# PaddlePaddle/Paddle3D

Measured on AMD Instinct MI355X. Metric: scenes/sec CenterPoint-Pillars nuScenes 300k-pt sweeps, higher is better.
Workload: dtype f32

## Files before the change

### include/paddle3d_amd.h

```cpp
#ifndef PADDLE3D_AMD_H
#define PADDLE3D_AMD_H

#include <stddef.h>
#include <stdint.h>

#ifdef __cplusplus
extern "C" {
#endif

#define PD3_OK 0
#define PD3_EINVAL (-1)
#define PD3_EWORKSPACE (-2)
#define PD3_EUNSUPPORTED (-3)

int pd3_version(void);
const char *pd3_target_arch(void);

int pd3_selfcheck_lds_atomic_order(const uint32_t *addr, uint32_t *old, int blocks, int waves_per_block, int rounds,
                                   int table, void *stream);

size_t pd3_hard_voxelize_workspace(int batch, int64_t max_points, int num_point_dim,
                                   const float *voxel_size, const float *point_cloud_range,
                                   int max_num_points_in_voxel, int max_voxels);
int pd3_hard_voxelize(const float *points, const int32_t *num_points, int batch, int64_t max_points,
                      int num_point_dim, const float *voxel_size, const float *point_cloud_range,
                      int max_num_points_in_voxel, int max_voxels, float *voxels, int32_t *coords,
                      int32_t *num_points_per_voxel, int32_t *num_voxels, int32_t *coors_batched,
                      void *workspace, size_t workspace_bytes, void *stream);
int pd3_hard_voxelize_path(const float *points, const int32_t *num_points, int batch, int64_t max_points,
                           int num_point_dim, const float *voxel_size, const float *point_cloud_range,
                           int max_num_points_in_voxel, int max_voxels, float *voxels, int32_t *coords,
                           int32_t *num_points_per_voxel, int32_t *num_voxels, int32_t *coors_batched,
                           void *workspace, size_t workspace_bytes, void *stream, int path);

int64_t pd3_hard_voxelize_index_list_entries(int batch, int64_t max_points);
int pd3_hard_voxelize_index(const float *points, const int32_t *num_points, int batch, int64_t max_points,
                            int num_point_dim, const float *voxel_size, const float *point_cloud_range,
                            int max_num_points_in_voxel, int max_voxels, int32_t *vox_span, int32_t *point_list,
                            int32_t *coords, int32_t *num_points_per_voxel, int32_t *num_voxels,
                            int32_t *coors_batched, void *workspace, size_t workspace_bytes, void *stream);

int pd3_hard_voxelize_f64(const double *points, const int32_t *num_points, int batch, int64_t max_points,
                          int num_point_dim, const float *voxel_size, const float *point_cloud_range,
                          int max_num_points_in_voxel, int max_voxels, double *voxels, int32_t *coords,
                          int32_t *num_points_per_voxel, int32_t *num_voxels, int32_t *coors_batched,
                          void *workspace, size_t workspace_bytes, void *stream);

int pd3_dynamic_voxelize(const float *points, int64_t num_points, int num_point_dim, const float *voxel_size,
                         const float *point_cloud_range, int32_t *coors, void *stream);

size_t pd3_pointpillars_scatter_workspace(int batch, int ny, int nx);
int pd3_pointpillars_scatter(const float *voxel_features, const int32_t *coords,
                             int64_t num_pillars, int channels, int batch, int ny, int nx,
                             float *canvas, void *workspace, size_t workspace_bytes, void *stream);

int pd3_pointpillars_inverse_map(const int32_t *coords, int64_t num_pillars, int batch, int ny, int nx,
                                 int32_t *inv, void *stream);
int pd3_scatter_conv3x3_bias_relu(const float *voxel_features, const int32_t *inv, const float *w_packed,
                                  const float *bias, int batch, int cin, int cout, int ny, int nx, int stride,
                                  int relu, float *out, int out_w, void *stream);

size_t pd3_pillar_conv_rulebook_workspace(int batch, int ny, int nx, int stride);
int pd3_pillar_conv_rulebook(const int32_t *inverse_map, int batch, int ny, int nx, int stride, int32_t *nbr,
                             int32_t *out_cell, int32_t *cell_row, int32_t *n_out, int capacity, int32_t *order,
                             void *workspace, size_t workspace_bytes, void *stream);
int pd3_rows_to_dense_fill(const float *rows, const int32_t *cell_row, const float *fill, int batch, int channels, int h,
                           int w, float *out, void *stream);

int pd3_pillar_feature_net(const float *voxels, const int32_t *num_points, const int32_t *coors,
                           int64_t num_pillars, int max_points, int num_point_dim,
                           int voxel_center_dims, float vx, float vy, float vz, float x_offset,
                           float y_offset, float z_offset, const float *w1, const float *scale1,
                           const float *shift1, int c1, const float *w2, const float *scale2,
                           const float *shift2, int c2, float *out, void *stream);

int pd3_pillar_feature_net_path(const float *voxels, const int32_t *num_points, const int32_t *coors,
                                int64_t num_pillars, int max_points, int num_point_dim,
                                int voxel_center_dims, float vx, float vy, float vz, float x_offset,
                                float y_offset, float z_offset, const float *w1, const float *scale1,
                                const float *shift1, int c1, const float *w2, const float *scale2,
                                const float *shift2, int c2, float *out, int path, void *stream);

int pd3_pillar_feature_net_indexed(const float *points, int64_t points_per_frame, const int32_t *vox_span,
                                   const int32_t *point_list, int64_t list_stride, const int32_t *coors,
                                   int64_t num_pillars, int pillars_per_frame, int max_points, int num_point_dim,
                                   int voxel_center_dims, float vx, float vy, float vz, float x_offset,
                                   float y_offset, float z_offset, const float *w1, const float *scale1,
                                   const float *shift1, int c1, const float *w2, const float *scale2,
                                   const float *shift2, int c2, float *out, void *stream);

int pd3_voxel_mean(const float *voxels, const int32_t *num_points, int64_t num_voxels,
                   int max_points, int num_point_dim, float *out, void *stream);

size_t pd3_nms_workspace(int num_boxes);
int pd3_nms_bev(const float *boxes, int num_boxes, float nms_overlap_thresh, int32_t *keep,
                int32_t *num_to_keep, void *workspace, size_t workspace_bytes, void *stream);
int pd3_nms_normal(const float *boxes, int num_boxes, float nms_overlap_thresh, int32_t *keep,
                   int32_t *num_to_keep, void *workspace, size_t workspace_bytes, void *stream);
int pd3_boxes_iou_bev(const float *boxes_a, int num_a, const float *boxes_b, int num_b,
                      float *ans_iou, void *stream);
int pd3_boxes_overlap_bev(const float *boxes_a, int num_a, const float *boxes_b, int num_b,
                          float *ans_overlap, void *stream);
int pd3_libm_eval(int op, const float *x, const float *y, float *out, int64_t n, void *stream);

size_t pd3_centerpoint_postprocess_workspace(int batch, int num_tasks, int feat_h, int feat_w,
                                             int nms_pre_max_size, int nms_post_max_size);
int pd3_centerpoint_postprocess(const float *const *hm, const float *const *reg,
                                const float *const *height, const float *const *dim,
                                const float *const *vel, const float *const *rot, int batch,
                                int num_tasks, const int *hm_channels, int feat_h, int feat_w,
                                const float *voxel_size, const float *point_cloud_range,
                                const float *post_center_range, const int *label_offsets,
                                int down_ratio, float score_threshold, float nms_iou_threshold,
                                int nms_pre_max_size, int nms_post_max_size, int with_velocity,
                                float *out_bboxes, float *out_scores, int64_t *out_labels,
                                int32_t *out_count, void *workspace, size_t workspace_bytes,
                                void *stream);

int pd3_centerpoint_postprocess_strided(const float *const *hm, const float *const *reg,
                                const float *const *height, const float *const *dim,
                                const float *const *vel, const float *const *rot, int64_t head_batch_stride, int batch,
                                int num_tasks, const int *hm_channels, int feat_h, int feat_w,
                                const float *voxel_size, const float *point_cloud_range,
                                const float *post_center_range, const int *label_offsets,
                                int down_ratio, float score_threshold, float nms_iou_threshold,
                                int nms_pre_max_size, int nms_post_max_size, int with_velocity,
                                float *out_bboxes, float *out_scores, int64_t *out_labels,
                                int32_t *out_count, void *workspace, size_t workspace_bytes,
                                void *stream, int selection);
int pd3_centerpoint_postprocess_records(const float *const *hm, const float *const *reg,
                                        const float *const *height, const float *const *dim,
                                        const float *const *vel, const float *const *rot,
                                        int64_t head_batch_stride, int batch, int num_tasks,
                                        const int *hm_channels, int feat_h, int feat_w, const float *voxel_size,
                                        const float *point_cloud_range, const float *post_center_range,
                                        const int *label_offsets, int down_ratio, float score_threshold,
                                        float nms_iou_threshold, int nms_pre_max_size, int nms_post_max_size,
                                        int with_velocity, float *out_bboxes, float *out_scores,
                                        int64_t *out_labels, int32_t *out_count, float *out_records,
                                        int max_per_img, void *workspace, size_t workspace_bytes, void *stream);

size_t pd3_bevdet_postprocess_workspace(int batch, int num_tasks, const int *task_classes, int feat_h, int feat_w,
                                        int max_num);
int pd3_bevdet_postprocess(const float *const *heatmap, const float *const *reg, const float *const *height,
                           const float *const *dim, const float *const *rot, const float *const *vel, int batch,
                           int num_tasks, const int *task_classes, int feat_h, int feat_w, const int *nms_type,
                           const float *nms_thr, const double *min_radius, const float *rescale_factors,
                           int max_num, int pre_max_size, int post_max_size, float score_threshold, int norm_bbox,
                           const float *post_center_range, const float *post_center_limit_range,
                           const float *pc_range, const float *voxel_size, float out_size_factor,
                           float *out_bboxes, float *out_scores, int32_t *out_labels, int32_t *out_count,
                           void *workspace, size_t workspace_bytes, void *stream);

size_t pd3_circle_nms_workspace(int n);
int pd3_circle_nms(const float *dets, int n, double thresh, int32_t *keep, int32_t *num_to_keep, void *workspace,
                   size_t workspace_bytes, void *stream);

int pd3_bevdet4d_align(const float *const *feats, const int64_t *strides, int num_frame, int with_current,
                       int batch, int channels, int feat_h, int feat_w, const float *const *rots_cur,
                       const float *const *trans_cur, const float *const *rots_adj, const float *const *trans_adj,
                       const float *const *bda, const float *const *bda_adj, const int64_t *pose_strides,
                       const float *grid_interval, const float *grid_lower_bound, float *out, float *out_grid,
                       void *stream);

int pd3_ms_deform_attn_forward(int dtype, const void *value, const int64_t *spatial_shapes,
                               const int64_t *level_start_index, const void *sampling_loc, const void *attn_weight,
                               int batch, int spatial_size, int num_heads, int channels, int num_levels,
                               int num_query, int num_point, void *out, void *stream);
int pd3_ms_deform_attn_backward(int dtype, const void *value, const int64_t *spatial_shapes,
                                const int64_t *level_start_index, const void *sampling_loc, const void *attn_weight,
                                const void *grad_out, int batch, int spatial_size, int num_heads, int channels,
                                int num_levels, int num_query, int num_point, void *grad_value,
                                void *grad_sampling_loc, void *grad_attn_weight, void *stream);

size_t pd3_farthest_point_sample_workspace(int batch, int n, int tier);
int pd3_farthest_point_sample(const float *xyz, int batch, int n, int m, int tier, void *workspace,
                              size_t workspace_bytes, int *idxs, void *stream);

int pd3_gather_points(const float *points, const int *idx, int batch, int channels, int n, int npoints, float *out,
                      void *stream);
int pd3_gather_points_grad(const float *grad_out, const int *idx, int batch, int channels, int n, int npoints,
                           float *grad_points, void *stream);

int pd3_ball_query_batch(const float *new_xyz, const float *xyz, int batch, int n, int m, float radius, int nsample,
                         int *idx, void *stream);

int pd3_group_points_batch(const float *points, const int *idx, int batch, int channels, int n, int npoints,
                           int nsample, float *out, void *stream);
int pd3_group_points_batch_grad(const float *grad_out, const int *idx, int batch, int channels, int n, int npoints,
                                int nsample, float *grad_points, void *stream);

int pd3_points_in_boxes(const float *pts, const float *boxes, int batch, int npts, int nboxes, int64_t box_row_stride,
                        int64_t box_batch_stride, int *box_idx_of_points, void *stream);

int pd3_ball_query_stack(const float *new_xyz, const int *new_xyz_batch_cnt, const float *xyz,
                         const int *xyz_batch_cnt, int batch, int m, int n, float radius, int nsample, int *idx,
                         void *stream);

int pd3_voxel_query(const float *new_xyz, const float *xyz, const int *new_coords, const int *point_indices, int m,
                    int n, int batch, int z, int y, int x, float radius, int nsample, int z_range, int y_range,
                    int x_range, int *idx, void *stream);

int pd3_group_points_stack(const float *features, const int *features_batch_cnt, const int *idx,
                           const int *idx_batch_cnt, int batch, int n, int channels, int m, int nsample, float *out,
                           void *stream);
int pd3_group_points_stack_grad(const float *grad_out, const int *idx, const int *idx_batch_cnt,
                                const int *features_batch_cnt, int batch, int n, int channels, int m, int nsample,
                                float *grad_features, void *stream);

int pd3_voxel_pool(const float *new_xyz, const float *xyz, const int *new_coords, const int *point_indices,
                   const float *features_in, const float *w_pos, const float *pos_scale, const float *pos_shift, int m,
                   int n, int batch, int z, int y, int x, int c1, float radius, int nsample, int z_range, int y_range,
                   int x_range, int pool, float *pooled, void *stream);

int pd3_roi_grid_points(const float *rois, int64_t num_rois, int rois_per_frame, int grid_size, const float *range_min,
                        const float *voxel_size, const int *strides, int num_strides, float *roi_grid_xyz, int *coords,
                        void *stream);

int pd3_rcnn_decode_boxes(const float *rois, const float *box_preds, int64_t n, float *out, void *stream);

size_t pd3_class_agnostic_nms_workspace(int batch, int64_t num_boxes, int nms_pre_maxsize);
int pd3_class_agnostic_nms(const float *box_preds, const float *cls_preds, int batch, int64_t num_boxes,
                           int num_classes, int apply_sigmoid, float score_thresh, const int64_t *labels,
                           int nms_pre_maxsize, float nms_thresh, int nms_post_maxsize, float *out_boxes,
                           float *out_scores, int64_t *out_labels, int32_t *out_count, void *workspace,
                           size_t workspace_bytes, void *stream);

int pd3_assign_score_withk_forward(const float *scores, const float *points, const float *centers,
                                   const int64_t *knn_idx, int batch, int n, int k, int m, int o, float *output,
                                   void *stream);
size_t pd3_assign_score_withk_backward_workspace(int batch, int n, int k, int o);
int pd3_assign_score_withk_backward(const float *grad_out, const float *scores, const float *points,
                                    const float *centers, const int64_t *knn_idx, int batch, int n, int k, int m,
                                    int o, float *grad_scores, float *grad_points, float *grad_centers,
                                    void *workspace, size_t workspace_bytes, void *stream);

int pd3_bev_pool_v2(const float *depth, const float *feat, const int32_t *ranks_depth,
                    const int32_t *ranks_feat, const int32_t *ranks_bev,
                    const int32_t *interval_lengths, const int32_t *interval_starts,
                    int n_intervals, int channels, int64_t out_elems, float *out, void *stream);
int pd3_bev_pool_v2_bkwd(const float *out_grad, const float *depth, const float *feat,
                         const int32_t *ranks_depth, const int32_t *ranks_feat,
                         const int32_t *ranks_bev, const int32_t *interval_lengths,
                         const int32_t *interval_starts, int n_intervals, int64_t n_points,
                         int channels, int64_t depth_elems, int64_t feat_elems, float *depth_grad,
                         float *feat_grad, void *stream);

int pd3_frustum_to_lidar(const float *frustum, int64_t points_per_camera, int batch, int num_cams,
                         const float *inv_post_rots, const float *post_trans, const float *cam_to_ego,
                         const float *trans, const float *bda, float *coor, void *stream);

size_t pd3_voxel_pooling_prepare_workspace(int64_t num_points);
int pd3_voxel_pooling_prepare(const float *coor, int64_t num_points, int batch, int depth_bins, int feat_hw,
                              const float *grid_lower, const float *grid_interval, const float *grid_size, int mode,
                              int32_t *ranks_bev, int32_t *ranks_depth, int32_t *ranks_feat,
                              int32_t *interval_starts, int32_t *interval_lengths, int32_t *counts, void *workspace,
                              size_t workspace_bytes, void *stream);

size_t pd3_sparse_conv3d_workspace(int n_in, const int *kernel_size, int subm, int out_cap);
int pd3_sparse_conv3d_indices(const int32_t *in_coords, int n_in, int batch, const int *spatial_shape,
                              const int *kernel_size, const int *stride, const int *padding, int subm,
                              int32_t *out_coords, int32_t *nbr, int32_t *n_out, int out_cap,
                              void *workspace, size_t workspace_bytes, void *stream);
int pd3_sparse_conv3d_features(const float *in_feats, const int32_t *nbr, const int32_t *n_out,
                               int n_out_cap, int kernel_volume, int cin, int cout,
                               const float *weight, const float *bias, const float *scale,
                               const float *shift, const float *residual, int relu, float *out,
                               void *stream);
int64_t pd3_sparse_tile_order_entries(int n_out_cap);
int pd3_sparse_tile_order(const int32_t *nbr, const int32_t *n_out, int n_out_cap, int kernel_volume,
                          int32_t *order, void *stream);
int pd3_sparse_conv3d_features_ordered(const float *in_feats, const int32_t *nbr, const int32_t *n_out,
                                       int n_out_cap, int kernel_volume, int cin, int cout,
                                       const float *weight, const float *bias, const float *scale,
                                       const float *shift, const float *residual, int relu,
                                       const int32_t *order, float *out, void *stream);
int pd3_sparse_pack_weight_bf16x3(const float *weight, int kernel_volume, int cin, int cout, void *packed, void *stream);
int pd3_sparse_conv3d_features_bf16x3(const float *in_feats, const int32_t *nbr, const int32_t *n_out, int n_out_cap,
                                      int kernel_volume, int cin, int cout, const void *weight_packed,
                                      const float *bias, const float *scale, const float *shift, const float *residual,
                                      int relu, const int32_t *order, float *out, void *stream);
int pd3_sparse_pack_weight_f16(const float *weight, int kernel_volume, int cin, int cout, void *packed, void *stream);
int pd3_sparse_conv3d_features_f16(const void *in_feats_f16, const int32_t *nbr, const int32_t *n_out, int n_out_cap,
                                   int kernel_volume, int cin, int cout, const void *weight_packed_f16,
                                   const float *bias, const float *scale, const float *shift,
                                   const void *residual_f16, int relu, const int32_t *order, void *out, int out_f32,
                                   void *stream);
int pd3_gather_gemm_f16(const void *in_feats_f16, const int32_t *nbr, const int32_t *n_out, int n_out_cap,
                        int kernel_volume, int cin, int cout, const void *weight_packed_f16, const float *bias,
                        const float *scale, const float *shift, const void *residual_f16, int relu,
                        const int32_t *order, void *out, int out_f32, int out_ld, int out_off, void *stream);
size_t pd3_sparse_plan_workspace(int n_cap);
size_t pd3_sparse_conv_outputs_workspace(int batch, const int *spatial_shape, const int *kernel_size,
                                         const int *stride, const int *padding);
int pd3_sparse_sort_coords(const int32_t *coords, int n, int batch, const int *spatial_shape,
                           uint32_t *keys_sorted, int32_t *order, int32_t *n_valid, void *workspace,
                           size_t workspace_bytes, void *stream);
int pd3_sparse_conv_outputs(const uint32_t *in_keys, const int32_t *n_in, int n_in_cap, int batch,
                            const int *spatial_shape, const int *kernel_size, const int *stride,
                            const int *padding, uint32_t *out_keys, int32_t *n_out, int out_cap,
                            void *workspace, size_t workspace_bytes, void *stream);
size_t pd3_sparse_rulebook_workspace(int batch, const int *spatial_shape);
int pd3_sparse_rulebook(const uint32_t *in_keys, const int32_t *n_in, int n_in_cap, const uint32_t *out_keys,
                        const int32_t *n_out, int n_out_cap, int batch, const int *spatial_shape,
                        const int *kernel_size, const int *stride, const int *padding, int subm, int32_t *nbr,
                        int32_t *out_coords, void *workspace, size_t workspace_bytes, void *stream);
int pd3_sparse_to_dense(const float *feats, const int32_t *coords, const int32_t *n, int n_cap,
                        int channels, int batch, const int *spatial_shape, float *dense, void *stream);

size_t pd3_merge_sweeps_workspace(int64_t num_points);
int pd3_merge_sweeps(const float *points, const int64_t *sweep_offsets, int num_sweeps, int dim_in,
                     int use_dim, const double *ref_from_curr, const int32_t *has_transform,
                     const float *time_lag, int use_time_lag,
                     float remove_radius, float *out, int32_t *num_out, void *workspace,
                     size_t workspace_bytes, void *stream);

int pd3_conv3x3_bias_relu(const float *x, const float *w_packed, const float *bias, int batch, int cin,
                          int cout, int h, int w, int w_valid, int stride, int relu, float *out, int out_w,
                          void *stream);

int pd3_conv3x3_winograd43_bias_relu(const float *x, const float *u_packed, const float *bias, int batch,
                                     int cin, int cout, int h, int w, int w_valid, int relu, float *out,
                                     int channels_per_tile, void *stream);

int pd3_conv3x3_winograd43_pp_bias_relu(const float *x, const float *u_lane, const float *bias, int batch, int cin,
                                        int cout, int h, int w, int w_valid, int relu, float *out, void *stream);

size_t pd3_winograd43_input_transform_floats(int batch, int cin, int h, int w);
int pd3_winograd43_input_transform(const float *x, int batch, int cin, int h, int w, int w_valid, float *v_pre,
                                   void *stream);
int pd3_conv3x3_winograd43_ppv_bias_relu(const float *v_pre, const float *u_lane, const float *bias, int batch, int cin,
                                         int cout, int h, int w, int w_valid, int relu, float *out, void *stream);
int pd3_conv3x3_winograd43_pp_trace(const float *x, const float *u_lane, const float *bias, int batch, int cin, int cout,
                                    int h, int w, int relu, float *out, long long *dbg, void *stream);

size_t pd3_stable_argsort_workspace(int64_t n, uint32_t max_key);
int pd3_stable_argsort(const void *keys, int64_t n, int mode, uint32_t max_key, int32_t *order, void *workspace,
                       size_t workspace_bytes, void *stream);

int pd3_conv3x3_f16_bias_relu(const void *x_f16_nhwc, const void *w_packed_f16, const float *bias, int batch, int cin,
                              int cout, int h, int w, int relu, void *out, int out_mode, int channels_per_tile,
                              void *stream);
int pd3_conv3x3_f16_bias_relu_dual(const void *x_f16_nhwc, const void *w_packed_f16, const float *bias, int batch,
                                   int cin, int cout, int h, int w, int relu, void *out_f16_nhwc, float *out_f32_nchw,
                                   int channels_per_tile, void *stream);
int pd3_conv3x3_s2_f16_bias_relu(const void *x_f16_nhwc, const void *w_packed_f16, const float *bias, int batch, int cin,
                                 int cout, int h, int w, int relu, void *out_f16_nhwc, void *stream);
int pd3_scatter_conv3x3_s2_f16_bias_relu(const void *features_f16, const int32_t *inverse_map, const void *w_packed_f16,
                                         const float *bias, int batch, int cin, int cout, int ny, int nx, int relu,
                                         void *out_f16_nhwc, int channels_per_tile, void *stream);
int pd3_grouped_conv3x3_small_f16(const void *x_f16_nhwc, const void *w_f16, const float *bias, int batch, int groups,
                                  int channels_per_group, int out_per_group, int h, int w, float *out, int out_groups,
                                  int out_group0, void *stream);
int pd3_grouped_conv3x3_small_f16_gm(const void *x_f16_group_major, const void *w_f16, const float *bias, int batch,
                                     int groups, int channels_per_group, int out_per_group, int h, int w, float *out,
                                     int out_groups, int out_group0, void *stream);
int pd3_f32_nchw_to_f16_nhwc(const float *x, int batch, int channels, int h, int w, void *out, void *stream);

int pd3_grouped_conv3x3_small(const float *x, const float *w_grouped, const float *bias, int batch, int groups,
                              int cin_per_group, int cout_per_group, int h, int w, float *out, void *stream);
int pd3_grouped_conv3x3_small_slice(const float *x, const float *w_grouped, const float *bias, int batch, int groups,
                                    int cin_per_group, int cout_per_group, int h, int w, float *out, int out_groups,
                                    int out_group0, void *stream);

int pd3_conv3x3_winograd_bias_relu(const float *x, const float *u_packed, const float *bias, int batch,
                                   int cin, int cout, int h, int w, int relu, float *out, void *stream);

int pd3_patch_conv_bias_relu(const float *x, const float *w_packed, const float *bias, int mode, int batch,
                             int cin, int cout, int h, int w, int w_valid, int relu, float *out,
                             int out_channels_total, int out_channel_offset, void *stream);

int pd3_patch_conv_x3_bias_relu(const float *x, const void *w_packed, const float *bias, int mode, int batch, int cin,
                                int cout, int h, int w, int w_valid, int relu, float *out, int out_channels_total,
                                int out_channel_offset, void *stream);

int pd3_conv3x3_s2_x3_bias_relu(const float *x, const void *w_packed, const float *bias, int batch, int cin, int cout,
                                int h, int w, int w_valid, int relu, float *out, int out_w, void *stream);

size_t pd3_ssd_postprocess_workspace(int batch, int feat_h, int feat_w, int anchors_per_loc, int grid_x, int grid_y,
                                     int nms_pre_max_size);
int pd3_ssd_postprocess(const float *head_map, int64_t batch_stride, int cls_channel0, int box_channel0,
                        int dir_channel0, int batch, int feat_h, int feat_w, int anchors_per_loc, int num_classes,
                        int encode_background_as_zeros, const float *anchors, const int32_t *anchors_bv,
                        const int32_t *coors, int64_t num_coors, int grid_x, int grid_y,
                        float anchor_area_threshold, float score_threshold, const float *center_limit_range,
                        float nms_iou_threshold, int nms_pre_max_size, int nms_post_max_size, float *out_boxes,
                        float *out_scores, int64_t *out_labels, int32_t *out_count, void *workspace,
                        size_t workspace_bytes, void *stream, int selection);

#ifdef __cplusplus
}
#endif
#endif
```

### paddle3d_amd/_lib.py

```python
from __future__ import annotations

import ctypes as C
import os
from functools import lru_cache

_HERE = os.path.dirname(os.path.abspath(__file__))
LIB_PATH = os.path.join(_HERE, "lib", "libpaddle3d_amd.so")

c_f32p = C.c_void_p
c_i32p = C.c_void_p

_SIGNATURES = {
    "pd3_version": (C.c_int, []),
    "pd3_target_arch": (C.c_char_p, []),
    "pd3_hard_voxelize_workspace": (C.c_size_t, [C.c_int, C.c_int64, C.c_int, C.c_void_p, C.c_void_p,
                                                 C.c_int, C.c_int]),
    "pd3_hard_voxelize": (C.c_int, [C.c_void_p, C.c_void_p, C.c_int, C.c_int64, C.c_int, C.c_void_p,
                                    C.c_void_p, C.c_int, C.c_int, C.c_void_p, C.c_void_p, C.c_void_p,
                                    C.c_void_p, C.c_void_p, C.c_void_p, C.c_size_t, C.c_void_p]),
    "pd3_hard_voxelize_f64": (C.c_int, [C.c_void_p, C.c_void_p, C.c_int, C.c_int64, C.c_int, C.c_void_p,
                                    C.c_void_p, C.c_int, C.c_int, C.c_void_p, C.c_void_p, C.c_void_p,
                                    C.c_void_p, C.c_void_p, C.c_void_p, C.c_size_t, C.c_void_p]),
    "pd3_hard_voxelize_path": (C.c_int, [C.c_void_p, C.c_void_p, C.c_int, C.c_int64, C.c_int, C.c_void_p,
                                         C.c_void_p, C.c_int, C.c_int, C.c_void_p, C.c_void_p, C.c_void_p,
                                         C.c_void_p, C.c_void_p, C.c_void_p, C.c_size_t, C.c_void_p, C.c_int]),
    "pd3_hard_voxelize_index_list_entries": (C.c_int64, [C.c_int, C.c_int64]),
    "pd3_hard_voxelize_index": (C.c_int, [C.c_void_p, C.c_void_p, C.c_int, C.c_int64, C.c_int, C.c_void_p,
                                          C.c_void_p, C.c_int, C.c_int, C.c_void_p, C.c_void_p, C.c_void_p,
                                          C.c_void_p, C.c_void_p, C.c_void_p, C.c_void_p, C.c_size_t, C.c_void_p]),
    "pd3_pillar_feature_net_indexed": (C.c_int, [C.c_void_p, C.c_int64, C.c_void_p, C.c_void_p, C.c_int64, C.c_void_p,
                                                 C.c_int64, C.c_int, C.c_int, C.c_int, C.c_int, C.c_float, C.c_float,
                                                 C.c_float, C.c_float, C.c_float, C.c_float, C.c_void_p, C.c_void_p,
                                                 C.c_void_p, C.c_int, C.c_void_p, C.c_void_p, C.c_void_p, C.c_int,
                                                 C.c_void_p, C.c_void_p]),
    "pd3_pointpillars_scatter_workspace": (C.c_size_t, [C.c_int, C.c_int, C.c_int]),
    "pd3_pointpillars_scatter": (C.c_int, [C.c_void_p, C.c_void_p, C.c_int64, C.c_int, C.c_int, C.c_int,
                                           C.c_int, C.c_void_p, C.c_void_p, C.c_size_t, C.c_void_p]),
    "pd3_pillar_feature_net": (C.c_int, [C.c_void_p, C.c_void_p, C.c_void_p, C.c_int64, C.c_int, C.c_int,
                                         C.c_int, C.c_float, C.c_float, C.c_float, C.c_float, C.c_float,
                                         C.c_float, C.c_void_p,
                                         C.c_void_p, C.c_void_p, C.c_int, C.c_void_p, C.c_void_p,
                                         C.c_void_p, C.c_int, C.c_void_p, C.c_void_p]),
    "pd3_pillar_feature_net_path": (C.c_int, [C.c_void_p, C.c_void_p, C.c_void_p, C.c_int64, C.c_int, C.c_int,
                                              C.c_int, C.c_float, C.c_float, C.c_float, C.c_float, C.c_float,
                                              C.c_float, C.c_void_p,
                                              C.c_void_p, C.c_void_p, C.c_int, C.c_void_p, C.c_void_p,
                                              C.c_void_p, C.c_int, C.c_void_p, C.c_int, C.c_void_p]),
    "pd3_voxel_mean": (C.c_int, [C.c_void_p, C.c_void_p, C.c_int64, C.c_int, C.c_int, C.c_void_p,
                                 C.c_void_p]),
    "pd3_nms_workspace": (C.c_size_t, [C.c_int]),
    "pd3_nms_bev": (C.c_int, [C.c_void_p, C.c_int, C.c_float, C.c_void_p, C.c_void_p, C.c_void_p,
                              C.c_size_t, C.c_void_p]),
    "pd3_nms_normal": (C.c_int, [C.c_void_p, C.c_int, C.c_float, C.c_void_p, C.c_void_p, C.c_void_p,
                                 C.c_size_t, C.c_void_p]),
    "pd3_boxes_iou_bev": (C.c_int, [C.c_void_p, C.c_int, C.c_void_p, C.c_int, C.c_void_p, C.c_void_p]),
    "pd3_boxes_overlap_bev": (C.c_int, [C.c_void_p, C.c_int, C.c_void_p, C.c_int, C.c_void_p,
                                        C.c_void_p]),
    "pd3_libm_eval": (C.c_int, [C.c_int, C.c_void_p, C.c_void_p, C.c_void_p, C.c_int64, C.c_void_p]),
    "pd3_centerpoint_postprocess_workspace": (C.c_size_t, [C.c_int, C.c_int, C.c_int, C.c_int, C.c_int, C.c_int]),
    "pd3_centerpoint_postprocess": (C.c_int, [C.c_void_p] * 6 + [C.c_int, C.c_int, C.c_void_p, C.c_int, C.c_int,
                                              C.c_void_p, C.c_void_p, C.c_void_p, C.c_void_p, C.c_int,
                                              C.c_float, C.c_float, C.c_int, C.c_int, C.c_int,
                                              C.c_void_p, C.c_void_p, C.c_void_p, C.c_void_p,
                                              C.c_void_p, C.c_size_t, C.c_void_p]),
    "pd3_centerpoint_postprocess_strided": (C.c_int, [C.c_void_p] * 6 + [C.c_int64, C.c_int, C.c_int, C.c_void_p,
                                                      C.c_int, C.c_int, C.c_void_p, C.c_void_p, C.c_void_p,
                                                      C.c_void_p, C.c_int, C.c_float, C.c_float, C.c_int, C.c_int,
                                                      C.c_int, C.c_void_p, C.c_void_p, C.c_void_p, C.c_void_p,
                                                      C.c_void_p, C.c_size_t, C.c_void_p, C.c_int]),
    "pd3_centerpoint_postprocess_records": (C.c_int, [C.c_void_p] * 6 + [C.c_int64, C.c_int, C.c_int, C.c_void_p,
                                                      C.c_int, C.c_int, C.c_void_p, C.c_void_p, C.c_void_p,
                                                      C.c_void_p, C.c_int, C.c_float, C.c_float, C.c_int, C.c_int,
                                                      C.c_int, C.c_void_p, C.c_void_p, C.c_void_p, C.c_void_p,
                                                      C.c_void_p, C.c_int, C.c_void_p, C.c_size_t, C.c_void_p]),
    "pd3_ms_deform_attn_forward": (C.c_int, [C.c_int] + [C.c_void_p] * 5 + [C.c_int] * 7 + [C.c_void_p] * 2),
    "pd3_ms_deform_attn_backward": (C.c_int, [C.c_int] + [C.c_void_p] * 6 + [C.c_int] * 7 + [C.c_void_p] * 4),
    "pd3_farthest_point_sample_workspace": (C.c_size_t, [C.c_int, C.c_int, C.c_int]),
    "pd3_farthest_point_sample": (C.c_int, [C.c_void_p, C.c_int, C.c_int, C.c_int, C.c_int, C.c_void_p, C.c_size_t,
                                            C.c_void_p, C.c_void_p]),
    "pd3_gather_points": (C.c_int, [C.c_void_p, C.c_void_p] + [C.c_int] * 4 + [C.c_void_p, C.c_void_p]),
    "pd3_gather_points_grad": (C.c_int, [C.c_void_p, C.c_void_p] + [C.c_int] * 4 + [C.c_void_p, C.c_void_p]),
    "pd3_ball_query_batch": (C.c_int, [C.c_void_p, C.c_void_p, C.c_int, C.c_int, C.c_int, C.c_float, C.c_int,
                                       C.c_void_p, C.c_void_p]),
    "pd3_group_points_batch": (C.c_int, [C.c_void_p, C.c_void_p] + [C.c_int] * 5 + [C.c_void_p, C.c_void_p]),
    "pd3_group_points_batch_grad": (C.c_int, [C.c_void_p, C.c_void_p] + [C.c_int] * 5 + [C.c_void_p, C.c_void_p]),
    "pd3_points_in_boxes": (C.c_int, [C.c_void_p, C.c_void_p, C.c_int, C.c_int, C.c_int, C.c_int64, C.c_int64,
                                      C.c_void_p, C.c_void_p]),
    "pd3_ball_query_stack": (C.c_int, [C.c_void_p] * 4 + [C.c_int] * 3 + [C.c_float, C.c_int, C.c_void_p,
                                                                            C.c_void_p]),
    "pd3_voxel_query": (C.c_int, [C.c_void_p] * 4 + [C.c_int] * 6 + [C.c_float] + [C.c_int] * 4 + [C.c_void_p] * 2),
    "pd3_group_points_stack": (C.c_int, [C.c_void_p] * 4 + [C.c_int] * 5 + [C.c_void_p] * 2),
    "pd3_group_points_stack_grad": (C.c_int, [C.c_void_p] * 4 + [C.c_int] * 5 + [C.c_void_p] * 2),
    "pd3_assign_score_withk_forward": (C.c_int, [C.c_void_p] * 4 + [C.c_int] * 5 + [C.c_void_p] * 2),
    "pd3_assign_score_withk_backward_workspace": (C.c_size_t, [C.c_int] * 4),
    "pd3_assign_score_withk_backward": (C.c_int, [C.c_void_p] * 5 + [C.c_int] * 5 + [C.c_void_p] * 4 +
                                        [C.c_size_t, C.c_void_p]),
    "pd3_bev_pool_v2": (C.c_int, [C.c_void_p] * 7 + [C.c_int, C.c_int, C.c_int64, C.c_void_p,
                                                     C.c_void_p]),
    "pd3_bev_pool_v2_bkwd": (C.c_int, [C.c_void_p] * 8 + [C.c_int, C.c_int64, C.c_int, C.c_int64, C.c_int64,
                                                          C.c_void_p, C.c_void_p, C.c_void_p]),
    "pd3_frustum_to_lidar": (C.c_int, [C.c_void_p, C.c_int64, C.c_int, C.c_int] + [C.c_void_p] * 7),
    "pd3_voxel_pooling_prepare_workspace": (C.c_size_t, [C.c_int64]),
    "pd3_voxel_pooling_prepare": (C.c_int, [C.c_void_p, C.c_int64, C.c_int, C.c_int, C.c_int, C.c_void_p, C.c_void_p,
                                            C.c_void_p, C.c_int] + [C.c_void_p] * 7 + [C.c_size_t, C.c_void_p]),
    "pd3_sparse_conv3d_workspace": (C.c_size_t, [C.c_int, C.c_void_p, C.c_int, C.c_int]),
    "pd3_sparse_conv3d_indices": (C.c_int, [C.c_void_p, C.c_int, C.c_int, C.c_void_p, C.c_void_p, C.c_void_p,
                                            C.c_void_p, C.c_int, C.c_void_p, C.c_void_p, C.c_void_p, C.c_int,
                                            C.c_void_p, C.c_size_t, C.c_void_p]),
    "pd3_sparse_conv3d_features": (C.c_int, [C.c_void_p, C.c_void_p, C.c_void_p, C.c_int, C.c_int, C.c_int,
                                             C.c_int, C.c_void_p, C.c_void_p, C.c_void_p, C.c_void_p,
                                             C.c_void_p, C.c_int, C.c_void_p, C.c_void_p]),
    "pd3_sparse_conv3d_features_ordered": (C.c_int, [C.c_void_p, C.c_void_p, C.c_void_p, C.c_int, C.c_int, C.c_int,
                                                     C.c_int, C.c_void_p, C.c_void_p, C.c_void_p, C.c_void_p,
                                                     C.c_void_p, C.c_int, C.c_void_p, C.c_void_p, C.c_void_p]),
    "pd3_sparse_pack_weight_bf16x3": (C.c_int, [C.c_void_p, C.c_int, C.c_int, C.c_int, C.c_void_p, C.c_void_p]),
    "pd3_sparse_conv3d_features_bf16x3": (C.c_int, [C.c_void_p, C.c_void_p, C.c_void_p, C.c_int, C.c_int, C.c_int,
                                                    C.c_int, C.c_void_p, C.c_void_p, C.c_void_p, C.c_void_p, C.c_void_p,
                                                    C.c_int, C.c_void_p, C.c_void_p, C.c_void_p]),
    "pd3_sparse_pack_weight_f16": (C.c_int, [C.c_void_p, C.c_int, C.c_int, C.c_int, C.c_void_p, C.c_void_p]),
    "pd3_sparse_conv3d_features_f16": (C.c_int, [C.c_void_p, C.c_void_p, C.c_void_p, C.c_int, C.c_int, C.c_int, C.c_int,
                                                 C.c_void_p, C.c_void_p, C.c_void_p, C.c_void_p, C.c_void_p, C.c_int,
                                                 C.c_void_p, C.c_void_p, C.c_int, C.c_void_p]),
    "pd3_gather_gemm_f16": (C.c_int, [C.c_void_p, C.c_void_p, C.c_void_p, C.c_int, C.c_int, C.c_int, C.c_int,
                                      C.c_void_p, C.c_void_p, C.c_void_p, C.c_void_p, C.c_void_p, C.c_int, C.c_void_p,
                                      C.c_void_p, C.c_int, C.c_int, C.c_int, C.c_void_p]),
    "pd3_sparse_tile_order_entries": (C.c_int64, [C.c_int]),
    "pd3_sparse_tile_order": (C.c_int, [C.c_void_p, C.c_void_p, C.c_int, C.c_int, C.c_void_p, C.c_void_p]),
    "pd3_sparse_plan_workspace": (C.c_size_t, [C.c_int]),
    "pd3_sparse_conv_outputs_workspace": (C.c_size_t, [C.c_int] + [C.c_void_p] * 4),
    "pd3_sparse_sort_coords": (C.c_int, [C.c_void_p, C.c_int, C.c_int, C.c_void_p, C.c_void_p, C.c_void_p,
                                         C.c_void_p, C.c_void_p, C.c_size_t, C.c_void_p]),
    "pd3_sparse_conv_outputs": (C.c_int, [C.c_void_p, C.c_void_p, C.c_int, C.c_int, C.c_void_p, C.c_void_p,
                                          C.c_void_p, C.c_void_p, C.c_void_p, C.c_void_p, C.c_int, C.c_void_p,
                                          C.c_size_t, C.c_void_p]),
    "pd3_sparse_rulebook_workspace": (C.c_size_t, [C.c_int, C.c_void_p]),
    "pd3_sparse_rulebook": (C.c_int, [C.c_void_p, C.c_void_p, C.c_int, C.c_void_p, C.c_void_p, C.c_int, C.c_int,
                                      C.c_void_p, C.c_void_p, C.c_void_p, C.c_void_p, C.c_int, C.c_void_p,
                                      C.c_void_p, C.c_void_p, C.c_size_t, C.c_void_p]),
    "pd3_sparse_to_dense": (C.c_int, [C.c_void_p, C.c_void_p, C.c_void_p, C.c_int, C.c_int, C.c_int,
                                      C.c_void_p, C.c_void_p, C.c_void_p]),
    "pd3_selfcheck_lds_atomic_order": (C.c_int, [C.c_void_p, C.c_void_p, C.c_int, C.c_int, C.c_int, C.c_int,
                                                 C.c_void_p]),
    "pd3_conv3x3_f16_bias_relu": (C.c_int, [C.c_void_p, C.c_void_p, C.c_void_p, C.c_int, C.c_int, C.c_int, C.c_int,
                                            C.c_int, C.c_int, C.c_void_p, C.c_int, C.c_int, C.c_void_p]),
    "pd3_f32_nchw_to_f16_nhwc": (C.c_int, [C.c_void_p, C.c_int, C.c_int, C.c_int, C.c_int, C.c_void_p, C.c_void_p]),
    "pd3_conv3x3_f16_bias_relu_dual": (C.c_int, [C.c_void_p, C.c_void_p, C.c_void_p, C.c_int, C.c_int, C.c_int, C.c_int,
                                                 C.c_int, C.c_int, C.c_void_p, C.c_void_p, C.c_int, C.c_void_p]),
    "pd3_conv3x3_s2_f16_bias_relu": (C.c_int, [C.c_void_p, C.c_void_p, C.c_void_p, C.c_int, C.c_int, C.c_int, C.c_int,
                                               C.c_int, C.c_int, C.c_void_p, C.c_void_p]),
    "pd3_scatter_conv3x3_s2_f16_bias_relu": (C.c_int, [C.c_void_p, C.c_void_p, C.c_void_p, C.c_void_p, C.c_int, C.c_int,
                                                       C.c_int, C.c_int, C.c_int, C.c_int, C.c_void_p, C.c_int,
                                                       C.c_void_p]),
    "pd3_grouped_conv3x3_small_f16": (C.c_int, [C.c_void_p, C.c_void_p, C.c_void_p, C.c_int, C.c_int, C.c_int, C.c_int,
                                                C.c_int, C.c_int, C.c_void_p, C.c_int, C.c_int, C.c_void_p]),
    "pd3_grouped_conv3x3_small_f16_gm": (C.c_int, [C.c_void_p, C.c_void_p, C.c_void_p, C.c_int, C.c_int, C.c_int, C.c_int,
                                                   C.c_int, C.c_int, C.c_void_p, C.c_int, C.c_int, C.c_void_p]),
    "pd3_stable_argsort_workspace": (C.c_size_t, [C.c_int64, C.c_uint32]),
    "pd3_stable_argsort": (C.c_int, [C.c_void_p, C.c_int64, C.c_int, C.c_uint32, C.c_void_p, C.c_void_p, C.c_size_t,
                                     C.c_void_p]),
    "pd3_conv3x3_winograd43_pp_bias_relu": (C.c_int, [C.c_void_p, C.c_void_p, C.c_void_p, C.c_int, C.c_int, C.c_int,
                                                       C.c_int, C.c_int, C.c_int, C.c_int, C.c_void_p, C.c_void_p]),
    "pd3_conv3x3_winograd43_pp_trace": (C.c_int, [C.c_void_p, C.c_void_p, C.c_void_p, C.c_int, C.c_int, C.c_int, C.c_int,
                                                  C.c_int, C.c_int, C.c_void_p, C.c_void_p, C.c_void_p]),
    "pd3_merge_sweeps_workspace": (C.c_size_t, [C.c_int64]),
    "pd3_merge_sweeps": (C.c_int, [C.c_void_p, C.c_void_p, C.c_int, C.c_int, C.c_int, C.c_void_p, C.c_void_p,
                                   C.c_void_p, C.c_int, C.c_float, C.c_void_p, C.c_void_p, C.c_void_p, C.c_size_t,
                                   C.c_void_p]),
    "pd3_dynamic_voxelize": (C.c_int, [C.c_void_p, C.c_int64, C.c_int, C.c_void_p, C.c_void_p, C.c_void_p, C.c_void_p]),
    "pd3_conv3x3_bias_relu": (C.c_int, [C.c_void_p, C.c_void_p, C.c_void_p, C.c_int, C.c_int, C.c_int, C.c_int,
                                        C.c_int, C.c_int, C.c_int, C.c_int, C.c_void_p, C.c_int, C.c_void_p]),
    "pd3_conv3x3_winograd_bias_relu": (C.c_int, [C.c_void_p, C.c_void_p, C.c_void_p, C.c_int, C.c_int, C.c_int,
                                                 C.c_int, C.c_int, C.c_int, C.c_void_p, C.c_void_p]),
    "pd3_conv3x3_winograd43_bias_relu": (C.c_int, [C.c_void_p, C.c_void_p, C.c_void_p, C.c_int, C.c_int, C.c_int,
                                                   C.c_int, C.c_int, C.c_int, C.c_int, C.c_void_p, C.c_int,
                                                   C.c_void_p]),
    "pd3_patch_conv_bias_relu": (C.c_int, [C.c_void_p, C.c_void_p, C.c_void_p, C.c_int, C.c_int, C.c_int, C.c_int,
                                           C.c_int, C.c_int, C.c_int, C.c_int, C.c_void_p, C.c_int, C.c_int,
                                           C.c_void_p]),
    "pd3_patch_conv_x3_bias_relu": (C.c_int, [C.c_void_p, C.c_void_p, C.c_void_p, C.c_int, C.c_int, C.c_int, C.c_int,
                                              C.c_int, C.c_int, C.c_int, C.c_int, C.c_void_p, C.c_int, C.c_int,
                                              C.c_void_p]),
    "pd3_conv3x3_s2_x3_bias_relu": (C.c_int, [C.c_void_p, C.c_void_p, C.c_void_p, C.c_int, C.c_int, C.c_int, C.c_int,
                                              C.c_int, C.c_int, C.c_int, C.c_void_p, C.c_int, C.c_void_p]),
    "pd3_winograd43_input_transform_floats": (C.c_size_t, [C.c_int] * 4),
    "pd3_winograd43_input_transform": (C.c_int, [C.c_void_p, C.c_int, C.c_int, C.c_int, C.c_int, C.c_int, C.c_void_p,
                                                 C.c_void_p]),
    "pd3_conv3x3_winograd43_ppv_bias_relu": (C.c_int, [C.c_void_p, C.c_void_p, C.c_void_p, C.c_int, C.c_int, C.c_int,
                                                       C.c_int, C.c_int, C.c_int, C.c_int, C.c_void_p, C.c_void_p]),
    "pd3_ssd_postprocess_workspace": (C.c_size_t, [C.c_int] * 7),
    "pd3_ssd_postprocess": (C.c_int, [C.c_void_p, C.c_int64, C.c_int, C.c_int, C.c_int, C.c_int, C.c_int, C.c_int,
                                      C.c_int, C.c_int, C.c_int, C.c_void_p, C.c_void_p, C.c_void_p, C.c_int64,
                                      C.c_int, C.c_int, C.c_float, C.c_float, C.c_void_p, C.c_float, C.c_int, C.c_int,
                                      C.c_void_p, C.c_void_p, C.c_void_p, C.c_void_p, C.c_void_p, C.c_size_t,
                                      C.c_void_p, C.c_int]),
    "pd3_pointpillars_inverse_map": (C.c_int, [C.c_void_p, C.c_int64, C.c_int, C.c_int, C.c_int, C.c_void_p,
                                               C.c_void_p]),
    "pd3_scatter_conv3x3_bias_relu": (C.c_int, [C.c_void_p, C.c_void_p, C.c_void_p, C.c_void_p, C.c_int, C.c_int,
                                                C.c_int, C.c_int, C.c_int, C.c_int, C.c_int, C.c_void_p, C.c_int,
                                                C.c_void_p]),
    "pd3_pillar_conv_rulebook_workspace": (C.c_size_t, [C.c_int] * 4),
    "pd3_pillar_conv_rulebook": (C.c_int, [C.c_void_p, C.c_int, C.c_int, C.c_int, C.c_int, C.c_void_p, C.c_void_p,
                                           C.c_void_p, C.c_void_p, C.c_int, C.c_void_p, C.c_void_p, C.c_size_t,
                                           C.c_void_p]),
    "pd3_rows_to_dense_fill": (C.c_int, [C.c_void_p, C.c_void_p, C.c_void_p, C.c_int, C.c_int, C.c_int, C.c_int,
                                         C.c_void_p, C.c_void_p]),
    "pd3_bevdet_postprocess_workspace": (C.c_size_t, [C.c_int, C.c_int, C.c_void_p, C.c_int, C.c_int, C.c_int]),
    "pd3_bevdet_postprocess": (C.c_int, [C.c_void_p] * 6 + [C.c_int, C.c_int, C.c_void_p, C.c_int, C.c_int,
                                         C.c_void_p, C.c_void_p, C.c_void_p, C.c_void_p, C.c_int, C.c_int,
                                         C.c_int, C.c_float, C.c_int, C.c_void_p, C.c_void_p, C.c_void_p,
                                         C.c_void_p, C.c_float, C.c_void_p, C.c_void_p, C.c_void_p, C.c_void_p,
                                         C.c_void_p, C.c_size_t, C.c_void_p]),
    "pd3_circle_nms_workspace": (C.c_size_t, [C.c_int]),
    "pd3_circle_nms": (C.c_int, [C.c_void_p, C.c_int, C.c_double, C.c_void_p, C.c_void_p, C.c_void_p, C.c_size_t,
                                 C.c_void_p]),
    "pd3_bevdet4d_align": (C.c_int, [C.c_void_p, C.c_void_p] + [C.c_int] * 6 + [C.c_void_p] * 12),
    "pd3_grouped_conv3x3_small": (C.c_int, [C.c_void_p, C.c_void_p, C.c_void_p, C.c_int, C.c_int, C.c_int, C.c_int,
                                            C.c_int, C.c_int, C.c_void_p, C.c_void_p]),
    "pd3_grouped_conv3x3_small_slice": (C.c_int, [C.c_void_p, C.c_void_p, C.c_void_p, C.c_int, C.c_int, C.c_int,
                                                  C.c_int, C.c_int, C.c_int, C.c_void_p, C.c_int, C.c_int,
                                                  C.c_void_p]),
}

SYMBOLS = tuple(_SIGNATURES)

_SIGNATURES_ROI = {
    "pd3_voxel_pool": (C.c_int, [C.c_void_p] * 8 + [C.c_int] * 7 + [C.c_float] + [C.c_int] * 5 + [C.c_void_p] * 2),
    "pd3_roi_grid_points": (C.c_int, [C.c_void_p, C.c_int64, C.c_int, C.c_int] + [C.c_void_p] * 3 + [C.c_int] +
                            [C.c_void_p] * 3),
    "pd3_rcnn_decode_boxes": (C.c_int, [C.c_void_p, C.c_void_p, C.c_int64, C.c_void_p, C.c_void_p]),
    "pd3_class_agnostic_nms_workspace": (C.c_size_t, [C.c_int, C.c_int64, C.c_int]),
    "pd3_class_agnostic_nms": (C.c_int, [C.c_void_p, C.c_void_p, C.c_int, C.c_int64, C.c_int, C.c_int, C.c_float,
                                         C.c_void_p, C.c_int, C.c_float, C.c_int] + [C.c_void_p] * 5 +
                               [C.c_size_t, C.c_void_p]),
}

SYMBOLS_ROI = tuple(_SIGNATURES_ROI)


class Paddle3DAmdError(RuntimeError):
    pass


@lru_cache(maxsize=None)
def lib() -> C.CDLL:
    if not os.path.exists(LIB_PATH):
        raise Paddle3DAmdError(
            f"{LIB_PATH} not found: build it with `python -m paddle3d_amd.build` "
            "(there is no CPU / PyTorch fallback for the HIP ops)")
    handle = C.CDLL(LIB_PATH)
    for name, (res, args) in list(_SIGNATURES.items()) + list(_SIGNATURES_ROI.items()):
        try:
            fn = getattr(handle, name)
        except AttributeError as e:
            raise Paddle3DAmdError(f"{LIB_PATH} does not export {name}") from e
        fn.restype = res
        fn.argtypes = args
    return handle


def check(status: int, what: str) -> None:
    if status == 0:
        return
    if status < 0:
        msg = {-1: "invalid argument", -2: "workspace too small", -3: "unsupported configuration"}.get(
            status, "error")
        raise Paddle3DAmdError(f"{what}: {msg} (status {status})")
    raise Paddle3DAmdError(f"{what}: HIP error {status}")
```

### paddle3d_amd/build.py

```python
from __future__ import annotations

import concurrent.futures as cf
import os
import subprocess
import sys

HERE = os.path.dirname(os.path.abspath(__file__))
CSRC = os.path.join(HERE, "csrc")
OBJ = os.path.join(HERE, "lib", "obj")
LIB = os.path.join(HERE, "lib", "libpaddle3d_amd.so")
ARCH = "gfx950"
HIPCC = os.environ.get("HIPCC", "/opt/rocm/bin/hipcc")
FLAGS = [f"--offload-arch={ARCH}", "-O3", "-std=c++17", "-fPIC", "-ffp-contract=off", "-fno-fast-math",
         "-Wall", "-Wno-unused-function", "-Wno-unused-result"]


def _sources():
    return sorted(os.path.join(CSRC, f) for f in os.listdir(CSRC) if f.endswith(".hip"))


def _headers():
    hs = [os.path.join(CSRC, f) for f in os.listdir(CSRC) if f.endswith(".hpp")]
    hs.append(os.path.join(HERE, "..", "include", "paddle3d_amd.h"))
    return hs


def _stale(target, deps):
    if not os.path.exists(target):
        return True
    t = os.path.getmtime(target)
    return any(os.path.getmtime(d) > t for d in deps)


EXTRA_FLAGS = {}


def _compile(src, force):
    obj = os.path.join(OBJ, os.path.basename(src)[:-4] + ".o")
    if force or _stale(obj, [src] + _headers()):
        cmd = [HIPCC, *FLAGS, *EXTRA_FLAGS.get(os.path.basename(src), []), "-c", src, "-o", obj]
        r = subprocess.run(cmd, capture_output=True, text=True)
        if r.returncode != 0:
            raise RuntimeError(f"hipcc failed for {src}:\n{r.stdout}\n{r.stderr}")
        if r.stderr.strip():
            sys.stderr.write(r.stderr)
    return obj


def build(force: bool = False) -> str:
    os.makedirs(OBJ, exist_ok=True)
    srcs = _sources()
    with cf.ThreadPoolExecutor(max_workers=min(8, len(srcs))) as ex:
        objs = list(ex.map(lambda s: _compile(s, force), srcs))
    if force or _stale(LIB, objs):
        cmd = [HIPCC, f"--offload-arch={ARCH}", "-shared", "-fPIC", "-o", LIB, *objs]
        r = subprocess.run(cmd, capture_output=True, text=True)
        if r.returncode != 0:
            raise RuntimeError(f"link failed:\n{r.stdout}\n{r.stderr}")
    return LIB


if __name__ == "__main__":
    print(build(force="--force" in sys.argv))
```

### paddle3d_amd/centerpoint.py

```python
from __future__ import annotations

import math

import numpy as np
import torch
import torch.nn as nn

from ._lib import Paddle3DAmdError
from .ops import centerpoint_postprocess as _cp
from .ops import conv as _conv
from .ops import pointpillars_scatter as _ps
from .ops import sparse_conv3d as _sp3
from .ops import voxel_encoder as _ve
from .ops import voxelize as _vox

__all__ = ["HardVoxelizer", "PillarFeatureNet", "HardVFE", "VoxelMean", "PointPillarsScatter", "SecondBackbone",
           "SecondFPN", "CenterHead", "CenterPoint", "centerpoint_pillars_nuscenes", "centerpoint_pillars_kitti",
           "centerpoint_voxels_nuscenes", "centerpoint_voxels_kitti", "load_paddle_state_dict"]


def _grid(voxel_size, point_cloud_range):
    pr = np.array(point_cloud_range, dtype=np.float32)
    vs = np.array(voxel_size, dtype=np.float32)
    return np.round((pr[3:] - pr[:3]) / vs).astype(np.int64)


class HardVoxelizer(nn.Module):

    def __init__(self, voxel_size, point_cloud_range, max_num_points_in_voxel, max_num_voxels, path: int = 0):
        super().__init__()
        self.path = int(path)
        self.voxel_size = list(map(float, voxel_size))
        self.point_cloud_range = list(map(float, point_cloud_range))
        self.max_num_points_in_voxel = int(max_num_points_in_voxel)
        if isinstance(max_num_voxels, (tuple, list)):
            self.max_num_voxels = list(max_num_voxels)
        else:
            self.max_num_voxels = [max_num_voxels, max_num_voxels]

    def forward(self, points: torch.Tensor, num_points: torch.Tensor | None = None):
        v = self.max_num_voxels[0] if self.training else self.max_num_voxels[1]
        voxels, _, npv, nv, coors = _vox.hard_voxelize_batch(points, self.voxel_size, self.point_cloud_range,
                                                             self.max_num_points_in_voxel, v, num_points,
                                                             with_batch_coors=True, path=self.path)
        return voxels, coors, npv, nv

    def index(self, points: torch.Tensor, num_points: torch.Tensor | None = None):
        if self.path != 0:
            return None
        v = self.max_num_voxels[0] if self.training else self.max_num_voxels[1]
        res = _vox.hard_voxelize_index_batch(points, self.voxel_size, self.point_cloud_range,
                                             self.max_num_points_in_voxel, v, num_points)
        if res is None:
            return None
        span, plist, _, npv, nv, coors = res
        return span, plist, coors, npv, nv


class PFNLayer(nn.Module):

    def __init__(self, in_channels, out_channels, last_layer=False):
        super().__init__()
        self.last_vfe = last_layer
        self.units = out_channels if last_layer else out_channels // 2
        self.linear = nn.Linear(in_channels, self.units, bias=False)
        self.norm = nn.BatchNorm1d(self.units, eps=1e-3, momentum=0.01)
        bound = 1 / math.sqrt(in_channels)
        nn.init.uniform_(self.linear.weight, -bound, bound)


class PillarFeatureNet(nn.Module):

    def __init__(self, in_channels=4, feat_channels=(64,), with_distance=False, max_num_points_in_voxel=20,
                 voxel_size=(0.2, 0.2, 4), point_cloud_range=(0, -40, -3, 70.4, 40, 1), legacy=False):
        super().__init__()
        if with_distance or legacy:
            raise NotImplementedError("with_distance / legacy PFN variants are not on the hot path")
        if len(feat_channels) not in (1, 2):
            raise NotImplementedError("the fused PFN op covers one or two PFN layers")
        self.in_channels = in_channels
        chans = [in_channels + 5] + list(feat_channels)
        self.pfn_layers = nn.ModuleList(
            PFNLayer(chans[i], chans[i + 1], last_layer=(i == len(chans) - 2)) for i in range(len(chans) - 1))
        for i in range(1, len(self.pfn_layers)):
            assert self.pfn_layers[i].linear.in_features == 2 * self.pfn_layers[i - 1].units
        self.vx, self.vy = float(voxel_size[0]), float(voxel_size[1])
        self.x_offset = self.vx / 2 + point_cloud_range[0]
        self.y_offset = self.vy / 2 + point_cloud_range[1]
        self.max_num_points_in_voxel = max_num_points_in_voxel
        self._folded = None

    def train(self, mode: bool = True):
        self._folded = None
        return super().train(mode)

    def _fold(self):
        out = []
        for l in self.pfn_layers:
            scale, shift = _ve.fold_batchnorm(l.norm.weight, l.norm.bias, l.norm.running_mean,
                                              l.norm.running_var, l.norm.eps)
            out += [l.linear.weight.t().contiguous(), scale, shift]
        return [t.detach() for t in out]

    def forward(self, features, num_points_per_voxel, coors):
        sig = _param_signature(self)
        if self.training or self._folded is None or self._folded[0] != sig:
            self._folded = (sig, self._fold())
        return _ve.pillar_feature_net(features, num_points_per_voxel, coors, self.vx, self.vy, self.x_offset,
                                      self.y_offset, *self._folded[1])

    def forward_indexed(self, points, vox_span, point_list, coors):
        if len(self.pfn_layers) != 2:
            return None
        sig = _param_signature(self)
        if self.training or self._folded is None or self._folded[0] != sig:
            self._folded = (sig, self._fold())
        return _ve.pillar_feature_net_indexed(points, vox_span, point_list, coors, self.max_num_points_in_voxel,
                                              self.vx, self.vy, self.x_offset, self.y_offset, *self._folded[1])


class HardVFE(nn.Module):

    def __init__(self, in_channels=4, feat_channels=(64, 64), with_distance=False, with_cluster_center=True,
                 with_voxel_center=True, voxel_size=(0.2, 0.2, 4), point_cloud_range=(0, -40, -3, 70.4, 40, 1)):
        super().__init__()
        if with_distance or not (with_cluster_center and with_voxel_center) or len(feat_channels) != 2:
            raise NotImplementedError("HardVFE: only the BEVFusion configuration is on the hot path")
        self.voxel_size, self.point_cloud_range = tuple(voxel_size), tuple(point_cloud_range)
        chans = [in_channels + 6] + list(feat_channels)

        class _VFE(nn.Module):
            def __init__(self, cin, cout):
                super().__init__()
                self.linear = nn.Linear(cin, cout, bias=False)
                self.norm = nn.BatchNorm1d(cout, eps=1e-3, momentum=0.01)

        self.vfe_layers = nn.ModuleList([_VFE(chans[0], chans[1]), _VFE(2 * chans[1], chans[2])])

    def forward(self, features, num_points, coors):
        args = []
        for l in self.vfe_layers:
            scale, shift = _ve.fold_batchnorm(l.norm.weight, l.norm.bias, l.norm.running_mean, l.norm.running_var,
                                              l.norm.eps)
            args += [l.linear.weight.t().contiguous().detach(), scale.detach(), shift.detach()]
        return _ve.hard_vfe(features, num_points, coors, self.voxel_size, self.point_cloud_range, *args)


class VoxelMean(nn.Module):

    def __init__(self, in_channels=4):
        super().__init__()
        self.in_channels = in_channels

    def forward(self, features, num_points_per_voxel, coors=None):
        assert self.in_channels == features.shape[-1]
        return _ve.voxel_mean(features, num_points_per_voxel)


class PointPillarsScatter(nn.Module):

    def __init__(self, in_channels, voxel_size, point_cloud_range):
        super().__init__()
        self.in_channels = in_channels
        g = _grid(voxel_size, point_cloud_range)
        self.nx, self.ny = int(g[0]), int(g[1])

    def forward(self, voxel_features, coords, batch_size):
        return _ps.pointpillars_scatter(voxel_features, coords, batch_size, self.ny, self.nx)

    def sparse(self, voxel_features, coords, batch_size):
        return _ps.SparseCanvas(voxel_features, coords, batch_size, self.ny, self.nx)


def _param_signature(module):
    return tuple((t.data_ptr(), t._version, str(t.device)) for t in list(module.parameters()) + list(module.buffers()))


def invalidate_derived(module):
    for m in module.modules():
        if hasattr(m, "_drop_cache"):
            m._drop_cache()
        if hasattr(m, "_folded"):
            m._folded = None
        if getattr(m, "_pd3_folded", None) is not None:
            object.__setattr__(m, "_pd3_folded", None)
    return module


class _InferenceCache:

    _cache = None
    _cache_sig = None

    def _drop_cache(self):
        self.__dict__["_cache"] = None
        self.__dict__["_cache_sig"] = None

    def _cache_valid(self):
        return self._cache is not None and self._cache_sig == _param_signature(self)

    def _store_cache(self, value):
        self.__dict__["_cache"] = value
        self.__dict__["_cache_sig"] = _param_signature(self)
        return value

    def train(self, mode: bool = True):
        self._drop_cache()
        return super().train(mode)

    def invalidate(self):
        invalidate_derived(self)
        return self

    def _require_eval(self):
        if self.training:
            raise RuntimeError(f"{type(self).__name__}: paddle3d_amd implements the inference path only "
                               "(BatchNorm folded into the HIP kernels); call .eval() first")


def _conv_bn_relu(cin, cout, k, stride=1, padding=0, transpose=False, eps=1e-3, momentum=0.01, bias=False):
    conv = (nn.ConvTranspose2d if transpose else nn.Conv2d)(cin, cout, k, stride=stride, padding=padding, bias=bias)
    return [conv, nn.BatchNorm2d(cout, eps=eps, momentum=momentum), nn.ReLU()]


def _fold_conv_bn(conv: nn.Conv2d, bn: nn.BatchNorm2d):
    scale = bn.weight / torch.sqrt(bn.running_var + bn.eps)
    if isinstance(conv, nn.ConvTranspose2d):
        w = conv.weight * scale.reshape(1, -1, 1, 1)
    else:
        w = conv.weight * scale.reshape(-1, 1, 1, 1)
    b = (conv.bias if conv.bias is not None else torch.zeros_like(bn.running_mean))
    return w.detach().contiguous(), ((b - bn.running_mean) * scale + bn.bias).detach().contiguous()


class _Conv3x3:

    def __init__(self, w, b, stride):
        self.w, self.b, self.stride = w, b, int(stride)
        self.cout, self.cin = int(w.shape[0]), int(w.shape[1])
        self.packed = {}

    def winograd43(self, h, pitch):
        if self.stride != 1:
            return None, None
        if self.cin >= _conv.WINOGRAD43_PP_MIN_CIN and _conv.winograd43_pp_supported(self.cin, self.cout, h, pitch):
            form, key, pack = "pp", "w43pp", _conv.pack_winograd43_lane_weight
        elif _conv.winograd43_supported(self.cin, self.cout, h, pitch):
            form, key, pack = "packed", "w43", _conv.pack_winograd43_weight
        else:
            return None, None
        if key not in self.packed:
            self.packed[key] = pack(self.w)
        return form, self.packed[key]

    def __call__(self, x, w_valid=None):
        h, wv = int(x.shape[2]), int(x.shape[3] if w_valid is None else w_valid)
        form, u = self.winograd43(h, int(x.shape[3]))
        if form == "pp":
            if 0 < _conv.WINOGRAD43_PPV_MIN_BLOCKS <= self.cout // 64:
                vpre = _conv.winograd43_input_transform(x, w_valid=wv)
                return _conv.conv3x3_winograd43_ppv_bias_relu(vpre, x.shape, u, self.b, self.cout, relu=True,
                                                              w_valid=wv), wv
            return _conv.conv3x3_winograd43_pp_bias_relu(x, u, self.b, self.cout, relu=True, w_valid=wv), wv
        if form == "packed":
            return _conv.conv3x3_winograd43_bias_relu(x, u, self.b, self.cout, relu=True, w_valid=wv), wv
        if (self.stride == 2 and _conv.S2_BF16X3 and int(x.shape[3]) % 4 == 0
                and _conv.conv3x3_s2_x3_supported(self.cin, self.cout, h, wv, int(x.shape[0]))):
            if "s2x3" not in self.packed:
                self.packed["s2x3"] = _conv.pack_conv3x3_s2_x3_weight(self.w)
            return _conv.conv3x3_s2_x3_bias_relu(x, self.packed["s2x3"], self.b, self.cout, relu=True,
                                                 w_valid=wv), wv // 2
        if _conv.supported(self.cin, self.cout, h, wv, self.stride):
            if "direct" not in self.packed:
                self.packed["direct"] = _conv.pack_conv3x3_weight(self.w)
            return _conv.conv3x3_bias_relu(x, self.packed["direct"], self.b, self.cout, relu=True, stride=self.stride,
                                           w_valid=wv), wv // self.stride
        raise Paddle3DAmdError(f"conv3x3: unsupported configuration (cin {self.cin}, cout {self.cout}, stride "
                               f"{self.stride}, input {h}x{wv}) (status -3)")

    def f16_ok(self, h, w):
        return self.stride == 1 and _conv.f16_supported(self.cin, self.cout, int(h), int(w))

    def f16_s2_ok(self):
        return self.stride == 2 and _conv.s2_f16_supported(self.cin, self.cout)

    def f16_s2(self, x_h):
        if "f16s2" not in self.packed:
            self.packed["f16s2"] = _conv.pack_conv3x3_f16_weight(self.w, tile=128)
        return _conv.conv3x3_s2_f16_bias_relu(x_h, self.packed["f16s2"], self.b, self.cout, relu=True)

    def f16_dual(self, x_h):
        if "f16" not in self.packed:
            self.packed["f16"] = _conv.pack_conv3x3_f16_weight(self.w)
        return _conv.conv3x3_f16_bias_relu_dual(x_h, self.packed["f16"], self.b, self.cout, relu=True)

    def f16(self, x_h, out_f32_nchw=False, out=None, tiles=None, group_major=False):
        if "f16" not in self.packed:
            self.packed["f16"] = _conv.pack_conv3x3_f16_weight(self.w)
        wp, b, cout = self.packed["f16"], self.b, self.cout
        if tiles is not None:
            t = int(wp.shape[4])
            wp, b, cout = wp[tiles[0]:tiles[1]], self.b[tiles[0] * t:tiles[1] * t], (tiles[1] - tiles[0]) * t
        return _conv.conv3x3_f16_bias_relu(x_h, wp, b, cout, relu=True, out_f32_nchw=out_f32_nchw, out=out,
                                           group_major=group_major)


def _valid_w(t) -> int:
    return int(getattr(t, "_pd3_valid_w", t.shape[3]))


def _f16_nhwc_to_f32_nchw(xh):
    x = xh.permute(0, 3, 1, 2).float()
    w = int(x.shape[3])
    pad = _conv.pitch4(w) - w
    if pad:
        x = torch.nn.functional.pad(x, (0, pad))
    return _tag_valid_w(x.contiguous(), w)


def _tag_valid_w(t, wv):
    if t.dtype == torch.float16:
        return t
    if wv != t.shape[3]:
        t._pd3_valid_w = int(wv)
    return t


def _fold_conv3x3(conv, bn):
    if (isinstance(conv, nn.ConvTranspose2d) or tuple(conv.kernel_size) != (3, 3) or tuple(conv.padding) != (1, 1)
            or tuple(conv.stride) not in ((1, 1), (2, 2))):
        raise Paddle3DAmdError(f"unsupported configuration: {conv} is not a 3x3 / pad 1 / stride 1|2 convolution")
    w, b = _fold_conv_bn(conv, bn)
    return _Conv3x3(w, b, conv.stride[0])


class SecondBackbone(_InferenceCache, nn.Module):

    def __init__(self, in_channels=128, out_channels=(128, 128, 256), layer_nums=(3, 5, 5),
                 downsample_strides=(2, 2, 2)):
        super().__init__()
        in_filters = [in_channels, *out_channels[:-1]]
        blocks = []
        for i, n in enumerate(layer_nums):
            block = _conv_bn_relu(in_filters[i], out_channels[i], 3, stride=downsample_strides[i], padding=1)
            for _ in range(n):
                block += _conv_bn_relu(out_channels[i], out_channels[i], 3, padding=1)
            blocks.append(nn.Sequential(*block))
        self.blocks = nn.ModuleList(blocks)
        self.sparse_first = True
        self.amp = False
        self.amp_out_f16 = False

    def _plan(self):
        if not self._cache_valid():
            plan = []
            for blk in self.blocks:
                mods = list(blk)
                plan.append([_fold_conv3x3(mods[i], mods[i + 1]) for i in range(0, len(mods), 3)])
            self._store_cache(plan)
        return self._cache

    def forward(self, x):
        self._require_eval()
        plan = self._plan()
        first = None
        first_h = None
        if isinstance(x, _ps.SparseCanvas):
            c0 = plan[0][0]
            if (self.amp and c0.stride == 2 and x.shape[1] == c0.cin and len(plan[0]) > 1
                    and _conv.scatter_conv_s2_f16_supported(c0.cin, c0.cout, x.ny, x.nx)
                    and plan[0][1].f16_ok(x.ny // 2, x.nx // 2)):
                key = "f16s2_64" if c0.cout % 128 else "f16s2"
                if key not in c0.packed:
                    c0.packed[key] = _conv.pack_conv3x3_f16_weight(c0.w, tile=64 if c0.cout % 128 else 128)
                first_h = _conv.scatter_conv3x3_s2_f16_bias_relu(x, c0.packed[key], c0.b, c0.cout)
                first = (None, x.nx // 2)
            elif (self.sparse_first and x.shape[1] == c0.cin
                  and _conv.scatter_conv_sparse_supported(c0.cin, c0.cout, x.ny, x.nx, c0.stride)):
                y, c0.packed["x3sparse"] = _conv.scatter_conv3x3_sparse(x, c0.w, c0.b, c0.packed.get("x3sparse"))
                first = (y, x.nx // 2)
            elif _conv.scatter_conv_supported(c0.cin, c0.cout, x.ny, x.nx, c0.stride) and x.shape[1] == c0.cin:
                if "direct" not in c0.packed:
                    c0.packed["direct"] = _conv.pack_conv3x3_weight(c0.w)
                first = (_conv.scatter_conv3x3_bias_relu(x, c0.packed["direct"], c0.b, c0.cout), x.nx // 2)
            else:
                x = x.dense()
        if first is None and x.shape[3] % 4:
            raise Paddle3DAmdError(f"SecondBackbone: unsupported configuration (input width {x.shape[3]} is not a "
                                   "multiple of 4) (status -3)")
        outs, wv = [], (0 if first is not None else int(x.shape[3]))
        carry = None
        for bi, layers in enumerate(plan):
            li = 0
            while li < len(layers):
                conv = layers[li]
                xh = None
                if first is not None and bi == 0 and li == 0:
                    x, wv = first
                    li += 1
                    if first_h is None:
                        continue
                    xh = first_h
                    conv = layers[li]
                if self.amp and li == 0 and carry is not None and conv.f16_s2_ok() and wv == carry.shape[2]:
                    xh = conv.f16_s2(carry)
                    li, wv = 1, wv // 2
                    x = None
                carry = None
                if xh is None and x.dtype == torch.float16:
                    x = _f16_nhwc_to_f32_nchw(x)
                h_now = int(xh.shape[1]) if xh is not None else int(x.shape[2])
                w_now = int(xh.shape[2]) if xh is not None else int(x.shape[3])
                run = li
                while (self.amp and run < len(layers) and wv == w_now and layers[run].f16_ok(h_now, w_now)):
                    run += 1
                if run > li and w_now % 4 and not (run == len(layers) and self.amp_out_f16):
                    run = li
                if run > li:
                    if xh is None:
                        xh = _conv.to_f16_nhwc(x)
                    nxt = plan[bi + 1][0] if bi + 1 < len(plan) else None
                    opens = run == len(layers) and nxt is not None and nxt.f16_s2_ok()
                    stage_h = run == len(layers) and self.amp_out_f16
                    for k in range(li, run):
                        if k == run - 1 and stage_h:
                            xh = layers[k].f16(xh)
                            x, carry = xh, (xh if opens else None)
                        elif k == run - 1 and opens:
                            carry, x = layers[k].f16_dual(xh)
                        else:
                            xh = layers[k].f16(xh, out_f32_nchw=(k == run - 1))
                            x = xh
                    li = run
                    continue
                if xh is not None:
                    x = _f16_nhwc_to_f32_nchw(xh)
                    continue
                x, wv = conv(x, wv)
                li += 1
            outs.append(_tag_valid_w(x, wv))
        return tuple(outs)


class SecondFPN(_InferenceCache, nn.Module):

    def __init__(self, in_channels=(128, 128, 256), out_channels=(256, 256, 256), upsample_strides=(1, 2, 4),
                 use_conv_for_no_stride=False):
        super().__init__()
        deblocks = []
        for i, oc in enumerate(out_channels):
            stride = upsample_strides[i]
            if stride > 1 or (stride == 1 and not use_conv_for_no_stride):
                layer = _conv_bn_relu(in_channels[i], oc, int(stride), stride=int(stride), transpose=True)
            else:
                s = round(1 / stride)
                layer = _conv_bn_relu(in_channels[i], oc, s, stride=s)
            deblocks.append(nn.Sequential(*layer))
        self.deblocks = nn.ModuleList(deblocks)

    def _plan(self):
        if not self._cache_valid():
            plan, off = [], 0
            for blk in self.deblocks:
                conv, bn = blk[0], blk[1]
                tr = isinstance(conv, nn.ConvTranspose2d)
                w, b = _fold_conv_bn(conv, bn)
                mode = _conv.patch_mode(w, conv.stride[0], tr)
                if mode is None or tuple(conv.padding) != (0, 0) or conv.stride[0] != conv.stride[1]:
                    raise Paddle3DAmdError(f"unsupported configuration: FPN level {conv} is not a kernel = stride "
                                           "(conv 1 / 2, transposed conv 1 / 2 / 4) layer (status -3)")
                cout = int(w.shape[1] if tr else w.shape[0])
                cin = int(w.shape[0] if tr else w.shape[1])
                plan.append(dict(mode=mode, w=_conv.pack_patch_weight(w, mode, tr), wraw=w, tr=tr, b=b, cin=cin, cout=cout, off=off,
                                 scale={0: 0.5, 1: 1, 2: 2, 3: 4}[mode]))
                off += cout
            self._store_cache((plan, off))
        return self._cache

    def _amp_level(self, i, p, n, h, w, dev, tag=None):
        key = (i, n, h, w, str(dev))
        cache = self.__dict__.setdefault("_amp_tables", {})
        if len(cache) > 64:
            cache.clear()
        if key not in cache:
            conv = self.deblocks[i][0]
            s = int(conv.stride[0])
            tr = isinstance(conv, nn.ConvTranspose2d)
            ho, wo = (h * s, w * s) if tr else (h // s, w // s)
            b = torch.arange(n, device=dev).view(n, 1, 1)
            y = torch.arange(ho, device=dev).view(1, ho, 1)
            x = torch.arange(wo, device=dev).view(1, 1, wo)
            if tr:
                src = ((b * h + y // s) * w + x // s).reshape(-1)
                tap = ((y % s) * s + x % s).expand(n, ho, wo).reshape(-1)
                nbr = torch.full((n * ho * wo, s * s), -1, dtype=torch.int32, device=dev)
                nbr[torch.arange(n * ho * wo, device=dev), tap] = src.int()
            else:
                cols = [((b * h + y * s + dy) * w + x * s + dx).reshape(-1) for dy in range(s) for dx in range(s)]
                nbr = torch.stack(cols, 1).int().contiguous()
            order = _sp3.tile_order(nbr) if tr and s > 1 else None
            cache[key] = (nbr, order, ho, wo)
        wkey = ("w", i, str(dev))
        if tag is None:
            tag = _param_signature(self)
        if wkey not in cache or cache[wkey][0] != tag:
            conv, bn = self.deblocks[i][0], self.deblocks[i][1]
            tr = isinstance(conv, nn.ConvTranspose2d)
            wf, bf = _fold_conv_bn(conv, bn)
            wk = wf.permute(2, 3, 0, 1) if tr else wf.permute(2, 3, 1, 0)
            wk = wk.reshape(-1, wk.shape[2], wk.shape[3]).contiguous()
            parts = []
            step = 128 if wk.shape[2] % 128 == 0 else (64 if wk.shape[2] % 64 == 0 else 32)
            for c0 in range(0, wk.shape[2], step):
                parts.append((c0, step, _sp3.pack_weight_f16(wk[:, :, c0:c0 + step].contiguous()), bf[c0:c0 + step].contiguous()))
            cache[wkey] = (tag, parts)
        return cache[key], cache[wkey][1]

    def amp_ok(self, xs):
        plan, _ = self._plan()
        return all(p["cin"] % 16 == 0 and p["cout"] % 32 == 0 and p["scale"] in (0.5, 1, 2, 4) for p in plan)

    def forward_f16(self, xs):
        self._require_eval()
        plan, ctot = self._plan()
        n = int(xs[0].shape[0])
        out = None
        tag = _param_signature(self)
        for i, (p, x) in enumerate(zip(plan, xs)):
            h, w = int(x.shape[1]), int(x.shape[2])
            (nbr, order, ho, wo), parts = self._amp_level(i, p, n, h, w, x.device, tag)
            if out is None:
                out = torch.empty((n, ho, wo, ctot), dtype=torch.float16, device=x.device)
            elif tuple(out.shape[1:3]) != (ho, wo):
                raise Paddle3DAmdError("SecondFPN: the levels do not meet at one resolution")
            for c0, step, wp, bias in parts:
                _sp3.gather_gemm_f16(x.view(n * h * w, p["cin"]), nbr, wp, p["cin"], step, out.view(n * ho * wo, ctot),
                                     p["off"] + c0, bias=bias, relu=True, order=order)
        return out

    def forward(self, xs):
        self._require_eval()
        plan, ctot = self._plan()
        if all(x.dtype == torch.float16 for x in xs):
            return self.forward_f16(xs)
        xs = [_f16_nhwc_to_f32_nchw(x) if x.dtype == torch.float16 else x for x in xs]
        sizes = {(int(x.shape[2] * p["scale"]), int(_valid_w(x) * p["scale"])) for p, x in zip(plan, xs)}
        if len(sizes) != 1 or len(plan) != len(xs):
            raise Paddle3DAmdError(f"SecondFPN: the levels do not meet at one resolution ({sorted(sizes)})")
        hw = sizes.pop()
        out = torch.empty((xs[0].shape[0], ctot, hw[0], hw[1]), dtype=torch.float32, device=xs[0].device)
        for p, x in zip(plan, xs):
            if not _conv.patch_supported(p["mode"], p["cin"], p["cout"], int(x.shape[2]), int(x.shape[3])):
                raise Paddle3DAmdError(f"patch_conv: unsupported configuration (mode {p['mode']}, cin {p['cin']}, "
                                       f"cout {p['cout']}, input {tuple(x.shape[2:])}) (status -3)")
            if p["mode"] < 2 and _valid_w(x) != x.shape[3]:
                raise Paddle3DAmdError(f"patch_conv: unsupported configuration (mode {p['mode']} on a map of width "
                                       f"{_valid_w(x)}, not a multiple of 4) (status -3)")
            if _conv.PATCH_BF16X3 and _conv.patch_x3_supported(p["mode"], p["cin"], p["cout"], int(x.shape[2]),
                                                               int(x.shape[3]), int(x.shape[0]), ctot):
                if "wx3" not in p:
                    p["wx3"] = _conv.pack_patch_weight_x3(p["wraw"], p["mode"], p["tr"])
                _conv.patch_conv_x3_bias_relu(x, p["wx3"], p["b"], p["mode"], p["cout"], out, p["off"], relu=True,
                                              w_valid=_valid_w(x))
                continue
            _conv.patch_conv_bias_relu(x, p["w"], p["b"], p["mode"], p["cout"], out, p["off"], relu=True,
                                       w_valid=_valid_w(x))
        return out


class ConvModule(nn.Module):

    def __init__(self, cin, cout, k, padding=0):
        super().__init__()
        self.conv = nn.Conv2d(cin, cout, k, padding=padding, bias=True)
        self.bn = nn.BatchNorm2d(cout, eps=1e-5, momentum=0.1)
        self.activate = nn.ReLU()


class SeparateHead(nn.Module):

    def __init__(self, in_channels, heads, head_conv=64, final_kernel=1, init_bias=-2.19):
        super().__init__()
        self.heads = heads
        for head, (classes, num_conv) in heads.items():
            layers, c_in = [], in_channels
            for _ in range(num_conv - 1):
                layers.append(ConvModule(c_in, head_conv, final_kernel, padding=final_kernel // 2))
                c_in = head_conv
            layers.append(nn.Conv2d(head_conv, classes, final_kernel, padding=final_kernel // 2, bias=True))
            setattr(self, head, nn.Sequential(*layers))
        with torch.no_grad():
            getattr(self, "hm")[-1].bias.fill_(init_bias)


class CenterHead(_InferenceCache, nn.Module):

    def __init__(self, in_channels, tasks, common_heads, init_bias=-2.19, share_conv_channel=64, num_hm_conv=2,
                 **_unused):
        super().__init__()
        self.num_classes = [len(t["class_names"]) for t in tasks]
        self.class_names = [t["class_names"] for t in tasks]
        self.with_velocity = "vel" in common_heads
        self.box_n_dim = 9 if self.with_velocity else 7
        self.shared_conv = ConvModule(in_channels, share_conv_channel, 3, padding=1)
        self.head_chunk = 0
        self.head_chunk_bytes = 1 << 30
        self.amp = False
        self.tasks = nn.ModuleList()
        for ncls in self.num_classes:
            heads = dict(common_heads)
            heads.update(hm=(ncls, num_hm_conv))
            self.tasks.append(SeparateHead(share_conv_channel, heads, final_kernel=3, init_bias=init_bias))

    def _plan(self):
        if not self._cache_valid():
            w0, b0 = _fold_conv_bn(self.shared_conv.conv, self.shared_conv.bn)
            ws, bs, plan, finals = [], [], [], []
            for t, task in enumerate(self.tasks):
                for head in task.heads:
                    seq = getattr(task, head)
                    if len(seq) != 2 or tuple(seq[1].kernel_size) != (3, 3):
                        raise Paddle3DAmdError("unsupported configuration: the fused CenterHead expects num_conv == 2 "
                                               "and 3x3 final convolutions for every head (status -3)")
                    w, b = _fold_conv_bn(seq[0].conv, seq[0].bn)
                    ws.append(w)
                    bs.append(b)
                    plan.append((t, head))
                    finals.append((seq[1].weight.detach(), seq[1].bias.detach()))
            cmax = max(f[0].shape[0] for f in finals)
            hc = ws[0].shape[0]
            wf = torch.zeros(len(finals) * cmax, hc, 3, 3, device=w0.device, dtype=w0.dtype)
            bf = torch.zeros(len(finals) * cmax, device=w0.device, dtype=w0.dtype)
            for g, (w, b) in enumerate(finals):
                wf[g * cmax:g * cmax + w.shape[0]] = w
                bf[g * cmax:g * cmax + w.shape[0]] = b
            self._store_cache(dict(
                shared=_Conv3x3(w0, b0, 1), first=_Conv3x3(torch.cat(ws, 0).contiguous(), torch.cat(bs, 0).contiguous(), 1),
                pf=_conv.pack_grouped_weight(wf, len(finals)), bf=bf, hc=int(hc), plan=plan, cmax=int(cmax), wf=wf,
                groups=len(finals), ncls=[int(f[0].shape[0]) for f in finals]))
        return self._cache

    def forward(self, x, want_shared=True):
        self._require_eval()
        f = self._plan()
        nhwc = x.dtype == torch.float16
        hh, ww = (int(x.shape[1]), int(x.shape[2])) if nhwc else (int(x.shape[2]), int(x.shape[3]))
        if ww % 4:
            raise Paddle3DAmdError(f"CenterHead: unsupported configuration (map width {ww} is not a multiple "
                                   "of 4) (status -3)")
        amp = self.amp and f["shared"].f16_ok(hh, ww) and f["first"].f16_ok(hh, ww) and f["hc"] == 64
        if nhwc and not amp:
            x, nhwc = x.permute(0, 3, 1, 2).float().contiguous(), False
        if amp:
            x = f["shared"].f16(x if nhwc else _conv.to_f16_nhwc(x))
            n, h, w, _ = (int(v) for v in x.shape)
        else:
            x, _ = f["shared"](x)
            n, _, h, w = (int(v) for v in x.shape)
        if not _conv.grouped_small_supported(f["hc"], f["cmax"], h, w):
            raise Paddle3DAmdError(f"grouped_conv3x3_small: unsupported configuration ({f['hc']} -> {f['cmax']} "
                                   f"channels per group, map {(h, w)}) (status -3)")
        first, groups = f["first"], f["groups"]
        full = n * f["hc"] * h * w * 4 * groups
        k = self.head_chunk if self.head_chunk else ((groups + 1) // 2 if full > self.head_chunk_bytes else groups)
        if amp:
            if "pf16" not in f:
                f["pf16"] = _conv.pack_grouped_weight_f16(f["wf"], groups)
            full = full // 2
            k = self.head_chunk if self.head_chunk else ((groups + 1) // 2 if full > self.head_chunk_bytes else groups)
            k = k + (k & 1) if k < groups else groups
            z = torch.empty((n, groups * f["cmax"], h, w), dtype=torch.float32, device=x.device)
            buf = torch.empty((n * min(k, groups) * 64 * h * w,), dtype=torch.float16, device=x.device)
            per = _conv.f16_tile(first.cout) // 64
            for c0 in range(0, groups, k):
                c1 = min(c0 + k, groups)
                y = buf[: n * (c1 - c0) * 64 * h * w].view(n, c1 - c0, h, w, 64)
                first.f16(x, out_f32_nchw=False, out=y, tiles=(c0 // per, c1 // per), group_major=True)
                _conv.grouped_conv3x3_small_f16(y, f["pf16"][c0:c1], f["bf"][c0 * f["cmax"]:c1 * f["cmax"]], c1 - c0,
                                                out=z, out_groups=groups, out_group0=c0, group_major=True)
            rets = [dict() for _ in self.tasks]
            for g, (t, head) in enumerate(f["plan"]):
                rets[t][head] = z[:, g * f["cmax"]:g * f["cmax"] + f["ncls"][g]]
            return rets, (x.permute(0, 3, 1, 2).float() if want_shared else None)
        form, u = first.winograd43(h, w) if k < groups and f["hc"] == 64 and w % 4 == 0 else (None, None)
        pp = form == "pp"
        if pp or (form == "packed" and int(u.shape[2]) * 16 == 64):
            wino = _conv.conv3x3_winograd43_pp_bias_relu if pp else _conv.conv3x3_winograd43_bias_relu
            z = torch.empty((n, groups * f["cmax"], h, w), dtype=torch.float32, device=x.device)
            buf = torch.empty((n * k * 64 * h * w,), dtype=torch.float32, device=x.device)
            vpre = (_conv.winograd43_input_transform(x)
                    if pp and 0 < _conv.WINOGRAD43_PPV_MIN_BLOCKS <= groups else None)
            for c0 in range(0, groups, k):
                c1 = min(c0 + k, groups)
                y = buf[: n * (c1 - c0) * 64 * h * w].view(n, (c1 - c0) * 64, h, w)
                if vpre is not None:
                    _conv.conv3x3_winograd43_ppv_bias_relu(vpre, x.shape, u[c0:c1], first.b[c0 * 64:c1 * 64],
                                                           (c1 - c0) * 64, relu=True, out=y)
                else:
                    wino(x, u[c0:c1], first.b[c0 * 64:c1 * 64], (c1 - c0) * 64, relu=True, out=y)
                _conv.grouped_conv3x3_small(y, f["pf"][c0:c1], f["bf"][c0 * f["cmax"]:c1 * f["cmax"]], c1 - c0, out=z,
                                            out_groups=groups, out_group0=c0)
        else:
            y, _ = first(x)
            z = _conv.grouped_conv3x3_small(y, f["pf"], f["bf"], groups)
        rets = [dict() for _ in self.tasks]
        for g, (t, head) in enumerate(f["plan"]):
            rets[t][head] = z[:, g * f["cmax"]:g * f["cmax"] + f["ncls"][g]]
        return rets, x

    @torch.no_grad()
    def predict_by_custom_op(self, preds_dicts, test_cfg, device_only=False, records=0):
        hm, reg, height, dim, vel, rot = [], [], [], [], [], []
        for preds in preds_dicts:
            hm.append(preds["hm"])
            reg.append(preds["reg"])
            height.append(preds["height"])
            dim.append(preds["dim"])
            vel.append(preds["vel"] if self.with_velocity else preds["reg"])
            rot.append(preds["rot"])
        offsets = np.concatenate([[0], np.cumsum(self.num_classes)[:-1]]).astype(int).tolist()
        num_classes = offsets * len(preds_dicts)
        out = _cp.centerpoint_postprocess_device(
            hm, reg, height, dim, vel, rot, test_cfg["voxel_size"], test_cfg["point_cloud_range"],
            test_cfg["post_center_limit_range"], num_classes, test_cfg["down_ratio"], test_cfg["score_threshold"],
            test_cfg["nms"]["nms_iou_threshold"], test_cfg["nms"]["nms_pre_max_size"],
            test_cfg["nms"]["nms_post_max_size"], self.with_velocity, allow_batch=True,
            records=records if device_only else 0)
        if device_only:
            return out
        b, s, l, n = out
        counts = n.cpu().tolist()
        return [dict(box3d_lidar=b[i, :k], label_preds=l[i, :k], scores=s[i, :k]) for i, k in enumerate(counts)]


class CenterPoint(nn.Module):

    def __init__(self, voxelizer, voxel_encoder, middle_encoder, backbone, neck, bbox_head, test_cfg,
                 box_with_velocity=True):
        super().__init__()
        self.voxelizer = voxelizer
        self.voxel_encoder = voxel_encoder
        self.middle_encoder = middle_encoder
        self.backbone = backbone
        self.neck = neck
        self.bbox_head = bbox_head
        self.test_cfg = test_cfg
        self.box_with_velocity = box_with_velocity
        self.fuse_scatter = isinstance(middle_encoder, PointPillarsScatter) and isinstance(backbone, SecondBackbone)
        self.fuse_rows = isinstance(voxel_encoder, PillarFeatureNet) and isinstance(middle_encoder, PointPillarsScatter)

    def scatter(self, feats, coors, batch_size):
        if self.fuse_scatter:
            return self.middle_encoder.sparse(feats, coors, batch_size)
        return self.middle_encoder(feats, coors, batch_size)

    def invalidate(self):
        invalidate_derived(self)
        return self

    def set_amp(self, enabled: bool = True):
        for m in (self.backbone, self.bbox_head, self.middle_encoder):
            if hasattr(m, "amp"):
                m.amp = bool(enabled)
        if hasattr(self.backbone, "amp_out_f16"):
            self.backbone.amp_out_f16 = bool(enabled) and hasattr(self.neck, "amp_ok") and self.neck.amp_ok(None)
        return self

    def _pack(self, points):
        if isinstance(points, torch.Tensor):
            return points, None
        n = max(p.shape[0] for p in points)
        d = points[0].shape[1]
        out = torch.zeros((len(points), n, d), dtype=torch.float32, device=points[0].device)
        for i, p in enumerate(points):
            out[i, : p.shape[0]] = p
        lens = torch.tensor([p.shape[0] for p in points], dtype=torch.int32, device=points[0].device)
        return out, lens

    def extract_pillars(self, points, num_points=None, dense=True):
        if self.fuse_rows and isinstance(points, torch.Tensor) and points.dim() == 3:
            idx = self.voxelizer.index(points, num_points)
            if idx is not None:
                span, plist, coors, npv, nv = idx
                b, v = int(coors.shape[0]), int(coors.shape[1])
                coors = coors.view(b * v, 4)
                feats = self.voxel_encoder.forward_indexed(points, span, plist, coors)
                if feats is not None:
                    return self.middle_encoder(feats, coors, b) if dense else self.scatter(feats, coors, b)
        voxels, coors, npv, nv = self.voxelizer(points, num_points)
        b, v, p, d = voxels.shape
        voxels, coors, npv = voxels.view(b * v, p, d), coors.view(b * v, 4), npv.view(b * v)
        if not isinstance(self.middle_encoder, PointPillarsScatter) and \
                not getattr(self.middle_encoder, "accepts_padding_rows", False):
            keep = coors[:, 0] >= 0
            voxels, coors, npv = voxels[keep], coors[keep].contiguous(), npv[keep]
        feats = self.voxel_encoder(voxels, npv, coors)
        if dense:
            return self.middle_encoder(feats, coors, b)
        return self.scatter(feats, coors, b)

    def dense_forward(self, x):
        return self.neck(self.backbone(x))

    @torch.no_grad()
    def test_forward(self, points, device_only=False):
        import contextlib

        pts, lens = self._pack(points)
        checked = getattr(self.middle_encoder, "overflow_checked", None)
        take = getattr(self.middle_encoder, "take_overflow", None)
        for _attempt in range(2):
            with (checked() if (checked is not None and not device_only) else contextlib.nullcontext()):
                x = self.extract_pillars(pts, lens, dense=False)
            x = self.dense_forward(x)
            preds, _ = self.bbox_head(x, want_shared=False)
            out = self.bbox_head.predict_by_custom_op(preds, self.test_cfg, device_only=device_only)
            if device_only or take is None or not take():
                break
        return out

    forward = test_forward


NUSC_TASKS = [dict(num_class=1, class_names=["car"]), dict(num_class=2, class_names=["truck", "construction_vehicle"]),
              dict(num_class=2, class_names=["bus", "trailer"]), dict(num_class=1, class_names=["barrier"]),
              dict(num_class=2, class_names=["motorcycle", "bicycle"]),
              dict(num_class=2, class_names=["pedestrian", "traffic_cone"])]


def centerpoint_pillars_nuscenes(max_num_voxels=(30000, 60000)) -> CenterPoint:
    pcr, vs = [-51.2, -51.2, -5.0, 51.2, 51.2, 3.0], [0.2, 0.2, 8]
    test_cfg = dict(post_center_limit_range=[-61.2, -61.2, -10.0, 61.2, 61.2, 10.0], max_per_img=500,
                    nms=dict(nms_pre_max_size=1000, nms_post_max_size=83, nms_iou_threshold=0.2),
                    score_threshold=0.1, point_cloud_range=[-51.2, -51.2], down_ratio=4, voxel_size=[0.2, 0.2])
    return CenterPoint(
        voxelizer=HardVoxelizer(vs, pcr, 20, list(max_num_voxels)),
        voxel_encoder=PillarFeatureNet(5, (64, 64), False, 20, vs, pcr, legacy=False),
        middle_encoder=PointPillarsScatter(64, vs, pcr),
        backbone=SecondBackbone(64, (64, 128, 256), (3, 5, 5), (2, 2, 2)),
        neck=SecondFPN((64, 128, 256), (128, 128, 128), (0.5, 1, 2), use_conv_for_no_stride=True),
        bbox_head=CenterHead(384, NUSC_TASKS, dict(reg=(2, 2), height=(1, 2), dim=(3, 2), rot=(2, 2), vel=(2, 2))),
        test_cfg=test_cfg, box_with_velocity=True)


KITTI_TASKS = [dict(num_class=1, class_names=["Car"]), dict(num_class=2, class_names=["Cyclist", "Pedestrian"])]


def centerpoint_pillars_kitti(max_num_voxels=(12000, 40000)) -> CenterPoint:
    pcr, vs = [0.0, -39.68, -3.0, 69.12, 39.68, 1.0], [0.16, 0.16, 4]
    test_cfg = dict(post_center_limit_range=[-10.0, -50.0, -10.0, 80.0, 50.0, 10.0], max_per_img=500,
                    nms=dict(nms_pre_max_size=1000, nms_post_max_size=83, nms_iou_threshold=0.1),
                    score_threshold=0.1, point_cloud_range=pcr[:2], down_ratio=2, voxel_size=[0.16, 0.16])
    return CenterPoint(
        voxelizer=HardVoxelizer(vs, pcr, 100, list(max_num_voxels)),
        voxel_encoder=PillarFeatureNet(4, (64, 64), False, 100, vs, pcr, legacy=False),
        middle_encoder=PointPillarsScatter(64, vs, pcr),
        backbone=SecondBackbone(64, (64, 128, 256), (3, 5, 5), (1, 2, 2)),
        neck=SecondFPN((64, 128, 256), (128, 128, 128), (0.5, 1, 2), use_conv_for_no_stride=True),
        bbox_head=CenterHead(384, KITTI_TASKS, dict(reg=(2, 2), height=(1, 2), dim=(3, 2), rot=(2, 2))),
        test_cfg=test_cfg, box_with_velocity=False)


def centerpoint_voxels_nuscenes(max_num_voxels=(120000, 160000), point_cloud_range=None) -> CenterPoint:
    from .sparse import SparseResNet3D

    pcr = [-54.0, -54.0, -5.0, 54.0, 54.0, 3.0] if point_cloud_range is None else list(map(float, point_cloud_range))
    vs = [0.075, 0.075, 0.2]
    test_cfg = dict(post_center_limit_range=[-61.2, -61.2, -10.0, 61.2, 61.2, 10.0], max_per_img=500,
                    nms=dict(nms_pre_max_size=1000, nms_post_max_size=83, nms_iou_threshold=0.2),
                    score_threshold=0.1, point_cloud_range=pcr[:2], down_ratio=8, voxel_size=[0.075, 0.075])
    return CenterPoint(
        voxelizer=HardVoxelizer(vs, pcr, 10, list(max_num_voxels)),
        voxel_encoder=VoxelMean(5),
        middle_encoder=SparseResNet3D(5, vs, pcr),
        backbone=SecondBackbone(256, (128, 256), (5, 5), (1, 2)),
        neck=SecondFPN((128, 256), (256, 256), (1, 2), use_conv_for_no_stride=True),
        bbox_head=CenterHead(512, NUSC_TASKS, dict(reg=(2, 2), height=(1, 2), dim=(3, 2), rot=(2, 2), vel=(2, 2))),
        test_cfg=test_cfg, box_with_velocity=True)


def centerpoint_voxels_kitti(max_num_voxels=(12000, 40000)) -> CenterPoint:
    from .sparse import SparseResNet3D

    pcr, vs = [0.0, -39.68, -3.0, 69.12, 39.68, 1.0], [0.08, 0.08, 0.1]
    test_cfg = dict(post_center_limit_range=[-10.0, -50.0, -10.0, 80.0, 50.0, 10.0], max_per_img=500,
                    nms=dict(nms_pre_max_size=1000, nms_post_max_size=83, nms_iou_threshold=0.1),
                    score_threshold=0.1, point_cloud_range=pcr[:2], down_ratio=8, voxel_size=[0.08, 0.08])
    return CenterPoint(
        voxelizer=HardVoxelizer(vs, pcr, 100, list(max_num_voxels)),
        voxel_encoder=VoxelMean(4),
        middle_encoder=SparseResNet3D(4, vs, pcr),
        backbone=SecondBackbone(256, (128, 256), (5, 5), (1, 2)),
        neck=SecondFPN((128, 256), (256, 256), (1, 2), use_conv_for_no_stride=True),
        bbox_head=CenterHead(512, KITTI_TASKS, dict(reg=(2, 2), height=(1, 2), dim=(3, 2), rot=(2, 2))),
        test_cfg=test_cfg, box_with_velocity=False)


from .checkpoint import load_paddle_state_dict
```

### paddle3d_amd/csrc/conv3x3.hip

```cpp
#include "../../include/paddle3d_amd.h"
#include "common.hpp"


namespace pd3 {

typedef float cv_f32x16 __attribute__((ext_vector_type(16)));
typedef float cv_f32x4 __attribute__((ext_vector_type(4)));

constexpr int kCvCo = 64;
constexpr int kCvCi = 8;
constexpr int kCvK = kCvCi * 9;

template <int R, int WT, int S, int XB, bool FUSED = false>
__global__ __launch_bounds__(256) void conv3x3_mfma_kernel(const float* __restrict__ x,
                                                           const float* __restrict__ wp,
                                                           const float* __restrict__ bias,
                                                           float* __restrict__ out, int cin, int cout,
                                                           int h, int w, int wi, int wv, int relu, int ptiles,
                                                           const int* __restrict__ imap) {
  static_assert(R * WT == 128 || R * WT == 256, "tile must hold 128 or 256 pixels");
  constexpr int NB = R * WT / 128;
  constexpr int XR = (R - 1) * S + 3, XW = S * WT + 8;
  constexpr int XQ = XW / 4;
  constexpr int XPL = XR * XW;
  constexpr int XN4 = kCvCi * XR * XQ;
  constexpr int XPT = (XN4 + 255) / 256;
  constexpr int WN4 = kCvK * kCvCo / 4;
  constexpr int WPT = (WN4 + 255) / 256;
  constexpr int XSZ = kCvCi * XPL;
  constexpr int WSZ = kCvK * kCvCo;
  extern __shared__ __attribute__((aligned(16))) float cv_smem[];
  const int lane = lane_id(), wave = wave_id();
  const int tiles_x = (w + WT - 1) / WT, tiles_y = (h + R - 1) / R;
  const int nct = cout / kCvCo;
  const int xcd = blockIdx.x & 7, slot = blockIdx.x >> 3;
  const int ct = slot % nct, pt = (slot / nct) * 8 + xcd;
  if (pt >= ptiles) return;
  const int tx = pt % tiles_x, ty = (pt / tiles_x) % tiles_y, n = pt / (tiles_x * tiles_y);
  const int y0 = ty * R, x0 = tx * WT;
  const int kk = lane >> 5;
  int xb[NB];
#pragma unroll
  for (int t = 0; t < NB; ++t) {
    const int pj = (wave * NB + t) * 32 + (lane & 31);
    xb[t] = kk * XPL + (pj / WT) * S * XW + (pj % WT) * S + 3;
  }
  const int wb = XB * XSZ + kk * kCvCo + (lane & 31);
  cv_f32x16 acc[2][NB];
#pragma unroll
  for (int m = 0; m < 2; ++m)
#pragma unroll
    for (int t = 0; t < NB; ++t)
#pragma unroll
      for (int i = 0; i < 16; ++i) acc[m][t][i] = 0.f;
  const int chunks = cin / kCvCi;
  const int64_t plane = (int64_t)h * w;
  const int hi = S * h;
  const int64_t iplane = (int64_t)hi * wi;
  const float* xin = x + (int64_t)n * cin * iplane;
  int gofs[XPT], ldst[XPT];
  unsigned live = 0;
  constexpr int NCELL = XR * XW, CPT = (NCELL + 255) / 256;
  int cpid[FUSED ? CPT : 1], cdst[FUSED ? CPT : 1];
  if (FUSED) {
    const int* im = imap + (int64_t)n * iplane;
#pragma unroll
    for (int i = 0; i < CPT; ++i) {
      const int e = (int)threadIdx.x + i * 256;
      const int r = e / XW, c = e - r * XW;
      const int gy = S * y0 - 1 + r, gx = S * x0 - 4 + c;
      const bool ok = e < NCELL && gy >= 0 && gy < hi && gx >= 0 && gx < wi;
      cpid[i] = ok ? im[(int64_t)gy * wi + gx] : -1;
      cdst[i] = min(e, NCELL - 1);
    }
    for (int e = threadIdx.x; e < XB * XSZ / 4; e += 256)
      reinterpret_cast<cv_f32x4*>(cv_smem)[e] = (cv_f32x4){0.f, 0.f, 0.f, 0.f};
    __syncthreads();
  }
#pragma unroll
  for (int i = 0; i < XPT; ++i) {
    const int e = min((int)threadIdx.x + i * 256, XN4 - 1);
    const int ci = e / (XR * XQ), rem = e - ci * (XR * XQ);
    const int r = rem / XQ, c4 = rem - r * XQ;
    const int gy = S * y0 - 1 + r, gx = S * x0 - 4 + c4 * 4;
    const bool ok = gy >= 0 && gy < hi && gx >= 0 && gx < wi;
    gofs[i] = ok ? (int)(ci * iplane + (int64_t)gy * wi + gx) : 0;
    live |= ok ? (1u << i) : 0u;
    ldst[i] = e * 4;
  }
  int wofs[WPT];
#pragma unroll
  for (int i = 0; i < WPT; ++i) wofs[i] = min((int)threadIdx.x + i * 256, WN4 - 1);
  const cv_f32x4* wsrc = reinterpret_cast<const cv_f32x4*>(wp) + (int64_t)ct * chunks * WN4;
  cv_f32x4 xr[FUSED ? 2 * CPT : XPT], wr[WPT];

#define CV_FETCH(cc)                                                                     \
  {                                                                                      \
    if (FUSED) {                                                                         \
      _Pragma("unroll") for (int i = 0; i < CPT; ++i)                                    \
        if (cpid[i] >= 0) {                                                              \
          const float* f_ = x + (int64_t)cpid[i] * cin + (cc) * kCvCi;                   \
          xr[2 * i] = *reinterpret_cast<const cv_f32x4*>(f_);                            \
          xr[2 * i + 1] = *reinterpret_cast<const cv_f32x4*>(f_ + 4);                    \
        }                                                                                \
    } else {                                                                             \
      const float* xc_ = xin + (int64_t)(cc) * kCvCi * iplane;                           \
      _Pragma("unroll") for (int i = 0; i < XPT; ++i)                                    \
          xr[i] = *reinterpret_cast<const cv_f32x4*>(xc_ + gofs[i]);                     \
    }                                                                                    \
    const cv_f32x4* wc_ = wsrc + (int64_t)(cc) * WN4;                                      \
    _Pragma("unroll") for (int i = 0; i < WPT; ++i) wr[i] = wc_[wofs[i]];                \
  }
#define CV_STASH(buf)                                                                    \
  {                                                                                      \
    float* xd_ = cv_smem + (XB == 2 ? (buf) : 0) * XSZ;                                  \
    float* wd_ = cv_smem + XB * XSZ + (buf) * WSZ;                                       \
    if (FUSED) {                                                                         \
      _Pragma("unroll") for (int i = 0; i < CPT; ++i)                                    \
        if (cpid[i] >= 0) {                                                              \
          float* d_ = xd_ + cdst[i];                                                     \
          _Pragma("unroll") for (int k_ = 0; k_ < 4; ++k_) {                             \
            d_[k_ * XPL] = xr[2 * i][k_];                                                \
            d_[(4 + k_) * XPL] = xr[2 * i + 1][k_];                                      \
          }                                                                              \
        }                                                                                \
    } else {                                                                             \
      _Pragma("unroll") for (int i = 0; i < XPT; ++i) {                                  \
        const bool on_ = (live >> i) & 1u;                                               \
        const cv_f32x4 z_ = {0.f, 0.f, 0.f, 0.f};                                        \
        *reinterpret_cast<cv_f32x4*>(xd_ + ldst[i]) = on_ ? xr[i] : z_;                  \
      }                                                                                  \
    }                                                                                    \
    _Pragma("unroll") for (int i = 0; i < WPT; ++i)                                      \
        *reinterpret_cast<cv_f32x4*>(wd_ + wofs[i] * 4) = wr[i];                         \
  }

  CV_FETCH(0)
  CV_STASH(0)
  __syncthreads();
  for (int cc = 0; cc < chunks; ++cc) {
    const int nx = min(cc + 1, chunks - 1);
    CV_FETCH(nx)
    __builtin_amdgcn_sched_barrier(0);
    const float* Xs = cv_smem + (XB == 2 ? (cc & 1) : 0) * XSZ;
    const float* Ws = cv_smem + (cc & 1) * WSZ + wb;
    float a0_[3], a1_[3], b_[3][NB];
#define CV_OPERANDS(s_, slot_)                                                           \
  {                                                                                      \
    const int cp_ = (s_) / 9, tap_ = (s_) % 9;                                           \
    const int xo_ = 2 * cp_ * XPL + (tap_ / 3) * XW + (tap_ % 3);                        \
    a0_[slot_] = Ws[(s_) * 2 * kCvCo];                                                   \
    a1_[slot_] = Ws[(s_) * 2 * kCvCo + 32];                                              \
    _Pragma("unroll") for (int t = 0; t < NB; ++t) b_[slot_][t] = Xs[xb[t] + xo_];       \
  }
    CV_OPERANDS(0, 0)
    CV_OPERANDS(1, 1)
#pragma unroll
    for (int s = 0; s < kCvK / 2; ++s) {
      if (s + 2 < kCvK / 2) CV_OPERANDS(s + 2, (s + 2) % 3)
      __builtin_amdgcn_sched_barrier(0);
#pragma unroll
      for (int t = 0; t < NB; ++t) {
        acc[0][t] = __builtin_amdgcn_mfma_f32_32x32x2f32(a0_[s % 3], b_[s % 3][t], acc[0][t], 0, 0, 0);
        acc[1][t] = __builtin_amdgcn_mfma_f32_32x32x2f32(a1_[s % 3], b_[s % 3][t], acc[1][t], 0, 0, 0);
      }
      __builtin_amdgcn_sched_barrier(0);
    }
#undef CV_OPERANDS
    __builtin_amdgcn_sched_barrier(0);
    if (XB == 1) __syncthreads();
    CV_STASH((cc + 1) & 1)
    __syncthreads();
  }
#undef CV_FETCH
#undef CV_STASH
  float bv[2][16];
#pragma unroll
  for (int m = 0; m < 2; ++m)
#pragma unroll
    for (int reg = 0; reg < 16; ++reg) bv[m][reg] = 0.f;
  if (bias) {
#pragma unroll
    for (int m = 0; m < 2; ++m)
#pragma unroll
      for (int reg = 0; reg < 16; ++reg)
        bv[m][reg] = bias[ct * kCvCo + m * 32 + (reg & 3) + 8 * (reg >> 2) + 4 * kk];
  }
#pragma unroll
  for (int t = 0; t < NB; ++t) {
    const int pj = (wave * NB + t) * 32 + (lane & 31);
    if (y0 + pj / WT >= h || x0 + pj % WT >= w) continue;
    float* obase = out + (int64_t)n * cout * plane + (int64_t)(y0 + pj / WT) * w + x0 + (pj % WT);
#pragma unroll
    for (int m = 0; m < 2; ++m)
#pragma unroll
      for (int reg = 0; reg < 16; ++reg) {
        const int co = ct * kCvCo + m * 32 + (reg & 3) + 8 * (reg >> 2) + 4 * kk;
        float v = acc[m][t][reg] + bv[m][reg];
        if (relu) v = fmaxf(v, 0.f);
        obase[(int64_t)co * plane] = (x0 + pj % WT < wv) ? v : 0.f;
      }
  }
}

template <int R, int WT, int S, int XB = 2, bool FUSED = false>
static int launch_conv3x3(int64_t tiles, hipStream_t s, const float* x, const float* wp, const float* bias,
                          float* out, int cin, int cout, int h, int w, int wi, int wv, int relu,
                          const int* imap = nullptr) {
  constexpr size_t lds = (size_t)(XB * kCvCi * ((R - 1) * S + 3) * (S * WT + 8) + 2 * kCvK * kCvCo) * sizeof(float);
  hipError_t e = pd3_max_dynamic_lds(reinterpret_cast<const void*>(conv3x3_mfma_kernel<R, WT, S, XB, FUSED>), (int)lds);
  if (e != hipSuccess) return (int)e;
  const int64_t nwg = (tiles + 7) / 8 * 8 * (cout / kCvCo);
  if (nwg >= (int64_t)1 << 31) return PD3_EUNSUPPORTED;
  conv3x3_mfma_kernel<R, WT, S, XB, FUSED><<<(unsigned)nwg, 256, lds, s>>>(x, wp, bias, out, cin, cout, h, w, wi, wv,
                                                                           relu, (int)tiles, imap);
  return launch_status();
}

constexpr int kGcCi = 4;
constexpr int kGcR = 8, kGcW = 128;
constexpr int kGcXR = kGcR + 2, kGcXW = kGcW + 8;

template <int CO>
__global__ __launch_bounds__(256) void grouped_conv3x3_small_kernel(const float* __restrict__ x,
                                                                    const float* __restrict__ wg,
                                                                    const float* __restrict__ bias,
                                                                    float* __restrict__ out, int groups,
                                                                    int cg, int h, int w, int out_groups,
                                                                    int out_group0) {
  __shared__ __attribute__((aligned(16))) float Xs[kGcCi * kGcXR * kGcXW];
  const int tiles_x = (w + kGcW - 1) / kGcW, tiles_y = (h + kGcR - 1) / kGcR;
  const int pt = blockIdx.x;
  const int tx = pt % tiles_x, ty = (pt / tiles_x) % tiles_y, n = pt / (tiles_x * tiles_y);
  const int g = blockIdx.y;
  const int y0 = ty * kGcR, x0 = tx * kGcW;
  const int tr = threadIdx.x >> 5, tc = (threadIdx.x & 31) * 4;
  const int64_t plane = (int64_t)h * w;
  const float* xin = x + ((int64_t)n * groups + g) * cg * plane;
  const float* wgp = wg + (int64_t)g * cg * CO * 9;
  float acc[CO][4];
#pragma unroll
  for (int c = 0; c < CO; ++c)
#pragma unroll
    for (int p = 0; p < 4; ++p) acc[c][p] = 0.f;
  constexpr int XQ = kGcXW / 4, XN4 = kGcCi * kGcXR * XQ;
  constexpr int XPT = (XN4 + 255) / 256;
  int gofs[XPT];
  unsigned live = 0;
#pragma unroll
  for (int i = 0; i < XPT; ++i) {
    const int e = min((int)threadIdx.x + i * 256, XN4 - 1);
    const int ci = e / (kGcXR * XQ), rem = e - ci * (kGcXR * XQ);
    const int r = rem / XQ, c4 = rem - r * XQ;
    const int gy = y0 - 1 + r, gx = x0 - 4 + c4 * 4;
    const bool ok = gy >= 0 && gy < h && gx >= 0 && gx < w;
    gofs[i] = ok ? (int)(ci * plane + (int64_t)gy * w + gx) : 0;
    live |= ok ? 1u << i : 0u;
  }
  cv_f32x4 xr[XPT];
#pragma unroll
  for (int i = 0; i < XPT; ++i) xr[i] = *reinterpret_cast<const cv_f32x4*>(xin + gofs[i]);
  for (int c0 = 0; c0 < cg; c0 += kGcCi) {
    __syncthreads();
#pragma unroll
    for (int i = 0; i < XPT; ++i) {
      const int e = min((int)threadIdx.x + i * 256, XN4 - 1);
      const cv_f32x4 z = {0.f, 0.f, 0.f, 0.f};
      *reinterpret_cast<cv_f32x4*>(Xs + e * 4) = ((live >> i) & 1u) ? xr[i] : z;
    }
    if (c0 + kGcCi < cg) {
      const float* xn = xin + (int64_t)(c0 + kGcCi) * plane;
#pragma unroll
      for (int i = 0; i < XPT; ++i) xr[i] = *reinterpret_cast<const cv_f32x4*>(xn + gofs[i]);
    }
    __syncthreads();
#pragma unroll
    for (int ci = 0; ci < kGcCi; ++ci) {
      const float* wc = wgp + (int64_t)(c0 + ci) * CO * 9;
#pragma unroll
      for (int ky = 0; ky < 3; ++ky) {
        const float* row = Xs + (ci * kGcXR + tr + ky) * kGcXW + tc;
        const cv_f32x4 mid = *reinterpret_cast<const cv_f32x4*>(row + 4);
        float in[6];
        in[1] = mid[0];
        in[2] = mid[1];
        in[3] = mid[2];
        in[4] = mid[3];
        in[0] = row[3];
        in[5] = row[8];
#pragma unroll
        for (int c = 0; c < CO; ++c)
#pragma unroll
          for (int kx = 0; kx < 3; ++kx) {
            const float wv = wc[c * 9 + ky * 3 + kx];
#pragma unroll
            for (int p = 0; p < 4; ++p) acc[c][p] = __builtin_fmaf(wv, in[p + kx], acc[c][p]);
          }
      }
    }
  }
#pragma unroll
  for (int c = 0; c < CO; ++c) {
    const float b = bias ? bias[g * CO + c] : 0.f;
    cv_f32x4 v = {acc[c][0] + b, acc[c][1] + b, acc[c][2] + b, acc[c][3] + b};
    if (y0 + tr < h && x0 + tc < w)
      *reinterpret_cast<cv_f32x4*>(out + ((int64_t)n * out_groups * CO + (out_group0 + g) * CO + c) * plane +
                                   (int64_t)(y0 + tr) * w + x0 + tc) = v;
  }
}

}

using namespace pd3;

extern "C" int pd3_conv3x3_bias_relu(const float* x, const float* w_packed, const float* bias,
                                     int batch, int cin, int cout, int h, int w, int w_valid, int stride, int relu,
                                     float* out, int out_w, void* stream) {
  if (!x || !w_packed || !out || batch <= 0 || cin <= 0 || cout <= 0 || h <= 0 || w <= 0 || w_valid <= 0 ||
      w_valid > w || out_w <= 0)
    return PD3_EINVAL;
  if (stride != 1 && stride != 2) return PD3_EUNSUPPORTED;
  if (cin % kCvCi != 0 || cout % kCvCo != 0 || h % stride != 0 || w_valid % stride != 0) return PD3_EUNSUPPORTED;
  if (w % 4 != 0 || out_w % 4 != 0 || out_w < w_valid / stride) return PD3_EUNSUPPORTED;
  if (reinterpret_cast<uintptr_t>(w_packed) % 16 != 0 || reinterpret_cast<uintptr_t>(x) % 16 != 0)
    return PD3_EINVAL;
  if ((int64_t)cin * h * w >= (int64_t)1 << 31) return PD3_EUNSUPPORTED;
  hipStream_t s = static_cast<hipStream_t>(stream);
  const int ho = h / stride, wo = out_w, wv = w_valid / stride;
#define PD3_CV(R, WT, S)                                                                                     \
  launch_conv3x3<R, WT, S>((int64_t)batch * ceil_div(ho, R) * ceil_div(wo, WT), s, x, w_packed, bias, out, cin, \
                           cout, ho, wo, w, wv, relu)
  if (stride == 1) {
    if (wo % 128 == 0 && ho % 2 == 0) return PD3_CV(2, 128, 1);
    if (wo % 64 == 0 && ho % 4 == 0) return PD3_CV(4, 64, 1);
    if (wo % 128 == 0) return PD3_CV(1, 128, 1);
    if (wo % 64 == 0 && ho % 2 == 0) return PD3_CV(2, 64, 1);
    return PD3_CV(4, 32, 1);
  } else {
    if (wo % 128 == 0 && ho % 2 == 0)
      return launch_conv3x3<2, 128, 2, 1>((int64_t)batch * ho * wo / 256, s, x, w_packed, bias, out, cin, cout, ho, wo,
                                          w, wv, relu);
    if (wo % 64 == 0 && ho % 2 == 0) return PD3_CV(2, 64, 2);
    return PD3_CV(4, 32, 2);
  }
#undef PD3_CV
}

extern "C" int pd3_scatter_conv3x3_bias_relu(const float* feats, const int32_t* imap, const float* w_packed,
                                             const float* bias, int batch, int cin, int cout, int ny, int nx,
                                             int stride, int relu, float* out, int out_w, void* stream) {
  if (!feats || !imap || !w_packed || !out || batch <= 0 || cin <= 0 || cout <= 0 || ny <= 0 || nx <= 0 || out_w <= 0)
    return PD3_EINVAL;
  if (stride != 2) return PD3_EUNSUPPORTED;
  if (cin % kCvCi != 0 || cout % kCvCo != 0 || ny % 2 != 0 || nx % 2 != 0 || out_w % 4 != 0 || out_w < nx / 2)
    return PD3_EUNSUPPORTED;
  if (reinterpret_cast<uintptr_t>(w_packed) % 16 != 0 || reinterpret_cast<uintptr_t>(feats) % 16 != 0 || cin % 4 != 0)
    return PD3_EINVAL;
  if ((int64_t)ny * nx >= (int64_t)1 << 31) return PD3_EUNSUPPORTED;
  hipStream_t s = static_cast<hipStream_t>(stream);
  const int ho = ny / 2, wo = out_w, wv = nx / 2;
  const int* im = reinterpret_cast<const int*>(imap);
  if (wo % 128 == 0 && ho % 2 == 0)
    return launch_conv3x3<2, 128, 2, 1, true>((int64_t)batch * ho * wo / 256, s, feats, w_packed, bias, out, cin, cout, ho,
                                              wo, nx, wv, relu, im);
  if (wo % 64 == 0 && ho % 2 == 0)
    return launch_conv3x3<2, 64, 2, 2, true>((int64_t)batch * ceil_div(ho, 2) * ceil_div(wo, 64), s, feats, w_packed, bias,
                                             out, cin, cout, ho, wo, nx, wv, relu, im);
  return launch_conv3x3<4, 32, 2, 2, true>((int64_t)batch * ceil_div(ho, 4) * ceil_div(wo, 32), s, feats, w_packed, bias,
                                           out, cin, cout, ho, wo, nx, wv, relu, im);
}

static int grouped_small_launch(const float* x, const float* w_grouped, const float* bias, int batch, int groups,
                                int cin_per_group, int cout_per_group, int h, int w, float* out, int out_groups,
                                int out_group0, void* stream) {
  if (!x || !w_grouped || !out || batch <= 0 || groups <= 0 || cin_per_group <= 0 || h <= 0 || w <= 0 ||
      out_group0 < 0 || out_group0 + groups > out_groups)
    return PD3_EINVAL;
  if (cout_per_group < 1 || cout_per_group > 4 || cin_per_group % kGcCi != 0 || w % 4 != 0)
    return PD3_EUNSUPPORTED;
  if (reinterpret_cast<uintptr_t>(x) % 16 != 0 || reinterpret_cast<uintptr_t>(out) % 16 != 0) return PD3_EINVAL;
  hipStream_t s = static_cast<hipStream_t>(stream);
  dim3 grid((unsigned)((int64_t)batch * ceil_div(h, kGcR) * ceil_div(w, kGcW)), (unsigned)groups);
#define PD3_GC(CO)                                                                                                  \
  grouped_conv3x3_small_kernel<CO><<<grid, 256, 0, s>>>(x, w_grouped, bias, out, groups, cin_per_group, h, w,        \
                                                        out_groups, out_group0)
  switch (cout_per_group) {
    case 1: PD3_GC(1); break;
    case 2: PD3_GC(2); break;
    case 3: PD3_GC(3); break;
    default: PD3_GC(4); break;
  }
#undef PD3_GC
  return launch_status();
}

extern "C" int pd3_grouped_conv3x3_small(const float* x, const float* w_grouped, const float* bias, int batch,
                                         int groups, int cin_per_group, int cout_per_group, int h, int w,
                                         float* out, void* stream) {
  return grouped_small_launch(x, w_grouped, bias, batch, groups, cin_per_group, cout_per_group, h, w, out, groups, 0,
                              stream);
}

extern "C" int pd3_grouped_conv3x3_small_slice(const float* x, const float* w_grouped, const float* bias, int batch,
                                               int groups, int cin_per_group, int cout_per_group, int h, int w,
                                               float* out, int out_groups, int out_group0, void* stream) {
  return grouped_small_launch(x, w_grouped, bias, batch, groups, cin_per_group, cout_per_group, h, w, out, out_groups,
                              out_group0, stream);
}
```

### paddle3d_amd/csrc/conv_winograd43.hpp

```cpp
#pragma once
#include "../../include/paddle3d_amd.h"
#include "common.hpp"

#include <type_traits>

namespace pd3 {

typedef float w4_f32x4 __attribute__((ext_vector_type(4)));
typedef float w4_f32x2 __attribute__((ext_vector_type(2)));

constexpr int kW4Ci = 4;
constexpr int kW4TR = 2, kW4TC = 16;
constexpr int kW4Cs = 36;
constexpr int kW4RawR = 4 * kW4TR + 2;
constexpr int kW4RawW = 4 * kW4TC + 8;
constexpr int kW4RawPl = kW4RawR * kW4RawW;
constexpr int kW4Vsz = kW4TR * kW4Ci * kW4TC * kW4Cs;
constexpr int kW4RawSz = kW4Ci * kW4RawPl;
constexpr int kW4XN4 = kW4RawSz / 4;

__device__ __forceinline__ void w4_in(const float d0, const float d1, const float d2, const float d3, const float d4,
                                      const float d5, float (&t)[6]) {
  const float a = __builtin_fmaf(-4.f, d2, d4), b = __builtin_fmaf(-4.f, d1, d3);
  const float c = d4 - d2, e = d3 - d1;
  t[0] = __builtin_fmaf(4.f, d0, __builtin_fmaf(-5.f, d2, d4));
  t[1] = a + b;
  t[2] = a - b;
  t[3] = __builtin_fmaf(2.f, e, c);
  t[4] = __builtin_fmaf(-2.f, e, c);
  t[5] = __builtin_fmaf(4.f, d1, __builtin_fmaf(-5.f, d3, d5));
}

__device__ __forceinline__ void w4_out(const float m0, const float m1, const float m2, const float m3, const float m4,
                                       const float m5, float (&s)[4]) {
  const float p = m1 + m2, q = m1 - m2, r = m3 + m4, u = m3 - m4;
  s[0] = m0 + p + r;
  s[1] = __builtin_fmaf(2.f, u, q);
  s[2] = __builtin_fmaf(4.f, r, p);
  s[3] = __builtin_fmaf(8.f, u, q) + m5;
}

__device__ __forceinline__ float w4_swap_pair(float v) {
  return __builtin_bit_cast(float, __builtin_amdgcn_mov_dpp(__builtin_bit_cast(int, v), 0xB1, 0xf, 0xf, true));
}

__device__ __forceinline__ void w4_lds_barrier() { asm volatile("s_waitcnt lgkmcnt(0)\n\ts_barrier" ::: "memory"); }

__device__ inline void w4_pair_transform(const float (&rv)[3][6], const int hf, float* v) {
  float lo[3][3], hi[3][3];
#pragma unroll
  for (int b = 0; b < 3; ++b) {
    float t[6];
    w4_in(rv[b][0], rv[b][1], rv[b][2], rv[b][3], rv[b][4], rv[b][5], t);
#pragma unroll
    for (int a = 0; a < 3; ++a) {
      lo[a][b] = t[a];
      hi[a][b] = t[3 + a];
    }
  }
#pragma unroll
  for (int a = 0; a < 3; ++a) {
    float f[3], l[3];
#pragma unroll
    for (int b = 0; b < 3; ++b) {
      const float ph = w4_swap_pair(hi[a][b]), pl = w4_swap_pair(lo[a][b]);
      f[b] = hf ? ph : lo[a][b];
      l[b] = hf ? hi[a][b] : pl;
    }
    float o[6];
    w4_in(f[0], f[1], f[2], l[0], l[1], l[2], o);
    *reinterpret_cast<w4_f32x2*>(v + a * 6 + 0) = (w4_f32x2){o[0], o[1]};
    *reinterpret_cast<w4_f32x2*>(v + a * 6 + 2) = (w4_f32x2){o[2], o[3]};
    *reinterpret_cast<w4_f32x2*>(v + a * 6 + 4) = (w4_f32x2){o[4], o[5]};
  }
}

struct w4_no_hook {
  __device__ __forceinline__ void operator()() const {}
};
template <int N, int HOOK = -1, class UA, class VP, class F = w4_no_hook>
__device__ __forceinline__ void w4_mfma_stream(w4_f32x4 (&acc)[36], const UA& ua, const VP& vptr, const F& hook = F()) {
  constexpr bool kRing = !std::is_array<UA>::value;
  w4_f32x4 a[3], b[3];
  auto load = [&](const int g) {
    if constexpr (kRing) a[g % 3] = *reinterpret_cast<const w4_f32x4*>(ua(g));
    b[g % 3] = *reinterpret_cast<const w4_f32x4*>(vptr(g));
  };
  load(0);
  load(1);
#pragma unroll
  for (int g = 0; g < N; ++g) {
    if (g + 2 < N) load(g + 2);
    __builtin_amdgcn_sched_barrier(0);
#pragma unroll
    for (int j = 0; j < 4; ++j) {
      float av;
      if constexpr (kRing) av = a[g % 3][j];
      else av = ua[g][j];
      acc[(g % 9) * 4 + j] = __builtin_amdgcn_mfma_f32_16x16x4f32(av, b[g % 3][j], acc[(g % 9) * 4 + j], 0, 0, 0);
    }
    __builtin_amdgcn_sched_barrier(0);
    if (g == HOOK) {
      hook();
      __builtin_amdgcn_sched_barrier(0);
    }
  }
}

__device__ __forceinline__ void w4_output_step(const w4_f32x4 (&acc)[36], const w4_f32x4 bv, const int n, const int cout,
                                               const int co0, const int oy, const int ox, const int h, const int w,
                                               const int wv, const int relu, const int64_t plane,
                                               float* __restrict__ out) {
#pragma unroll
  for (int r = 0; r < 4; ++r) {
    float s[4][6];
#pragma unroll
    for (int j = 0; j < 6; ++j) {
      float c4[4];
      w4_out(acc[0 * 6 + j][r], acc[1 * 6 + j][r], acc[2 * 6 + j][r], acc[3 * 6 + j][r], acc[4 * 6 + j][r],
             acc[5 * 6 + j][r], c4);
#pragma unroll
      for (int k = 0; k < 4; ++k) s[k][j] = c4[k];
    }
    float* o = out + ((int64_t)n * cout + co0 + r) * plane + (int64_t)oy * w + ox;
#pragma unroll
    for (int k = 0; k < 4; ++k) {
      float y4[4];
      w4_out(s[k][0], s[k][1], s[k][2], s[k][3], s[k][4], s[k][5], y4);
#pragma unroll
      for (int j = 0; j < 4; ++j) {
        y4[j] += bv[r];
        if (relu) y4[j] = fmaxf(y4[j], 0.f);
        if (ox + j >= wv) y4[j] = 0.f;
      }
      if (oy + k < h && ox < w)
        __builtin_nontemporal_store((w4_f32x4){y4[0], y4[1], y4[2], y4[3]},
                                    reinterpret_cast<w4_f32x4*>(o + (int64_t)k * w));
    }
  }
}

struct w4_tile {
  int cg, pt, n, y0, x0;
};
__device__ __forceinline__ w4_tile w4_decode_block(const int groups, const int h, const int w) {
  const int tiles_x = (w + 4 * kW4TC - 1) / (4 * kW4TC), tiles_y = (h + 4 * kW4TR - 1) / (4 * kW4TR);
  const int xcd = blockIdx.x & 7, slot = blockIdx.x >> 3;
  const int pt = (slot / groups) * 8 + xcd;
  const int tx = pt % tiles_x, ty = (pt / tiles_x) % tiles_y;
  return {slot % groups, pt, pt / (tiles_x * tiles_y), ty * 4 * kW4TR, tx * 4 * kW4TC};
}

inline int w4_check_args(const void* in, const void* u, const void* out, int batch, int cin, int cout, int h, int w,
                         int w_valid, int cin_multiple, int cout_multiple) {
  if (!in || !u || !out || batch <= 0 || cin <= 0 || cout <= 0 || h <= 0 || w <= 0 || w_valid <= 0 || w_valid > w)
    return PD3_EINVAL;
  if (cin % cin_multiple != 0 || cout % cout_multiple != 0 || w % 4 != 0) return PD3_EUNSUPPORTED;
  if (reinterpret_cast<uintptr_t>(in) % 16 != 0 || reinterpret_cast<uintptr_t>(u) % 16 != 0 ||
      reinterpret_cast<uintptr_t>(out) % 16 != 0)
    return PD3_EINVAL;
  return PD3_OK;
}

inline int64_t w4_grid(int batch, int h, int w, int groups, int64_t* ptiles) {
  *ptiles = (int64_t)batch * ceil_div(h, 4 * kW4TR) * ceil_div(w, 4 * kW4TC);
  return (*ptiles + 7) / 8 * 8 * groups;
}

}
```

### paddle3d_amd/csrc/conv_winograd43_pp.hip

```cpp
#include "../../include/paddle3d_amd.h"
#include "common.hpp"
#include "conv_winograd43_pp.hpp"

#include <type_traits>

namespace pd3 {

constexpr int kPpRawR = 6;
constexpr int kPpRawPl = kPpRawR * kW4RawW;
constexpr int kPpRawSz = kPpCi * kPpRawPl;
constexpr int kPpXPT = (2 * kPpRawPl / 4 + 63) / 64;

__global__ __launch_bounds__(512, 1) void conv3x3_winograd43_pp_kernel(const float* __restrict__ x,
                                                                       const float* __restrict__ ulane,
                                                                       const float* __restrict__ bias,
                                                                       float* __restrict__ out, int cin, int cout, int h,
                                                                       int w, int wv, int relu, int ptiles,
                                                                       long long* __restrict__ dbg) {
  constexpr int CO = 64;
  long long t_tr = 0, t_mu = 0, t_ba = 0, t_all = dbg ? clock64() : 0;
  extern __shared__ __attribute__((aligned(16))) float smem[];
  const int lane = lane_id(), wave = __builtin_amdgcn_readfirstlane(wave_id());
  const int grp = wave >> 2, cb = wave & 3;
  const int gt = cb * 64 + lane;
  float* Us = smem;
  float* Raw = smem + kPpUsz + grp * (kPpRawSz + kPpVsz);
  float* Vs = Raw + kPpRawSz;
  const w4_tile tl = w4_decode_block(cout / CO, h, w);
  if (tl.pt >= ptiles) return;
  const int ct = tl.cg, n = tl.n, y0 = tl.y0, x0 = tl.x0;
  const int slots = cin / kPpCi;
  const int64_t plane = (int64_t)h * w;
  const float* xin = x + (int64_t)n * cin * plane;

  constexpr int kWvN4 = 2 * kPpRawPl / 4;
  unsigned gofs[kPpXPT];
#pragma unroll
  for (int i = 0; i < kPpXPT; ++i) {
    const int e = min(lane + i * 64, kWvN4 - 1);
    const int cl = e / (kPpRawR * (kW4RawW / 4)), rem = e - cl * (kPpRawR * (kW4RawW / 4));
    const int r = rem / (kW4RawW / 4), c4 = rem - r * (kW4RawW / 4);
    const int gy = y0 + 4 * grp - 1 + r, gx = x0 - 4 + c4 * 4;
    const bool ok = gy >= 0 && gy < h && gx >= 0 && gx < w;
    gofs[i] = ok ? (unsigned)(4 * ((2 * cb + cl) * plane + (int64_t)gy * w + gx)) : 0x7ffffff0u;
  }
  const int pidx = gt >> 1, hf = gt & 1;
  const int pci = pidx >> 4, ptile = pidx & 15;
  const int rsrc = pci * kPpRawPl + 4 * ptile + 3 + 3 * hf;
  const int vdst = (pci * kW4TC + ptile) * kW4Cs + 18 * hf;
  const int bbase = pp_bbase(lane);
  const float* uct = ulane + (int64_t)ct * slots * kPpUsz;

  w4_f32x4 acc[36];
#pragma unroll
  for (int c = 0; c < 36; ++c) acc[c] = (w4_f32x4){0.f, 0.f, 0.f, 0.f};

  auto fetch_x = [&](int s) {
#pragma unroll
    for (int i = 0; i < kPpXPT; ++i) {
      if (lane + i * 64 < kWvN4)
        pp_dma(xin + (int64_t)s * kPpCi * plane, (unsigned)(kPpCi * plane * 4), Raw + 2 * cb * kPpRawPl + i * 256, gofs[i],
               0);
    }
  };
  auto fetch_u = [&](int s, int hh) { pp_fetch_u(uct, (unsigned)((int64_t)slots * kPpUsz * 4), Us, cb, lane, s, hh); };
  float rv[3][6];
  auto read_rows = [&]() {
#pragma unroll
    for (int b = 0; b < 3; ++b) {
      const float* d = Raw + rsrc + b;
#pragma unroll
      for (int r = 0; r < 6; ++r) rv[b][r] = d[r * kW4RawW];
    }
  };
  auto transform = [&](int sn, auto&& after_fetch) {
    fetch_x(sn);
    after_fetch();
    __builtin_amdgcn_sched_barrier(0);
    __builtin_amdgcn_sched_barrier(0);
    w4_pair_transform(rv, hf, Vs + vdst);
  };
  auto vptr = [&](int g) { return pp_vptr(Vs, bbase, g); };
  auto uptr = [&](int g) { return pp_uptr(Us, cb, lane, g); };
  w4_f32x4 ua[18];
  auto next_rows = [&]() {
    __builtin_amdgcn_s_waitcnt(0x0f70);
    read_rows();
  };
  auto multiply_ring = [&]() { w4_mfma_stream<18, 15>(acc, uptr, vptr, next_rows); };
  auto multiply_regs = [&]() { w4_mfma_stream<18, 16>(acc, ua, vptr, next_rows); };

  fetch_x(0);
  if (grp == 0) {
    fetch_u(0, 0);
    fetch_u(0, 1);
  }
  __builtin_amdgcn_s_waitcnt(0x0f70);
  read_rows();
  w4_lds_barrier();
  auto sync = [&]() {
    const long long c1 = dbg ? clock64() : 0;
    w4_lds_barrier();
    if (dbg) t_ba += clock64() - c1;
  };
  auto run = [&](auto is_g0) {
    constexpr bool G0 = decltype(is_g0)::value;
    if (!G0) sync();
    for (int s = 0; s < slots; ++s) {
      {
        const long long c0 = dbg ? clock64() : 0;
        const int sn = min(s + 1, slots - 1);
        if (G0) {
          if (s > 0) {
            fetch_u(s, 0);
            fetch_u(s, 1);
          }
          transform(sn, [&]() {});
          __builtin_amdgcn_s_waitcnt(0x0f70 | 4);
        } else {
          transform(sn, [&]() {
#pragma unroll
            for (int g = 0; g < 9; ++g) ua[g] = *reinterpret_cast<const w4_f32x4*>(uptr(g));
          });
#pragma unroll
          for (int g = 9; g < 18; ++g) ua[g] = *reinterpret_cast<const w4_f32x4*>(uptr(g));
        }
        if (dbg) t_tr += clock64() - c0;
      }
      sync();
      {
        const long long c0 = dbg ? clock64() : 0;
        if (G0) multiply_ring();
        else multiply_regs();
        if (dbg) t_mu += clock64() - c0;
      }
      sync();
    }
    if (G0) sync();
  };
  if (grp == 0) run(std::true_type{});
  else run(std::false_type{});
  if (dbg && blockIdx.x == 8 && lane == 0) {
    dbg[wave * 4 + 0] = t_tr;
    dbg[wave * 4 + 1] = t_mu;
    dbg[wave * 4 + 2] = t_ba;
    dbg[wave * 4 + 3] = (clock64() - t_all) | ((long long)__builtin_amdgcn_s_getreg(2308) << 56);
  }

  w4_f32x4 bv = {0.f, 0.f, 0.f, 0.f};
  const int co0 = ct * CO + cb * 16 + 4 * (lane >> 4);
  if (bias) {
#pragma unroll
    for (int r = 0; r < 4; ++r) bv[r] = bias[co0 + r];
  }
  w4_output_step(acc, bv, n, cout, co0, y0 + 4 * grp, x0 + 4 * (lane & 15), h, w, wv, relu, plane, out);
}

}

using namespace pd3;

static int launch_wino43_pp(const float* x, const float* u_lane, const float* bias, int batch, int cin, int cout, int h,
                            int w, int w_valid, int relu, float* out, hipStream_t s, long long* dbg = nullptr) {
  constexpr size_t lds = ((size_t)kPpUsz + 2 * (kPpRawSz + kPpVsz)) * sizeof(float);
  const void* fn = reinterpret_cast<const void*>(conv3x3_winograd43_pp_kernel);
  hipError_t e = pd3_max_dynamic_lds(fn, (int)lds);
  if (e != hipSuccess) return (int)e;
  int64_t ptiles;
  const int64_t nwg = w4_grid(batch, h, w, cout / 64, &ptiles);
  if (nwg >= (int64_t)1 << 31) return PD3_EUNSUPPORTED;
  conv3x3_winograd43_pp_kernel<<<(unsigned)nwg, 512, lds, s>>>(x, u_lane, bias, out, cin, cout, h, w, w_valid, relu,
                                                               (int)ptiles, dbg);
  return launch_status();
}

static int check_wino43_pp(const float* x, const float* u_lane, const float* out, int batch, int cin, int cout, int h,
                           int w, int w_valid) {
  const int st = w4_check_args(x, u_lane, out, batch, cin, cout, h, w, w_valid, kPpCi, 64);
  if (st != PD3_OK) return st;
  if ((int64_t)kPpCi * h * w >= (int64_t)1 << 29) return PD3_EUNSUPPORTED;
  if ((int64_t)(cin / kPpCi) * kPpUsz >= (int64_t)1 << 29) return PD3_EUNSUPPORTED;
  return PD3_OK;
}

extern "C" int pd3_conv3x3_winograd43_pp_bias_relu(const float* x, const float* u_lane, const float* bias, int batch,
                                                   int cin, int cout, int h, int w, int w_valid, int relu, float* out,
                                                   void* stream) {
  const int st = check_wino43_pp(x, u_lane, out, batch, cin, cout, h, w, w_valid);
  if (st != PD3_OK) return st;
  return launch_wino43_pp(x, u_lane, bias, batch, cin, cout, h, w, w_valid, relu, out, static_cast<hipStream_t>(stream));
}

extern "C" int pd3_conv3x3_winograd43_pp_trace(const float* x, const float* u_lane, const float* bias, int batch, int cin,
                                               int cout, int h, int w, int relu, float* out, long long* dbg,
                                               void* stream) {
  const int st = check_wino43_pp(x, u_lane, out, batch, cin, cout, h, w, w);
  if (st != PD3_OK || !dbg) return st != PD3_OK ? st : PD3_EINVAL;
  return launch_wino43_pp(x, u_lane, bias, batch, cin, cout, h, w, w, relu, out, static_cast<hipStream_t>(stream), dbg);
}
```

### paddle3d_amd/csrc/conv_winograd43_pp.hpp

```cpp
#pragma once
#include "conv_winograd43.hpp"

namespace pd3 {

constexpr int kPpKT = 2;
constexpr int kPpCi = kPpKT * kW4Ci;
constexpr int kPpVsz = kPpCi * kW4TC * kW4Cs;
constexpr int kPpUHalf = 9 * 64 * 4;
constexpr int kPpUsz = kPpKT * 4 * kPpUHalf;

__device__ __forceinline__ void pp_dma(const float* base, unsigned bytes, float* lds, unsigned voff, unsigned soff) {
  const __amdgpu_buffer_rsrc_t r = __builtin_amdgcn_make_buffer_rsrc(const_cast<float*>(base), 0, (int)bytes, 0x00020000);
  __builtin_amdgcn_raw_ptr_buffer_load_lds(r, (__attribute__((address_space(3))) void*)lds, 16, (int)voff, (int)soff, 0, 0);
}

__device__ __forceinline__ int pp_bbase(int lane) { return ((lane >> 4) * kW4TC + (lane & 15)) * kW4Cs; }
__device__ __forceinline__ const float* pp_vptr(const float* V, int bbase, int g) {
  return V + (g / 9) * (kW4Ci * kW4TC * kW4Cs) + bbase + (g % 9) * 4;
}
__device__ __forceinline__ const float* pp_uptr(const float* Us, int cb, int lane, int g) {
  return Us + (((g / 9) * 4 + cb) * 9 + (g % 9)) * 256 + lane * 4;
}

__device__ __forceinline__ void pp_fetch_u(const float* u, unsigned bytes, float* Us, int cb, int lane, int slot, int hh) {
  const int blk = (hh * 4 + cb) * kPpUHalf;
  const unsigned so = __builtin_amdgcn_readfirstlane((unsigned)((slot * kPpUsz + blk) * 4));
#pragma unroll
  for (int q = 0; q < 9; ++q) pp_dma(u, bytes, Us + blk + q * 256, lane * 16, so + (unsigned)(q * 1024));
}

}
```

### paddle3d_amd/csrc/conv_winograd43_ppv.hip

```cpp
#include "../../include/paddle3d_amd.h"
#include "common.hpp"
#include "conv_winograd43_pp.hpp"

#include <type_traits>

namespace pd3 {

constexpr int kPvMaxBlocks = 18;

__global__ __launch_bounds__(128) void w43_input_transform_kernel(const float* __restrict__ x, int cin, int h, int w,
                                                                  int wv, int tiles_x, int tiles_y, int slots,
                                                                  float* __restrict__ v) {
  __shared__ __attribute__((aligned(16))) float blk[kPpVsz];
  const int g = blockIdx.x & 1, s = (blockIdx.x >> 1) % slots, pt = (blockIdx.x >> 1) / slots;
  const int tx = pt % tiles_x, ty = (pt / tiles_x) % tiles_y, n = pt / (tiles_x * tiles_y);
  const int ci = threadIdx.x >> 4, tile = threadIdx.x & 15;
  const int y0 = ty * 4 * kW4TR + 4 * g - 1, x0 = tx * 4 * kW4TC + 4 * tile - 1;
  const float* xin = x + ((int64_t)n * cin + s * kPpCi + ci) * (int64_t)h * w;
  float d[6][6];
#pragma unroll
  for (int r = 0; r < 6; ++r)
#pragma unroll
    for (int c = 0; c < 6; ++c) {
      const int gy = y0 + r, gx = x0 + c;
      d[r][c] = gy >= 0 && gy < h && gx >= 0 && gx < wv ? xin[(int64_t)gy * w + gx] : 0.f;
    }
  float t[6][6];
#pragma unroll
  for (int c = 0; c < 6; ++c) {
    float o[6];
    w4_in(d[0][c], d[1][c], d[2][c], d[3][c], d[4][c], d[5][c], o);
#pragma unroll
    for (int a = 0; a < 6; ++a) t[a][c] = o[a];
  }
  float* dst = blk + (ci * kW4TC + tile) * kW4Cs;
#pragma unroll
  for (int a = 0; a < 6; ++a) {
    float o[6];
    w4_in(t[a][0], t[a][1], t[a][2], t[a][3], t[a][4], t[a][5], o);
#pragma unroll
    for (int c = 0; c < 6; ++c) dst[a * 6 + c] = o[c];
  }
  __syncthreads();
  w4_f32x4* out4 = reinterpret_cast<w4_f32x4*>(v + (int64_t)blockIdx.x * kPpVsz);
  const w4_f32x4* b4 = reinterpret_cast<const w4_f32x4*>(blk);
#pragma unroll
  for (int i = 0; i < kPpVsz / 4 / 128; ++i) out4[threadIdx.x + i * 128] = b4[threadIdx.x + i * 128];
}

__global__ __launch_bounds__(512, 1) void conv3x3_winograd43_ppv_kernel(const float* __restrict__ vpre,
                                                                        const float* __restrict__ ulane,
                                                                        const float* __restrict__ bias,
                                                                        float* __restrict__ out, int cin, int cout, int h,
                                                                        int w, int wv, int relu, int ptiles, int ipw) {
  constexpr int CO = 64;
  extern __shared__ __attribute__((aligned(16))) float smem[];
  const int lane = lane_id(), wave = __builtin_amdgcn_readfirstlane(wave_id());
  const int grp = wave >> 2, cb = wave & 3;
  float* Us = smem;
  float* Vs = smem + kPpUsz + grp * 2 * kPpVsz;
  float* bias_s = smem + kPpUsz + 4 * kPpVsz;
  const w4_tile tl = w4_decode_block((cout / CO) / ipw, h, w);
  if (tl.pt >= ptiles) return;
  const int ct0 = tl.cg * ipw, pt = tl.pt, n = tl.n, y0 = tl.y0, x0 = tl.x0;
  const int slots = cin / kPpCi;
  const bool whole_tiles = h % (4 * kW4TR) == 0 && w % (4 * kW4TC) == 0;
  const int64_t plane = (int64_t)h * w;
  const int bbase = pp_bbase(lane);
  const float* vpt = vpre + (int64_t)pt * slots * 2 * kPpVsz;
  const unsigned vbytes = (unsigned)(slots * 2 * kPpVsz * 4);
  const int nv = cb < 2 ? 5 : 4;

  w4_f32x4 acc[36];
#pragma unroll
  for (int c = 0; c < 36; ++c) acc[c] = (w4_f32x4){0.f, 0.f, 0.f, 0.f};

  auto fetch_v = [&](int s) {
    float* dst = Vs + (s & 1) * kPpVsz;
    const unsigned so = (unsigned)((s * 2 + grp) * kPpVsz * 4);
#pragma unroll
    for (int i = 0; i < 5; ++i) {
      const int piece = cb + 4 * i;
      if (i < 4 || cb < 2) pp_dma(vpt, vbytes, dst + piece * 256, lane * 16, so + piece * 1024);
    }
  };
  const unsigned ubytes = (unsigned)((int64_t)(cout / CO) * slots * kPpUsz * 4);
  int ct = ct0;
  auto fetch_u = [&](int c, int s, int hh) {
    pp_fetch_u(ulane, ubytes, Us, cb, lane, c * slots + s, hh);
  };
  auto uptr = [&](int g) { return pp_uptr(Us, cb, lane, g); };
  w4_f32x4 ua[18];
  auto multiply_ring = [&](const float* V) { w4_mfma_stream<18>(acc, uptr, [&](int g) { return pp_vptr(V, bbase, g); }); };
  auto multiply_regs = [&](const float* V) { w4_mfma_stream<18>(acc, ua, [&](int g) { return pp_vptr(V, bbase, g); }); };

  for (int t = threadIdx.x; t < ipw * CO; t += 512) bias_s[t] = bias ? bias[ct0 * CO + t] : 0.f;
  fetch_v(0);
  if (grp == 0) {
    fetch_u(ct0, 0, 0);
    fetch_u(ct0, 0, 1);
  }
  __builtin_amdgcn_s_waitcnt(0x0f70);
  w4_lds_barrier();
  auto run = [&](auto is_g0) {
    constexpr bool G0 = decltype(is_g0)::value;
    if (!G0) w4_lds_barrier();
    for (int s = 0; s < slots; ++s) {
      {
        if (G0 && s > 0) {
          fetch_u(ct, s, 0);
          fetch_u(ct, s, 1);
        }
        const bool more = s + 1 < slots;
        if (more) fetch_v(s + 1);
        if (!G0) {
#pragma unroll
          for (int g = 0; g < 18; ++g) ua[g] = *reinterpret_cast<const w4_f32x4*>(uptr(g));
        }
        if (s == 0 && ct != ct0) {
        } else if (!more) {
          __builtin_amdgcn_s_waitcnt(0x0f70);
        } else if (nv == 5) {
          __builtin_amdgcn_s_waitcnt(0x0f70 | 5);
        } else {
          __builtin_amdgcn_s_waitcnt(0x0f70 | 4);
        }
      }
      w4_lds_barrier();
      {
        const float* V = Vs + (s & 1) * kPpVsz;
        if (G0) multiply_ring(V);
        else multiply_regs(V);
      }
      w4_lds_barrier();
    }
    if (G0) w4_lds_barrier();
  };
  auto blocks = [&](auto is_g0) {
  for (int it = 0; it < ipw; ++it) {
  ct = ct0 + it;
  run(is_g0);
  if (it + 1 < ipw) {
    fetch_v(0);
    if (grp == 0) {
      fetch_u(ct + 1, 0, 0);
      fetch_u(ct + 1, 0, 1);
    }
  }

  const int co0 = ct * CO + cb * 16 + 4 * (lane >> 4);
  const w4_f32x4 b4 = *reinterpret_cast<const w4_f32x4*>(bias_s + it * CO + cb * 16 + 4 * (lane >> 4));
  w4_output_step(acc, b4, n, cout, co0, y0 + 4 * grp, x0 + 4 * (lane & 15), h, w, wv, relu, plane, out);
  if (it + 1 < ipw) {
#pragma unroll
    for (int c = 0; c < 36; ++c) acc[c] = (w4_f32x4){0.f, 0.f, 0.f, 0.f};
    if (whole_tiles) __builtin_amdgcn_s_waitcnt(0x0f70 | (16 & 15) | ((16 >> 4) << 14));
    else __builtin_amdgcn_s_waitcnt(0x0f70);
    w4_lds_barrier();
  }
  }
  };
  if (grp == 0) blocks(std::true_type{});
  else blocks(std::false_type{});
}

}

using namespace pd3;

extern "C" size_t pd3_winograd43_input_transform_floats(int batch, int cin, int h, int w) {
  if (batch <= 0 || cin <= 0 || h <= 0 || w <= 0 || cin % kPpCi != 0) return 0;
  int64_t ptiles;
  w4_grid(batch, h, w, 1, &ptiles);
  return (size_t)(ptiles * (cin / kPpCi) * 2 * kPpVsz);
}

extern "C" int pd3_winograd43_input_transform(const float* x, int batch, int cin, int h, int w, int w_valid, float* v,
                                              void* stream) {
  if (!x || !v || batch <= 0 || cin <= 0 || h <= 0 || w <= 0 || w_valid <= 0 || w_valid > w) return PD3_EINVAL;
  if (cin % kPpCi != 0) return PD3_EUNSUPPORTED;
  if (reinterpret_cast<uintptr_t>(v) % 16 != 0) return PD3_EINVAL;
  const int tiles_x = (int)ceil_div(w, 4 * kW4TC), tiles_y = (int)ceil_div(h, 4 * kW4TR);
  const int64_t blocks = (int64_t)batch * tiles_x * tiles_y * (cin / kPpCi) * 2;
  if (blocks >= (int64_t)1 << 31) return PD3_EUNSUPPORTED;
  w43_input_transform_kernel<<<(unsigned)blocks, 128, 0, static_cast<hipStream_t>(stream)>>>(x, cin, h, w, w_valid, tiles_x,
                                                                                           tiles_y, cin / kPpCi, v);
  return launch_status();
}

extern "C" int pd3_conv3x3_winograd43_ppv_bias_relu(const float* v_pre, const float* u_lane, const float* bias, int batch,
                                                    int cin, int cout, int h, int w, int w_valid, int relu, float* out,
                                                    void* stream) {
  const int st = w4_check_args(v_pre, u_lane, out, batch, cin, cout, h, w, w_valid, kPpCi, 64);
  if (st != PD3_OK) return st;
  if ((int64_t)(cout / 64) * (cin / kPpCi) * kPpUsz >= (int64_t)1 << 29 ||
      (int64_t)(cin / kPpCi) * 2 * kPpVsz >= (int64_t)1 << 29)
    return PD3_EUNSUPPORTED;
  const int nct = cout / 64;
  int64_t ptiles;
  const int64_t ptiles8 = w4_grid(batch, h, w, 1, &ptiles);
  int ipw = 1;
  for (int d = 2; d <= kPvMaxBlocks; ++d)
    if (nct % d == 0 && ptiles8 * (nct / d) >= 6 * 256) ipw = d;
  const size_t lds = ((size_t)kPpUsz + 4 * kPpVsz + kPvMaxBlocks * 64) * sizeof(float);
  const void* fn = reinterpret_cast<const void*>(conv3x3_winograd43_ppv_kernel);
  const hipError_t e = pd3_max_dynamic_lds(fn, (int)lds);
  if (e != hipSuccess) return (int)e;
  const int64_t nwg = ptiles8 * (nct / ipw);
  if (nwg >= (int64_t)1 << 31) return PD3_EUNSUPPORTED;
  conv3x3_winograd43_ppv_kernel<<<(unsigned)nwg, 512, lds, static_cast<hipStream_t>(stream)>>>(
      v_pre, u_lane, bias, out, cin, cout, h, w, w_valid, relu, (int)ptiles, ipw);
  return launch_status();
}
```

### paddle3d_amd/ops/conv.py

```python
from __future__ import annotations

import torch

from ._common import check, lib, ptr, require_gpu, stream_ptr

__all__ = ["pack_conv3x3_weight", "conv3x3_bias_relu", "supported", "pitch4", "pack_grouped_weight", "grouped_conv3x3_small",
           "grouped_small_supported", "winograd_supported", "pack_winograd_weight", "conv3x3_winograd_bias_relu",
           "patch_mode", "patch_supported", "pack_patch_weight", "patch_conv_bias_relu",
           "patch_x3_supported", "pack_patch_weight_x3", "patch_conv_x3_bias_relu", "split_bf16x3",
           "conv3x3_s2_x3_supported", "pack_conv3x3_s2_x3_weight", "conv3x3_s2_x3_bias_relu",
           "winograd43_input_transform", "conv3x3_winograd43_ppv_bias_relu",
           "winograd43_supported", "winograd43_tile", "pack_winograd43_weight", "conv3x3_winograd43_bias_relu",
           "WINOGRAD43_PP_MIN_CIN", "winograd43_pp_supported", "pack_winograd43_lane_weight", "conv3x3_winograd43_pp_bias_relu",
           "f16_supported", "f16_tile", "pack_conv3x3_f16_weight", "conv3x3_f16_bias_relu", "to_f16_nhwc",
           "pack_grouped_weight_f16", "grouped_conv3x3_small_f16", "conv3x3_f16_bias_relu_dual",
           "s2_f16_supported", "conv3x3_s2_f16_bias_relu", "scatter_conv_s2_f16_supported",
           "scatter_conv3x3_s2_f16_bias_relu", "scatter_conv_sparse_supported", "scatter_conv3x3_sparse"]


def pitch4(w: int) -> int:
    return (int(w) + 3) // 4 * 4


def supported(cin: int, cout: int, h: int, w: int, stride: int = 1) -> bool:
    return stride in (1, 2) and cin % 8 == 0 and cout % 64 == 0 and h % stride == 0 and w % stride == 0


def pack_conv3x3_weight(weight: torch.Tensor) -> torch.Tensor:
    cout, cin = weight.shape[:2]
    assert weight.shape[2:] == (3, 3) and cout % 64 == 0 and cin % 8 == 0
    w = weight.reshape(cout // 64, 64, cin // 8, 4, 2, 9).permute(0, 2, 3, 5, 4, 1)
    return w.reshape(cout // 64, cin // 8, 72, 64).contiguous()


def conv3x3_bias_relu(x: torch.Tensor, w_packed: torch.Tensor, bias, cout: int, relu: bool = True,
                      stride: int = 1, out: torch.Tensor | None = None, w_valid: int | None = None) -> torch.Tensor:
    xx = require_gpu(x, "conv3x3_bias_relu")
    n, cin, h, w = xx.shape
    wv = w if w_valid is None else int(w_valid)
    if out is None:
        out = torch.empty((n, cout, h // stride, pitch4(wv // stride)), dtype=torch.float32, device=xx.device)
    check(lib().pd3_conv3x3_bias_relu(ptr(xx), ptr(w_packed), ptr(bias), n, cin, cout, h, w, wv, int(stride),
                                      int(bool(relu)), ptr(out), int(out.shape[3]), stream_ptr(xx.device)),
          "conv3x3_bias_relu")
    return out


def scatter_conv_supported(cin: int, cout: int, ny: int, nx: int, stride: int) -> bool:
    return stride == 2 and cin % 8 == 0 and cout % 64 == 0 and ny % 2 == 0 and nx % 2 == 0


def scatter_conv3x3_bias_relu(canvas, w_packed: torch.Tensor, bias, cout: int, relu: bool = True) -> torch.Tensor:
    f, inv = canvas.features, canvas.inv
    n, cin, ny, nx = canvas.shape
    wo = pitch4(nx // 2)
    out = torch.empty((n, cout, ny // 2, wo), dtype=torch.float32, device=f.device)
    check(lib().pd3_scatter_conv3x3_bias_relu(ptr(f), ptr(inv), ptr(w_packed), ptr(bias), n, cin, cout, ny, nx, 2,
                                              int(bool(relu)), ptr(out), wo, stream_ptr(f.device)),
          "scatter_conv3x3_bias_relu")
    return out


def scatter_conv_sparse_supported(cin: int, cout: int, ny: int, nx: int, stride: int) -> bool:
    ho, wo = (ny - 1) // stride + 1, (nx - 1) // stride + 1
    return stride == 2 and cin % 16 == 0 and cout in (64, 128) and wo % 4 == 0 and (ho * wo) % 4 == 0


def scatter_conv3x3_sparse(canvas, weight: torch.Tensor, bias: torch.Tensor, packed=None, relu: bool = True):
    from . import sparse_conv3d as sp
    from ._common import workspace

    f, inv = canvas.features, canvas.inv
    n, cin, ny, nx = canvas.shape
    cout = int(weight.shape[0])
    ho, wo = (ny - 1) // 2 + 1, (nx - 1) // 2 + 1
    cap = n * ho * wo
    dev = f.device
    L = lib()
    nbr = torch.empty((cap, 9), dtype=torch.int32, device=dev)
    out_cell = torch.empty((cap,), dtype=torch.int32, device=dev)
    cell_row = torch.empty((n, ho * wo), dtype=torch.int32, device=dev)
    n_out = torch.empty((1,), dtype=torch.int32, device=dev)
    ws = workspace(L.pd3_pillar_conv_rulebook_workspace(n, ny, nx, 2), dev)
    order = torch.empty((int(L.pd3_sparse_tile_order_entries(cap)),), dtype=torch.int32, device=dev)
    check(L.pd3_pillar_conv_rulebook(ptr(inv), n, ny, nx, 2, ptr(nbr), ptr(out_cell), ptr(cell_row), ptr(n_out), cap,
                                     ptr(order), ptr(ws), ws.numel(), stream_ptr(dev)), "pillar_conv_rulebook")
    idx = sp.SparseIndices(None, nbr, cap, (1, ho, wo), 9, order, n_out)
    if packed is None:
        packed = sp.pack_weight_bf16x3(weight.permute(2, 3, 1, 0).reshape(1, 3, 3, cin, cout).contiguous())
    rows = sp.features_bf16x3(f, idx, packed, cin, cout, bias, None, None, None, relu)
    fill = torch.relu(bias) if relu else bias
    out = torch.empty((n, cout, ho, wo), dtype=torch.float32, device=dev)
    check(L.pd3_rows_to_dense_fill(ptr(rows), ptr(cell_row), ptr(fill.contiguous()), n, cout, ho, wo, ptr(out),
                                   stream_ptr(dev)), "rows_to_dense_fill")
    return out, packed


def winograd_supported(cin: int, cout: int, h: int, w: int) -> bool:
    return cin % 8 == 0 and cout % 32 == 0 and w % 4 == 0


def pack_winograd_weight(weight: torch.Tensor) -> torch.Tensor:
    cout, cin = weight.shape[:2]
    assert weight.shape[2:] == (3, 3) and cout % 32 == 0 and cin % 8 == 0
    g = torch.tensor([[1.0, 0.0, 0.0], [0.5, 0.5, 0.5], [0.5, -0.5, 0.5], [0.0, 0.0, 1.0]], dtype=torch.float64,
                     device=weight.device)
    u = torch.einsum("ij,ocjk,lk->ocil", g, weight.double(), g).float()
    u = u.reshape(cout // 32, 2, 16, cin // 8, 8, 16).permute(0, 3, 1, 4, 2, 5)
    return u.contiguous()


def conv3x3_winograd_bias_relu(x: torch.Tensor, u_packed: torch.Tensor, bias, cout: int, relu: bool = True,
                               out: torch.Tensor | None = None) -> torch.Tensor:
    xx = require_gpu(x, "conv3x3_winograd_bias_relu")
    n, cin, h, w = xx.shape
    if out is None:
        out = torch.empty((n, cout, h, w), dtype=torch.float32, device=xx.device)
    check(lib().pd3_conv3x3_winograd_bias_relu(ptr(xx), ptr(u_packed), ptr(bias), n, cin, cout, h, w,
                                               int(bool(relu)), ptr(out), stream_ptr(xx.device)),
          "conv3x3_winograd_bias_relu")
    return out


def winograd43_supported(cin: int, cout: int, h: int, w: int) -> bool:
    return cin % 4 == 0 and cout % 32 == 0


def winograd43_tile(cout: int) -> int:
    return 64 if cout % 64 == 0 else 32


def _winograd43_u(weight: torch.Tensor) -> torch.Tensor:
    g = torch.tensor([[1 / 4, 0, 0], [-1 / 6, -1 / 6, -1 / 6], [-1 / 6, 1 / 6, -1 / 6], [1 / 24, 1 / 12, 1 / 6],
                      [1 / 24, -1 / 12, 1 / 6], [0, 0, 1]], dtype=torch.float64, device=weight.device)
    return torch.einsum("ij,ocjk,lk->ocil", g, weight.double(), g).float()


def pack_winograd43_weight(weight: torch.Tensor, tile: int | None = None) -> torch.Tensor:
    cout, cin = weight.shape[:2]
    t = winograd43_tile(cout) if tile is None else tile
    assert weight.shape[2:] == (3, 3) and cout % t == 0 and cin % 4 == 0 and t in (32, 64)
    u = _winograd43_u(weight).reshape(cout // t, t // 16, 16, cin // 4, 4, 36).permute(0, 3, 1, 4, 2, 5)
    return u.contiguous()


def conv3x3_winograd43_bias_relu(x: torch.Tensor, u_packed: torch.Tensor, bias, cout: int, relu: bool = True,
                                 out: torch.Tensor | None = None, w_valid: int | None = None) -> torch.Tensor:
    xx = require_gpu(x, "conv3x3_winograd43_bias_relu")
    n, cin, h, w = xx.shape
    tile = 16 * u_packed.shape[2]
    if out is None:
        out = torch.empty((n, cout, h, w), dtype=torch.float32, device=xx.device)
    check(lib().pd3_conv3x3_winograd43_bias_relu(ptr(xx), ptr(u_packed), ptr(bias), n, cin, cout, h, w,
                                                 w if w_valid is None else int(w_valid), int(bool(relu)), ptr(out),
                                                 tile, stream_ptr(xx.device)),
          "conv3x3_winograd43_bias_relu")
    return out


def patch_mode(weight: torch.Tensor, stride: int, transpose: bool):
    k = weight.shape[2]
    if weight.shape[2] != weight.shape[3] or k != stride:
        return None
    if k == 1:
        return 1
    if k == 2:
        return 2 if transpose else 0
    if k == 4 and transpose:
        return 3
    return None


def patch_supported(mode: int, cin: int, cout: int, h: int, w: int) -> bool:
    if mode == 0:
        return h % 4 == 0 and w % 4 == 0 and (cin * 4) % 16 == 0 and cout % 64 == 0
    if (h * w) % 4 or cin % 16:
        return False
    return {1: cout >= 1, 2: (cout * 4) % 64 == 0, 3: (cout * 16) % 64 == 0}.get(mode, False)


def pack_patch_weight(weight: torch.Tensor, mode: int, transpose: bool) -> torch.Tensor:
    if mode == 0:
        a = weight.reshape(weight.shape[0], -1)
    elif mode == 1:
        a = weight[:, :, 0, 0].t() if transpose else weight[:, :, 0, 0]
        if a.shape[0] % 64:
            a = torch.cat([a, a.new_zeros(64 - a.shape[0] % 64, a.shape[1])], 0)
    else:
        a = weight.permute(1, 2, 3, 0).reshape(-1, weight.shape[0])
    m, k = a.shape
    assert m % 64 == 0 and k % 16 == 0
    return a.reshape(m // 64, 64, k // 16, 16).permute(0, 2, 3, 1).contiguous()


def patch_conv_bias_relu(x: torch.Tensor, w_packed: torch.Tensor, bias, mode: int, cout: int, out: torch.Tensor,
                         channel_offset: int = 0, relu: bool = True, w_valid: int | None = None) -> torch.Tensor:
    xx = require_gpu(x, "patch_conv_bias_relu")
    n, cin, h, w = xx.shape
    check(lib().pd3_patch_conv_bias_relu(ptr(xx), ptr(w_packed), ptr(bias), int(mode), n, cin, cout, h, w,
                                         w if w_valid is None else int(w_valid), int(bool(relu)), ptr(out),
                                         out.shape[1], int(channel_offset), stream_ptr(xx.device)),
          "patch_conv_bias_relu")
    return out


PATCH_BF16X3 = True


def patch_x3_supported(mode: int, cin: int, cout: int, h: int, w: int, batch: int = 1, ctot: int | None = None) -> bool:
    if mode == 0:
        ok, out_px = cin % 16 == 0 and cout % 128 == 0 and h % 2 == 0 and w % 64 == 0, (h // 2) * (w // 2)
    elif mode == 1:
        ok, out_px = cin % 32 == 0 and cout % 128 == 0 and (h * w) % 4 == 0, h * w
    elif mode == 2:
        ok, out_px = cin % 32 == 0 and cout % 64 == 0 and (h * w) % 4 == 0, 4 * h * w
    else:
        return False
    if not ok or cout > 1024:
        return False
    ctot = cout if ctot is None else int(ctot)
    steps = 2 * (cin // 16) if mode == 0 else cin // 32
    tiles = 2 * (cout // 64) if mode == 2 else cout // 128
    ptiles = batch * -(-min(out_px, h * w) // 256)
    return (batch * cin * h * w * 4 < 0x7ffffff0 and batch * ctot * out_px * 4 < 0x7ffffff0
            and tiles * steps * 32768 < 0x7ffffff0 and ptiles < 1 << 28)


def split_bf16x3(a: torch.Tensor) -> torch.Tensor:
    a = a.float()
    hi = a.bfloat16()
    r1 = a - hi.float()
    mid = r1.bfloat16()
    lo = (r1 - mid.float()).bfloat16()
    return torch.stack([hi, mid, lo])


def pack_patch_weight_x3(weight: torch.Tensor, mode: int, transpose: bool) -> torch.Tensor:
    w = weight.detach().float()
    if mode == 0:
        cout, cin = int(w.shape[0]), int(w.shape[1])
        a = w.reshape(cout // 128, 128, cin // 16, 16, 2, 2).permute(0, 4, 2, 1, 3, 5)
        a = a.reshape(cout // 128, 2 * (cin // 16), 128, 32)
    elif mode == 1:
        m = w[:, :, 0, 0].t() if transpose else w[:, :, 0, 0]
        cout, cin = int(m.shape[0]), int(m.shape[1])
        a = m.reshape(cout // 128, 128, cin // 32, 32).permute(0, 2, 1, 3)
    elif mode == 2:
        cin, cout = int(w.shape[0]), int(w.shape[1])
        a = w.reshape(cin // 32, 32, cout // 64, 64, 2, 2).permute(4, 2, 0, 5, 3, 1)
        a = a.reshape(2 * (cout // 64), cin // 32, 128, 32)
    else:
        raise ValueError(f"pack_patch_weight_x3: mode {mode}")
    pc = split_bf16x3(a.contiguous()).permute(1, 2, 0, 3, 4)
    pc = torch.nn.functional.pad(pc, (0, 8)).reshape(pc.shape[0], pc.shape[1], 3 * 128 * 40)
    return torch.nn.functional.pad(pc, (0, 16384 - 3 * 128 * 40)).contiguous()


def patch_conv_x3_bias_relu(x: torch.Tensor, w_packed: torch.Tensor, bias, mode: int, cout: int, out: torch.Tensor,
                            channel_offset: int = 0, relu: bool = True, w_valid: int | None = None) -> torch.Tensor:
    xx = require_gpu(x, "patch_conv_x3_bias_relu")
    n, cin, h, w = xx.shape
    check(lib().pd3_patch_conv_x3_bias_relu(ptr(xx), ptr(w_packed), ptr(bias), int(mode), n, cin, cout, h, w,
                                            w if w_valid is None else int(w_valid), int(bool(relu)), ptr(out),
                                            out.shape[1], int(channel_offset), stream_ptr(xx.device)),
          "patch_conv_x3_bias_relu")
    return out


S2_BF16X3 = True


def conv3x3_s2_x3_supported(cin: int, cout: int, h: int, w: int, batch: int = 1) -> bool:
    return (cin % 16 == 0 and cout % 128 == 0 and cout <= 1024 and h % 2 == 0 and w % 2 == 0
            and batch * max(cin, cout) * h * pitch4(w) * 4 < 0x7ffffff0)


def pack_conv3x3_s2_x3_weight(weight: torch.Tensor) -> torch.Tensor:
    w = weight.detach().float()
    cout, cin = int(w.shape[0]), int(w.shape[1])
    a = w.reshape(cout // 128, 128, cin // 16, 16, 3, 3).permute(0, 2, 4, 1, 5, 3)
    a = a.reshape(cout // 128, (cin // 16) * 3, 128, 48)
    pc = split_bf16x3(a.contiguous()).permute(1, 2, 0, 3, 4)
    pc = torch.nn.functional.pad(pc, (0, 8)).reshape(pc.shape[0], pc.shape[1], 3 * 128 * 56)
    return torch.nn.functional.pad(pc, (0, 24576 - 3 * 128 * 56)).contiguous()


def conv3x3_s2_x3_bias_relu(x: torch.Tensor, w_packed: torch.Tensor, bias, cout: int, relu: bool = True,
                            w_valid: int | None = None) -> torch.Tensor:
    xx = require_gpu(x, "conv3x3_s2_x3_bias_relu")
    n, cin, h, w = xx.shape
    wv = w if w_valid is None else int(w_valid)
    out = torch.empty((n, cout, h // 2, pitch4(wv // 2)), dtype=torch.float32, device=xx.device)
    check(lib().pd3_conv3x3_s2_x3_bias_relu(ptr(xx), ptr(w_packed), ptr(bias), n, cin, cout, h, w, wv, int(bool(relu)),
                                            ptr(out), int(out.shape[3]), stream_ptr(xx.device)),
          "conv3x3_s2_x3_bias_relu")
    return out


WINOGRAD43_PPV_MIN_BLOCKS = 8


def winograd43_input_transform(x: torch.Tensor, w_valid: int | None = None, out: torch.Tensor | None = None) -> torch.Tensor:
    xx = require_gpu(x, "winograd43_input_transform")
    n, cin, h, w = xx.shape
    floats = int(lib().pd3_winograd43_input_transform_floats(n, cin, h, w))
    if floats == 0:
        raise RuntimeError("winograd43_input_transform: cin must be a multiple of 8")
    if out is None or out.numel() < floats:
        out = torch.empty((floats,), dtype=torch.float32, device=xx.device)
    check(lib().pd3_winograd43_input_transform(ptr(xx), n, cin, h, w, w if w_valid is None else int(w_valid), ptr(out),
                                               stream_ptr(xx.device)), "winograd43_input_transform")
    return out


def conv3x3_winograd43_ppv_bias_relu(v_pre: torch.Tensor, shape, u_lane: torch.Tensor, bias, cout: int, relu: bool = True,
                                     out: torch.Tensor | None = None, w_valid: int | None = None) -> torch.Tensor:
    n, cin, h, w = (int(v) for v in shape)
    ul = require_gpu(u_lane, "conv3x3_winograd43_ppv_bias_relu")
    if ul.numel() != cout * cin * 36:
        raise RuntimeError("conv3x3_winograd43_ppv_bias_relu: u_lane does not belong to a [cout, cin, 3, 3] weight")
    if out is None:
        out = torch.empty((n, cout, h, w), dtype=torch.float32, device=v_pre.device)
    check(lib().pd3_conv3x3_winograd43_ppv_bias_relu(ptr(v_pre), ptr(ul), ptr(bias), n, cin, cout, h, w,
                                                     w if w_valid is None else int(w_valid), int(bool(relu)), ptr(out),
                                                     stream_ptr(v_pre.device)), "conv3x3_winograd43_ppv_bias_relu")
    return out


def grouped_small_supported(cin_per_group: int, cout_per_group: int, h: int, w: int) -> bool:
    return 1 <= cout_per_group <= 4 and cin_per_group % 4 == 0 and w % 4 == 0


def pack_grouped_weight(weight: torch.Tensor, groups: int) -> torch.Tensor:
    gco, cg = weight.shape[:2]
    co = gco // groups
    return weight.reshape(groups, co, cg, 9).permute(0, 2, 1, 3).contiguous()


def grouped_conv3x3_small(x: torch.Tensor, w_grouped: torch.Tensor, bias, groups: int,
                          out: torch.Tensor | None = None, out_groups: int | None = None,
                          out_group0: int = 0) -> torch.Tensor:
    xx = require_gpu(x, "grouped_conv3x3_small")
    n, c, h, w = xx.shape
    cg, co = w_grouped.shape[1], w_grouped.shape[2]
    assert c == groups * cg
    total = groups if out_groups is None else int(out_groups)
    if out is None:
        out = torch.empty((n, total * co, h, w), dtype=torch.float32, device=xx.device)
    assert out.is_contiguous() and tuple(out.shape) == (n, total * co, h, w)
    check(lib().pd3_grouped_conv3x3_small_slice(ptr(xx), ptr(w_grouped), ptr(bias), n, groups, cg, co, h, w, ptr(out),
                                                total, int(out_group0), stream_ptr(xx.device)),
          "grouped_conv3x3_small")
    return out


def f16_tile(cout: int) -> int:
    return 128 if cout % 128 == 0 else 64


def f16_supported(cin: int, cout: int, h: int, w: int) -> bool:
    t = f16_tile(cout)
    return cin % 16 == 0 and cout % t == 0 and h > 0 and w > 0


def pack_conv3x3_f16_weight(weight: torch.Tensor, tile: int | None = None) -> torch.Tensor:
    cout, cin = weight.shape[:2]
    t = f16_tile(cout) if tile is None else tile
    assert weight.shape[2:] == (3, 3) and cout % t == 0 and cin % 16 == 0 and t in (64, 128)
    w = weight.to(torch.float16).reshape(cout // t, t, cin // 16, 2, 8, 9).permute(0, 2, 5, 3, 1, 4)
    return w.contiguous()


def to_f16_nhwc(x: torch.Tensor) -> torch.Tensor:
    xx = require_gpu(x, "f32_nchw_to_f16_nhwc")
    n, c, h, w = xx.shape
    out = torch.empty((n, h, w, c), dtype=torch.float16, device=xx.device)
    check(lib().pd3_f32_nchw_to_f16_nhwc(ptr(xx), n, c, h, w, ptr(out), stream_ptr(xx.device)), "f32_nchw_to_f16_nhwc")
    return out


def conv3x3_f16_bias_relu(x: torch.Tensor, w_packed: torch.Tensor, bias, cout: int, relu: bool = True,
                          out_f32_nchw: bool = False, out: torch.Tensor | None = None,
                          group_major: bool = False) -> torch.Tensor:
    if x.dtype != torch.float16 or not x.is_cuda or not x.is_contiguous():
        raise RuntimeError("conv3x3_f16_bias_relu: x must be a contiguous fp16 NHWC tensor on the GPU")
    n, h, w, cin = x.shape
    tile = int(w_packed.shape[4])
    if out is None:
        out = (torch.empty((n, cout, h, w), dtype=torch.float32, device=x.device) if out_f32_nchw
               else torch.empty((n, cout // 64, h, w, 64) if group_major else (n, h, w, cout), dtype=torch.float16,
                                device=x.device))
    assert not (group_major and out_f32_nchw)
    check(lib().pd3_conv3x3_f16_bias_relu(ptr(x), ptr(w_packed), ptr(bias), n, cin, cout, h, w, int(bool(relu)),
                                          ptr(out), 1 if out_f32_nchw else (3 if group_major else 0), tile,
                                          stream_ptr(x.device)),
          "conv3x3_f16_bias_relu")
    return out


def conv3x3_f16_bias_relu_dual(x: torch.Tensor, w_packed: torch.Tensor, bias, cout: int, relu: bool = True):
    if x.dtype != torch.float16 or not x.is_cuda or not x.is_contiguous():
        raise RuntimeError("conv3x3_f16_bias_relu: x must be a contiguous fp16 NHWC tensor on the GPU")
    n, h, w, cin = x.shape
    tile = int(w_packed.shape[4])
    oh = torch.empty((n, h, w, cout), dtype=torch.float16, device=x.device)
    of = torch.empty((n, cout, h, w), dtype=torch.float32, device=x.device)
    check(lib().pd3_conv3x3_f16_bias_relu_dual(ptr(x), ptr(w_packed), ptr(bias), n, cin, cout, h, w, int(bool(relu)),
                                               ptr(oh), ptr(of), tile, stream_ptr(x.device)),
          "conv3x3_f16_bias_relu_dual")
    return oh, of


def s2_f16_supported(cin: int, cout: int) -> bool:
    return cin % 16 == 0 and cout % 128 == 0


def conv3x3_s2_f16_bias_relu(x: torch.Tensor, w_packed: torch.Tensor, bias, cout: int, relu: bool = True) -> torch.Tensor:
    if x.dtype != torch.float16 or not x.is_cuda or not x.is_contiguous():
        raise RuntimeError("conv3x3_s2_f16_bias_relu: x must be a contiguous fp16 NHWC tensor on the GPU")
    n, h, w, cin = x.shape
    assert int(w_packed.shape[4]) == 128
    out = torch.empty((n, (h - 1) // 2 + 1, (w - 1) // 2 + 1, cout), dtype=torch.float16, device=x.device)
    check(lib().pd3_conv3x3_s2_f16_bias_relu(ptr(x), ptr(w_packed), ptr(bias), n, cin, cout, h, w, int(bool(relu)),
                                             ptr(out), stream_ptr(x.device)), "conv3x3_s2_f16_bias_relu")
    return out


def scatter_conv_s2_f16_supported(cin: int, cout: int, ny: int, nx: int) -> bool:
    return cin % 16 == 0 and cout % 64 == 0 and ny % 2 == 0 and nx % 2 == 0


def scatter_conv3x3_s2_f16_bias_relu(canvas, w_packed: torch.Tensor, bias, cout: int, relu: bool = True) -> torch.Tensor:
    f, inv = canvas.features, canvas.inv
    fh = f if f.dtype == torch.float16 else f.half()
    n, cin, ny, nx = canvas.shape
    tile = int(w_packed.shape[4])
    out = torch.empty((n, (ny - 1) // 2 + 1, (nx - 1) // 2 + 1, cout), dtype=torch.float16, device=f.device)
    check(lib().pd3_scatter_conv3x3_s2_f16_bias_relu(ptr(fh), ptr(inv), ptr(w_packed), ptr(bias), n, cin, cout, ny, nx,
                                                     int(bool(relu)), ptr(out), tile, stream_ptr(f.device)),
          "scatter_conv3x3_s2_f16_bias_relu")
    return out


def pack_grouped_weight_f16(weight: torch.Tensor, groups: int) -> torch.Tensor:
    gco, cg = weight.shape[:2]
    co = gco // groups
    assert weight.shape[2:] == (3, 3) and cg == 64 and gco == groups * co and 1 <= co <= 4
    return weight.to(torch.float16).reshape(groups, co, cg, 9).permute(0, 3, 1, 2).contiguous()


def grouped_conv3x3_small_f16(x_h: torch.Tensor, w_f16: torch.Tensor, bias, groups: int,
                              out: torch.Tensor | None = None, out_groups: int | None = None,
                              out_group0: int = 0, group_major: bool = False) -> torch.Tensor:
    if x_h.dtype != torch.float16 or not x_h.is_cuda or not x_h.is_contiguous():
        raise RuntimeError("grouped_conv3x3_small_f16: x must be a contiguous fp16 tensor on the GPU")
    if group_major:
        n, gg, h, w, c64 = x_h.shape
        c = gg * c64
        assert c64 == 64
    else:
        n, h, w, c = x_h.shape
    co = int(w_f16.shape[2])
    assert c == groups * 64 and tuple(w_f16.shape) == (groups, 9, co, 64)
    total = groups if out_groups is None else int(out_groups)
    if out is None:
        out = torch.empty((n, total * co, h, w), dtype=torch.float32, device=x_h.device)
    assert out.is_contiguous() and tuple(out.shape) == (n, total * co, h, w)
    fn = lib().pd3_grouped_conv3x3_small_f16_gm if group_major else lib().pd3_grouped_conv3x3_small_f16
    check(fn(ptr(x_h), ptr(w_f16.contiguous()), ptr(bias), n, groups, 64, co, h, w, ptr(out), total, int(out_group0),
             stream_ptr(x_h.device)), "grouped_conv3x3_small_f16")
    return out


WINOGRAD43_PP_MIN_CIN = 64


def winograd43_pp_supported(cin: int, cout: int, h: int, w: int) -> bool:
    return cin % 8 == 0 and cout % 64 == 0 and w % 4 == 0


def pack_winograd43_lane_weight(weight: torch.Tensor) -> torch.Tensor:
    cout, cin = weight.shape[:2]
    assert weight.shape[2:] == (3, 3) and cout % 64 == 0 and cin % 8 == 0
    u = _winograd43_u(weight).reshape(cout // 64, 4, 16, cin // 8, 2, 4, 9, 4).permute(0, 3, 4, 1, 6, 5, 2, 7)
    return u.contiguous()


def conv3x3_winograd43_pp_bias_relu(x: torch.Tensor, u_lane: torch.Tensor, bias, cout: int, relu: bool = True,
                                    out: torch.Tensor | None = None, w_valid: int | None = None) -> torch.Tensor:
    xx = require_gpu(x, "conv3x3_winograd43_pp_bias_relu")
    ul = require_gpu(u_lane, "conv3x3_winograd43_pp_bias_relu")
    n, cin, h, w = xx.shape
    if ul.numel() != cout * cin * 36:
        raise RuntimeError("conv3x3_winograd43_pp_bias_relu: u_lane does not belong to a [cout, cin, 3, 3] weight")
    if out is None:
        out = torch.empty((n, cout, h, w), dtype=torch.float32, device=xx.device)
    check(lib().pd3_conv3x3_winograd43_pp_bias_relu(ptr(xx), ptr(ul), ptr(bias), n, cin, cout, h, w,
                                                    w if w_valid is None else int(w_valid), int(bool(relu)),
                                                    ptr(out), stream_ptr(xx.device)),
          "conv3x3_winograd43_pp_bias_relu")
    return out
```

Baseline: 2313.

## Add per-group cout grouped conv kernel and specialize winograd43 kernels for whole tiles

Adds a grouped 3x3 conv kernel that takes a real output-channel count per group. It computes only the real heatmap channels, zero-fills the padding, and stages input through LDS with buffer-load DMA and double buffering. The CenterPoint head now uses it for the per-class heatmap conv. Separately, the winograd43 pp/ppv kernels are templated on relu, debug and whole-tile flags, drop the accumulator zeroing by feeding zeros into the first MFMA pass, and skip bounds checks on whole tiles. It also adds -fno-slp-vectorize for those files, at the cost of more template instantiations and compile time.

Measured after the change: 2404 (median of 6 runs). 1.04x the previous value.

```diff
diff --git a/include/paddle3d_amd.h b/include/paddle3d_amd.h
--- a/include/paddle3d_amd.h
+++ b/include/paddle3d_amd.h
@@ -362,6 +362,9 @@
 int pd3_grouped_conv3x3_small_slice(const float *x, const float *w_grouped, const float *bias, int batch, int groups,
                                     int cin_per_group, int cout_per_group, int h, int w, float *out, int out_groups,
                                     int out_group0, void *stream);
+int pd3_grouped_conv3x3_small_counts_slice(const float *x, const float *w_grouped, const float *bias, int batch, int groups,
+                                           int cin_per_group, int cout_per_group, const int *group_couts, int h, int w,
+                                           float *out, int out_groups, int out_group0, void *stream);
 
 int pd3_conv3x3_winograd_bias_relu(const float *x, const float *u_packed, const float *bias, int batch,
                                    int cin, int cout, int h, int w, int relu, float *out, void *stream);
diff --git a/paddle3d_amd/_lib.py b/paddle3d_amd/_lib.py
--- a/paddle3d_amd/_lib.py
+++ b/paddle3d_amd/_lib.py
@@ -236,6 +236,14 @@
 
 SYMBOLS_ROI = tuple(_SIGNATURES_ROI)
 
+_SIGNATURES_HEAD = {
+    "pd3_grouped_conv3x3_small_counts_slice": (C.c_int, [C.c_void_p, C.c_void_p, C.c_void_p, C.c_int, C.c_int, C.c_int,
+                                                         C.c_int, C.c_void_p, C.c_int, C.c_int, C.c_void_p, C.c_int,
+                                                         C.c_int, C.c_void_p]),
+}
+
+SYMBOLS_HEAD = tuple(_SIGNATURES_HEAD)
+
 
 class Paddle3DAmdError(RuntimeError):
     pass
@@ -248,7 +256,8 @@
             f"{LIB_PATH} not found: build it with `python -m paddle3d_amd.build` "
             "(there is no CPU / PyTorch fallback for the HIP ops)")
     handle = C.CDLL(LIB_PATH)
-    for name, (res, args) in list(_SIGNATURES.items()) + list(_SIGNATURES_ROI.items()):
+    for name, (res, args) in (list(_SIGNATURES.items()) + list(_SIGNATURES_ROI.items()) +
+                              list(_SIGNATURES_HEAD.items())):
         try:
             fn = getattr(handle, name)
         except AttributeError as e:
diff --git a/paddle3d_amd/build.py b/paddle3d_amd/build.py
--- a/paddle3d_amd/build.py
+++ b/paddle3d_amd/build.py
@@ -22,6 +22,7 @@
 def _headers():
     hs = [os.path.join(CSRC, f) for f in os.listdir(CSRC) if f.endswith(".hpp")]
     hs.append(os.path.join(HERE, "..", "include", "paddle3d_amd.h"))
+    hs.append(os.path.abspath(__file__))
     return hs
 
 
@@ -32,7 +33,7 @@
     return any(os.path.getmtime(d) > t for d in deps)
 
 
-EXTRA_FLAGS = {}
+EXTRA_FLAGS = {"conv_winograd43_pp.hip": ["-fno-slp-vectorize"], "conv_winograd43_ppv.hip": ["-fno-slp-vectorize"]}
 
 
 def _compile(src, force):
diff --git a/paddle3d_amd/centerpoint.py b/paddle3d_amd/centerpoint.py
--- a/paddle3d_amd/centerpoint.py
+++ b/paddle3d_amd/centerpoint.py
@@ -699,7 +699,9 @@
                 else:
                     wino(x, u[c0:c1], first.b[c0 * 64:c1 * 64], (c1 - c0) * 64, relu=True, out=y)
                 _conv.grouped_conv3x3_small(y, f["pf"][c0:c1], f["bf"][c0 * f["cmax"]:c1 * f["cmax"]], c1 - c0, out=z,
-                                            out_groups=groups, out_group0=c0)
+                                            out_groups=groups, out_group0=c0,
+                                            group_couts=(f["ncls"][c0:c1]
+                                                         if c1 - c0 <= _conv.GROUPED_COUNTS_MAX_GROUPS else None))
         else:
             y, _ = first(x)
             z = _conv.grouped_conv3x3_small(y, f["pf"], f["bf"], groups)
diff --git a/paddle3d_amd/csrc/conv3x3.hip b/paddle3d_amd/csrc/conv3x3.hip
--- a/paddle3d_amd/csrc/conv3x3.hip
+++ b/paddle3d_amd/csrc/conv3x3.hip
@@ -1,5 +1,6 @@
 #include "../../include/paddle3d_amd.h"
 #include "common.hpp"
+#include "lds_dma.hpp"
 
 
 namespace pd3 {
@@ -220,6 +221,7 @@
 constexpr int kGcCi = 4;
 constexpr int kGcR = 8, kGcW = 128;
 constexpr int kGcXR = kGcR + 2, kGcXW = kGcW + 8;
+constexpr int kGcMaxGroups = 64;
 
 template <int CO>
 __global__ __launch_bounds__(256) void grouped_conv3x3_small_kernel(const float* __restrict__ x,
@@ -307,6 +309,115 @@
       *reinterpret_cast<cv_f32x4*>(out + ((int64_t)n * out_groups * CO + (out_group0 + g) * CO + c) * plane +
                                    (int64_t)(y0 + tr) * w + x0 + tc) = v;
   }
+}
+
+constexpr int kGnR = 16, kGnXR = kGnR + 2, kGnT = kGnR * 32;
+constexpr int kGcBuf = (kGcCi * kGnXR * kGcXW / 4 + 63) / 64 * 256;
+struct gc_counts {
+  int n[kGcMaxGroups];
+};
+
+template <int CO, int NC>
+__device__ __forceinline__ void grouped_counts_body(const float* __restrict__ x, const float* __restrict__ wg,
+                                                    const float* __restrict__ bias, float* __restrict__ out,
+                                                    const int groups, const int cg, const int h, const int w,
+                                                    const int out_groups, const int out_group0, float* Xs, const int pt,
+                                                    const int g) {
+  constexpr int XQ = kGcXW / 4, XN4 = kGcCi * kGnXR * XQ;
+  constexpr int XPT = (XN4 + kGnT - 1) / kGnT;
+  const int tiles_x = (w + kGcW - 1) / kGcW, tiles_y = (h + kGnR - 1) / kGnR;
+  const int tx = pt % tiles_x, ty = (pt / tiles_x) % tiles_y, n = pt / (tiles_x * tiles_y);
+  const int y0 = ty * kGnR, x0 = tx * kGcW;
+  const int tr = threadIdx.x >> 5, tc = (threadIdx.x & 31) * 4;
+  const int wave = __builtin_amdgcn_readfirstlane(threadIdx.x >> 6);
+  const int64_t plane = (int64_t)h * w;
+  const float* xin = x + ((int64_t)n * groups + g) * cg * plane;
+  const float* wgp = wg + (int64_t)g * cg * CO * 9;
+  float acc[NC][4];
+#pragma unroll
+  for (int c = 0; c < NC; ++c)
+#pragma unroll
+    for (int p = 0; p < 4; ++p) acc[c][p] = 0.f;
+  unsigned gofs[XPT];
+#pragma unroll
+  for (int i = 0; i < XPT; ++i) {
+    const int e = min((int)threadIdx.x + i * kGnT, XN4 - 1);
+    const int ci = e / (kGnXR * XQ), rem = e - ci * (kGnXR * XQ);
+    const int r = rem / XQ, c4 = rem - r * XQ;
+    const int gy = y0 - 1 + r, gx = x0 - 4 + c4 * 4;
+    const bool ok = gy >= 0 && gy < h && gx >= 0 && gx < w;
+    gofs[i] = ok ? (unsigned)(4 * (ci * plane + (int64_t)gy * w + gx)) : 0x7ffffff0u;
+  }
+  auto fetch = [&](const int c0) {
+    float* dst = Xs + ((c0 / kGcCi) & 1) * kGcBuf + wave * 256;
+#pragma unroll
+    for (int i = 0; i < XPT; ++i)
+      if ((i + 1) * kGnT <= XN4 || (int)threadIdx.x + i * kGnT < XN4)
+        pp_dma(xin + (int64_t)c0 * plane, (unsigned)(kGcCi * plane * 4), dst + i * kGnT * 4, gofs[i], 0);
+  };
+  fetch(0);
+  for (int c0 = 0; c0 < cg; c0 += kGcCi) {
+    __builtin_amdgcn_s_waitcnt(0x0f70);
+    w4_lds_barrier();
+    if (c0 + kGcCi < cg) fetch(c0 + kGcCi);
+    const float* Xb = Xs + ((c0 / kGcCi) & 1) * kGcBuf;
+#pragma unroll
+    for (int ci = 0; ci < kGcCi; ++ci) {
+      const float* wc = wgp + (int64_t)(c0 + ci) * CO * 9;
+#pragma unroll
+      for (int ky = 0; ky < 3; ++ky) {
+        const float* row = Xb + (ci * kGnXR + tr + ky) * kGcXW + tc;
+        const cv_f32x4 mid = *reinterpret_cast<const cv_f32x4*>(row + 4);
+        float in[6];
+        in[1] = mid[0];
+        in[2] = mid[1];
+        in[3] = mid[2];
+        in[4] = mid[3];
+        in[0] = row[3];
+        in[5] = row[8];
+#pragma unroll
+        for (int c = 0; c < NC; ++c)
+#pragma unroll
+          for (int kx = 0; kx < 3; ++kx) {
+            const float wv = wc[c * 9 + ky * 3 + kx];
+#pragma unroll
+            for (int p = 0; p < 4; ++p) acc[c][p] = __builtin_fmaf(wv, in[p + kx], acc[c][p]);
+          }
+      }
+    }
+  }
+  if (y0 + tr >= h || x0 + tc >= w) return;
+  float* o = out + ((int64_t)n * out_groups * CO + (out_group0 + g) * CO) * plane + (int64_t)(y0 + tr) * w + x0 + tc;
+#pragma unroll
+  for (int c = 0; c < CO; ++c) {
+    cv_f32x4 v = {0.f, 0.f, 0.f, 0.f};
+    if (c < NC) {
+      const float b = bias ? bias[g * CO + c] : 0.f;
+      v = (cv_f32x4){acc[c][0] + b, acc[c][1] + b, acc[c][2] + b, acc[c][3] + b};
+    }
+    *reinterpret_cast<cv_f32x4*>(o + c * plane) = v;
+  }
+}
+
+template <int CO>
+__global__ __launch_bounds__(kGnT) void grouped_conv3x3_small_counts_kernel(const float* __restrict__ x,
+                                                                            const float* __restrict__ wg,
+                                                                            const float* __restrict__ bias,
+                                                                            float* __restrict__ out, int groups, int cg,
+                                                                            int h, int w, int out_groups, int out_group0,
+                                                                            const gc_counts counts) {
+  __shared__ __attribute__((aligned(16))) float Xs[2 * kGcBuf];
+  const int g = blockIdx.y, pt = blockIdx.x;
+  const int nc = counts.n[g];
+#define PD3_GCB(NC)                                                                                              \
+  if constexpr (NC <= CO)                                                                                        \
+    if (nc == NC)                                                                                                \
+    return grouped_counts_body<CO, NC>(x, wg, bias, out, groups, cg, h, w, out_groups, out_group0, Xs, pt, g)
+  PD3_GCB(1);
+  PD3_GCB(2);
+  PD3_GCB(3);
+  PD3_GCB(4);
+#undef PD3_GCB
 }
 
 }
@@ -407,3 +518,34 @@
   return grouped_small_launch(x, w_grouped, bias, batch, groups, cin_per_group, cout_per_group, h, w, out, out_groups,
                               out_group0, stream);
 }
+
+extern "C" int pd3_grouped_conv3x3_small_counts_slice(const float* x, const float* w_grouped, const float* bias,
+                                                      int batch, int groups, int cin_per_group, int cout_per_group,
+                                                      const int* group_couts, int h, int w, float* out, int out_groups,
+                                                      int out_group0, void* stream) {
+  if (!x || !w_grouped || !out || !group_couts || batch <= 0 || groups <= 0 || cin_per_group <= 0 || h <= 0 || w <= 0 ||
+      out_group0 < 0 || out_group0 + groups > out_groups)
+    return PD3_EINVAL;
+  if (cout_per_group < 1 || cout_per_group > 4 || cin_per_group % kGcCi != 0 || w % 4 != 0 || groups > kGcMaxGroups)
+    return PD3_EUNSUPPORTED;
+  if ((int64_t)kGcCi * h * w >= (int64_t)1 << 29) return PD3_EUNSUPPORTED;
+  if (reinterpret_cast<uintptr_t>(x) % 16 != 0 || reinterpret_cast<uintptr_t>(out) % 16 != 0) return PD3_EINVAL;
+  gc_counts counts = {};
+  for (int g = 0; g < groups; ++g) {
+    if (group_couts[g] < 1 || group_couts[g] > cout_per_group) return PD3_EINVAL;
+    counts.n[g] = group_couts[g];
+  }
+  hipStream_t s = static_cast<hipStream_t>(stream);
+  dim3 grid((unsigned)((int64_t)batch * ceil_div(h, kGnR) * ceil_div(w, kGcW)), (unsigned)groups);
+#define PD3_GC(CO)                                                                                                   \
+  grouped_conv3x3_small_counts_kernel<CO><<<grid, kGnT, 0, s>>>(x, w_grouped, bias, out, groups, cin_per_group, h, w, \
+                                                                out_groups, out_group0, counts)
+  switch (cout_per_group) {
+    case 1: PD3_GC(1); break;
+    case 2: PD3_GC(2); break;
+    case 3: PD3_GC(3); break;
+    default: PD3_GC(4); break;
+  }
+#undef PD3_GC
+  return launch_status();
+}
diff --git a/paddle3d_amd/csrc/conv_winograd43.hpp b/paddle3d_amd/csrc/conv_winograd43.hpp
--- a/paddle3d_amd/csrc/conv_winograd43.hpp
+++ b/paddle3d_amd/csrc/conv_winograd43.hpp
@@ -1,6 +1,7 @@
 #pragma once
 #include "../../include/paddle3d_amd.h"
 #include "common.hpp"
+#include "lds_dma.hpp"
 
 #include <type_traits>
 
@@ -44,7 +45,6 @@
   return __builtin_bit_cast(float, __builtin_amdgcn_mov_dpp(__builtin_bit_cast(int, v), 0xB1, 0xf, 0xf, true));
 }
 
-__device__ __forceinline__ void w4_lds_barrier() { asm volatile("s_waitcnt lgkmcnt(0)\n\ts_barrier" ::: "memory"); }
 
 __device__ inline void w4_pair_transform(const float (&rv)[3][6], const int hf, float* v) {
   float lo[3][3], hi[3][3];
@@ -78,7 +78,7 @@
 struct w4_no_hook {
   __device__ __forceinline__ void operator()() const {}
 };
-template <int N, int HOOK = -1, class UA, class VP, class F = w4_no_hook>
+template <int N, int HOOK = -1, bool FIRST = false, class UA, class VP, class F = w4_no_hook>
 __device__ __forceinline__ void w4_mfma_stream(w4_f32x4 (&acc)[36], const UA& ua, const VP& vptr, const F& hook = F()) {
   constexpr bool kRing = !std::is_array<UA>::value;
   w4_f32x4 a[3], b[3];
@@ -97,7 +97,9 @@
       float av;
       if constexpr (kRing) av = a[g % 3][j];
       else av = ua[g][j];
-      acc[(g % 9) * 4 + j] = __builtin_amdgcn_mfma_f32_16x16x4f32(av, b[g % 3][j], acc[(g % 9) * 4 + j], 0, 0, 0);
+      const w4_f32x4 zero = {0.f, 0.f, 0.f, 0.f};
+      acc[(g % 9) * 4 + j] =
+          __builtin_amdgcn_mfma_f32_16x16x4f32(av, b[g % 3][j], FIRST && g < 9 ? zero : acc[(g % 9) * 4 + j], 0, 0, 0);
     }
     __builtin_amdgcn_sched_barrier(0);
     if (g == HOOK) {
@@ -107,6 +109,7 @@
   }
 }
 
+template <int RELU = -1, bool WHOLE = false>
 __device__ __forceinline__ void w4_output_step(const w4_f32x4 (&acc)[36], const w4_f32x4 bv, const int n, const int cout,
                                                const int co0, const int oy, const int ox, const int h, const int w,
                                                const int wv, const int relu, const int64_t plane,
@@ -130,10 +133,10 @@
 #pragma unroll
       for (int j = 0; j < 4; ++j) {
         y4[j] += bv[r];
-        if (relu) y4[j] = fmaxf(y4[j], 0.f);
-        if (ox + j >= wv) y4[j] = 0.f;
+        if (RELU < 0 ? relu != 0 : RELU != 0) y4[j] = fmaxf(y4[j], 0.f);
+        if (!WHOLE && ox + j >= wv) y4[j] = 0.f;
       }
-      if (oy + k < h && ox < w)
+      if (WHOLE || (oy + k < h && ox < w))
         __builtin_nontemporal_store((w4_f32x4){y4[0], y4[1], y4[2], y4[3]},
                                     reinterpret_cast<w4_f32x4*>(o + (int64_t)k * w));
     }
@@ -162,6 +165,8 @@
   return PD3_OK;
 }
 
+inline bool w4_whole(int h, int w, int w_valid) { return w_valid == w && h % (4 * kW4TR) == 0 && w % (4 * kW4TC) == 0; }
+
 inline int64_t w4_grid(int batch, int h, int w, int groups, int64_t* ptiles) {
   *ptiles = (int64_t)batch * ceil_div(h, 4 * kW4TR) * ceil_div(w, 4 * kW4TC);
   return (*ptiles + 7) / 8 * 8 * groups;
diff --git a/paddle3d_amd/csrc/conv_winograd43_pp.hip b/paddle3d_amd/csrc/conv_winograd43_pp.hip
--- a/paddle3d_amd/csrc/conv_winograd43_pp.hip
+++ b/paddle3d_amd/csrc/conv_winograd43_pp.hip
@@ -11,6 +11,7 @@
 constexpr int kPpRawSz = kPpCi * kPpRawPl;
 constexpr int kPpXPT = (2 * kPpRawPl / 4 + 63) / 64;
 
+template <bool DBG, int RELU, bool WHOLE>
 __global__ __launch_bounds__(512, 1) void conv3x3_winograd43_pp_kernel(const float* __restrict__ x,
                                                                        const float* __restrict__ ulane,
                                                                        const float* __restrict__ bias,
@@ -18,7 +19,7 @@
                                                                        int w, int wv, int relu, int ptiles,
                                                                        long long* __restrict__ dbg) {
   constexpr int CO = 64;
-  long long t_tr = 0, t_mu = 0, t_ba = 0, t_all = dbg ? clock64() : 0;
+  long long t_tr = 0, t_mu = 0, t_ba = 0, t_all = DBG ? clock64() : 0;
   extern __shared__ __attribute__((aligned(16))) float smem[];
   const int lane = lane_id(), wave = __builtin_amdgcn_readfirstlane(wave_id());
   const int grp = wave >> 2, cb = wave & 3;
@@ -26,6 +27,7 @@
   float* Us = smem;
   float* Raw = smem + kPpUsz + grp * (kPpRawSz + kPpVsz);
   float* Vs = Raw + kPpRawSz;
+  float* bias_s = smem + kPpUsz + 2 * (kPpRawSz + kPpVsz);
   const w4_tile tl = w4_decode_block(cout / CO, h, w);
   if (tl.pt >= ptiles) return;
   const int ct = tl.cg, n = tl.n, y0 = tl.y0, x0 = tl.x0;
@@ -51,9 +53,12 @@
   const int bbase = pp_bbase(lane);
   const float* uct = ulane + (int64_t)ct * slots * kPpUsz;
 
+  constexpr bool PEEL = WHOLE;
   w4_f32x4 acc[36];
-#pragma unroll
-  for (int c = 0; c < 36; ++c) acc[c] = (w4_f32x4){0.f, 0.f, 0.f, 0.f};
+  if constexpr (!PEEL) {
+#pragma unroll
+    for (int c = 0; c < 36; ++c) acc[c] = (w4_f32x4){0.f, 0.f, 0.f, 0.f};
+  }
 
   auto fetch_x = [&](int s) {
 #pragma unroll
@@ -87,28 +92,31 @@
     __builtin_amdgcn_s_waitcnt(0x0f70);
     read_rows();
   };
-  auto multiply_ring = [&]() { w4_mfma_stream<18, 15>(acc, uptr, vptr, next_rows); };
-  auto multiply_regs = [&]() { w4_mfma_stream<18, 16>(acc, ua, vptr, next_rows); };
-
+  auto multiply_ring = [&](auto first) { w4_mfma_stream<18, 15, decltype(first)::value>(acc, uptr, vptr, next_rows); };
+  auto multiply_regs = [&](auto first) { w4_mfma_stream<18, 16, decltype(first)::value>(acc, ua, vptr, next_rows); };
+
+  if (threadIdx.x < CO) bias_s[threadIdx.x] = bias ? bias[ct * CO + threadIdx.x] : 0.f;
   fetch_x(0);
   if (grp == 0) {
     fetch_u(0, 0);
     fetch_u(0, 1);
   }
-  __builtin_amdgcn_s_waitcnt(0x0f70);
-  read_rows();
-  w4_lds_barrier();
   auto sync = [&]() {
-    const long long c1 = dbg ? clock64() : 0;
+    const long long c1 = DBG ? clock64() : 0;
     w4_lds_barrier();
-    if (dbg) t_ba += clock64() - c1;
+    if (DBG) t_ba += clock64() - c1;
   };
   auto run = [&](auto is_g0) {
     constexpr bool G0 = decltype(is_g0)::value;
+    if constexpr (PEEL) {
+      __builtin_amdgcn_s_waitcnt(0x0f70);
+      read_rows();
+      w4_lds_barrier();
+    }
     if (!G0) sync();
-    for (int s = 0; s < slots; ++s) {
+    auto slot = [&](const int s, auto first) {
       {
-        const long long c0 = dbg ? clock64() : 0;
+        const long long c0 = DBG ? clock64() : 0;
         const int sn = min(s + 1, slots - 1);
         if (G0) {
           if (s > 0) {
@@ -125,53 +133,67 @@
 #pragma unroll
           for (int g = 9; g < 18; ++g) ua[g] = *reinterpret_cast<const w4_f32x4*>(uptr(g));
         }
-        if (dbg) t_tr += clock64() - c0;
+        if (DBG) t_tr += clock64() - c0;
       }
       sync();
       {
-        const long long c0 = dbg ? clock64() : 0;
-        if (G0) multiply_ring();
-        else multiply_regs();
-        if (dbg) t_mu += clock64() - c0;
+        const long long c0 = DBG ? clock64() : 0;
+        if (G0) multiply_ring(first);
+        else multiply_regs(first);
+        if (DBG) t_mu += clock64() - c0;
       }
       sync();
-    }
+    };
+    if constexpr (PEEL) slot(0, std::true_type{});
+    for (int s = PEEL ? 1 : 0; s < slots; ++s) slot(s, std::false_type{});
     if (G0) sync();
-  };
+    if (DBG && blockIdx.x == 8 && lane == 0) {
+      dbg[wave * 4 + 0] = t_tr;
+      dbg[wave * 4 + 1] = t_mu;
+      dbg[wave * 4 + 2] = t_ba;
+      dbg[wave * 4 + 3] = (clock64() - t_all) | ((long long)__builtin_amdgcn_s_getreg(2308) << 56);
+    }
+    const int cl = cb * 16 + 4 * (lane >> 4);
+    const w4_f32x4 bv = *reinterpret_cast<const w4_f32x4*>(bias_s + cl);
+    w4_output_step<RELU, WHOLE>(acc, bv, n, cout, ct * CO + cl, y0 + 4 * grp, x0 + 4 * (lane & 15), h, w, wv, relu, plane,
+                                out);
+  };
+  if constexpr (!PEEL) {
+    __builtin_amdgcn_s_waitcnt(0x0f70);
+    read_rows();
+    w4_lds_barrier();
+  }
   if (grp == 0) run(std::true_type{});
   else run(std::false_type{});
-  if (dbg && blockIdx.x == 8 && lane == 0) {
-    dbg[wave * 4 + 0] = t_tr;
-    dbg[wave * 4 + 1] = t_mu;
-    dbg[wave * 4 + 2] = t_ba;
-    dbg[wave * 4 + 3] = (clock64() - t_all) | ((long long)__builtin_amdgcn_s_getreg(2308) << 56);
-  }
-
-  w4_f32x4 bv = {0.f, 0.f, 0.f, 0.f};
-  const int co0 = ct * CO + cb * 16 + 4 * (lane >> 4);
-  if (bias) {
-#pragma unroll
-    for (int r = 0; r < 4; ++r) bv[r] = bias[co0 + r];
-  }
-  w4_output_step(acc, bv, n, cout, co0, y0 + 4 * grp, x0 + 4 * (lane & 15), h, w, wv, relu, plane, out);
 }
 
 }
 
 using namespace pd3;
 
-static int launch_wino43_pp(const float* x, const float* u_lane, const float* bias, int batch, int cin, int cout, int h,
-                            int w, int w_valid, int relu, float* out, hipStream_t s, long long* dbg = nullptr) {
-  constexpr size_t lds = ((size_t)kPpUsz + 2 * (kPpRawSz + kPpVsz)) * sizeof(float);
-  const void* fn = reinterpret_cast<const void*>(conv3x3_winograd43_pp_kernel);
+template <bool DBG, int RELU, bool WHOLE>
+static int launch_wino43_pp_as(const float* x, const float* u_lane, const float* bias, int batch, int cin, int cout, int h,
+                               int w, int w_valid, int relu, float* out, hipStream_t s, long long* dbg) {
+  constexpr size_t lds = ((size_t)kPpUsz + 2 * (kPpRawSz + kPpVsz) + 64) * sizeof(float);
+  const void* fn = reinterpret_cast<const void*>(conv3x3_winograd43_pp_kernel<DBG, RELU, WHOLE>);
   hipError_t e = pd3_max_dynamic_lds(fn, (int)lds);
   if (e != hipSuccess) return (int)e;
   int64_t ptiles;
   const int64_t nwg = w4_grid(batch, h, w, cout / 64, &ptiles);
   if (nwg >= (int64_t)1 << 31) return PD3_EUNSUPPORTED;
-  conv3x3_winograd43_pp_kernel<<<(unsigned)nwg, 512, lds, s>>>(x, u_lane, bias, out, cin, cout, h, w, w_valid, relu,
-                                                               (int)ptiles, dbg);
+  conv3x3_winograd43_pp_kernel<DBG, RELU, WHOLE><<<(unsigned)nwg, 512, lds, s>>>(x, u_lane, bias, out, cin, cout, h, w,
+                                                                                 w_valid, relu, (int)ptiles, dbg);
   return launch_status();
+}
+
+static int launch_wino43_pp(const float* x, const float* u_lane, const float* bias, int batch, int cin, int cout, int h,
+                            int w, int w_valid, int relu, float* out, hipStream_t s, long long* dbg = nullptr) {
+#define PD3_PP(DBG, RELU, WHOLE) \
+  launch_wino43_pp_as<DBG, RELU, WHOLE>(x, u_lane, bias, batch, cin, cout, h, w, w_valid, relu, out, s, dbg)
+  if (!w4_whole(h, w, w_valid)) return dbg ? PD3_PP(true, -1, false) : PD3_PP(false, -1, false);
+  if (dbg) return relu ? PD3_PP(true, 1, true) : PD3_PP(true, 0, true);
+  return relu ? PD3_PP(false, 1, true) : PD3_PP(false, 0, true);
+#undef PD3_PP
 }
 
 static int check_wino43_pp(const float* x, const float* u_lane, const float* out, int batch, int cin, int cout, int h,
diff --git a/paddle3d_amd/csrc/conv_winograd43_pp.hpp b/paddle3d_amd/csrc/conv_winograd43_pp.hpp
--- a/paddle3d_amd/csrc/conv_winograd43_pp.hpp
+++ b/paddle3d_amd/csrc/conv_winograd43_pp.hpp
@@ -9,10 +9,6 @@
 constexpr int kPpUHalf = 9 * 64 * 4;
 constexpr int kPpUsz = kPpKT * 4 * kPpUHalf;
 
-__device__ __forceinline__ void pp_dma(const float* base, unsigned bytes, float* lds, unsigned voff, unsigned soff) {
-  const __amdgpu_buffer_rsrc_t r = __builtin_amdgcn_make_buffer_rsrc(const_cast<float*>(base), 0, (int)bytes, 0x00020000);
-  __builtin_amdgcn_raw_ptr_buffer_load_lds(r, (__attribute__((address_space(3))) void*)lds, 16, (int)voff, (int)soff, 0, 0);
-}
 
 __device__ __forceinline__ int pp_bbase(int lane) { return ((lane >> 4) * kW4TC + (lane & 15)) * kW4Cs; }
 __device__ __forceinline__ const float* pp_vptr(const float* V, int bbase, int g) {
diff --git a/paddle3d_amd/csrc/conv_winograd43_ppv.hip b/paddle3d_amd/csrc/conv_winograd43_ppv.hip
--- a/paddle3d_amd/csrc/conv_winograd43_ppv.hip
+++ b/paddle3d_amd/csrc/conv_winograd43_ppv.hip
@@ -48,6 +48,7 @@
   for (int i = 0; i < kPpVsz / 4 / 128; ++i) out4[threadIdx.x + i * 128] = b4[threadIdx.x + i * 128];
 }
 
+template <int RELU, bool WHOLE>
 __global__ __launch_bounds__(512, 1) void conv3x3_winograd43_ppv_kernel(const float* __restrict__ vpre,
                                                                         const float* __restrict__ ulane,
                                                                         const float* __restrict__ bias,
@@ -72,8 +73,6 @@
   const int nv = cb < 2 ? 5 : 4;
 
   w4_f32x4 acc[36];
-#pragma unroll
-  for (int c = 0; c < 36; ++c) acc[c] = (w4_f32x4){0.f, 0.f, 0.f, 0.f};
 
   auto fetch_v = [&](int s) {
     float* dst = Vs + (s & 1) * kPpVsz;
@@ -91,8 +90,12 @@
   };
   auto uptr = [&](int g) { return pp_uptr(Us, cb, lane, g); };
   w4_f32x4 ua[18];
-  auto multiply_ring = [&](const float* V) { w4_mfma_stream<18>(acc, uptr, [&](int g) { return pp_vptr(V, bbase, g); }); };
-  auto multiply_regs = [&](const float* V) { w4_mfma_stream<18>(acc, ua, [&](int g) { return pp_vptr(V, bbase, g); }); };
+  auto multiply_ring = [&](const float* V, auto first) {
+    w4_mfma_stream<18, -1, decltype(first)::value>(acc, uptr, [&](int g) { return pp_vptr(V, bbase, g); });
+  };
+  auto multiply_regs = [&](const float* V, auto first) {
+    w4_mfma_stream<18, -1, decltype(first)::value>(acc, ua, [&](int g) { return pp_vptr(V, bbase, g); });
+  };
 
   for (int t = threadIdx.x; t < ipw * CO; t += 512) bias_s[t] = bias ? bias[ct0 * CO + t] : 0.f;
   fetch_v(0);
@@ -105,7 +108,7 @@
   auto run = [&](auto is_g0) {
     constexpr bool G0 = decltype(is_g0)::value;
     if (!G0) w4_lds_barrier();
-    for (int s = 0; s < slots; ++s) {
+    auto slot = [&](const int s, auto first) {
       {
         if (G0 && s > 0) {
           fetch_u(ct, s, 0);
@@ -129,11 +132,13 @@
       w4_lds_barrier();
       {
         const float* V = Vs + (s & 1) * kPpVsz;
-        if (G0) multiply_ring(V);
-        else multiply_regs(V);
+        if (G0) multiply_ring(V, first);
+        else multiply_regs(V, first);
       }
       w4_lds_barrier();
-    }
+    };
+    slot(0, std::true_type{});
+    for (int s = 1; s < slots; ++s) slot(s, std::false_type{});
     if (G0) w4_lds_barrier();
   };
   auto blocks = [&](auto is_g0) {
@@ -150,10 +155,8 @@
 
   const int co0 = ct * CO + cb * 16 + 4 * (lane >> 4);
   const w4_f32x4 b4 = *reinterpret_cast<const w4_f32x4*>(bias_s + it * CO + cb * 16 + 4 * (lane >> 4));
-  w4_output_step(acc, b4, n, cout, co0, y0 + 4 * grp, x0 + 4 * (lane & 15), h, w, wv, relu, plane, out);
+  w4_output_step<RELU, WHOLE>(acc, b4, n, cout, co0, y0 + 4 * grp, x0 + 4 * (lane & 15), h, w, wv, relu, plane, out);
   if (it + 1 < ipw) {
-#pragma unroll
-    for (int c = 0; c < 36; ++c) acc[c] = (w4_f32x4){0.f, 0.f, 0.f, 0.f};
     if (whole_tiles) __builtin_amdgcn_s_waitcnt(0x0f70 | (16 & 15) | ((16 >> 4) << 14));
     else __builtin_amdgcn_s_waitcnt(0x0f70);
     w4_lds_barrier();
@@ -203,12 +206,19 @@
   for (int d = 2; d <= kPvMaxBlocks; ++d)
     if (nct % d == 0 && ptiles8 * (nct / d) >= 6 * 256) ipw = d;
   const size_t lds = ((size_t)kPpUsz + 4 * kPpVsz + kPvMaxBlocks * 64) * sizeof(float);
-  const void* fn = reinterpret_cast<const void*>(conv3x3_winograd43_ppv_kernel);
-  const hipError_t e = pd3_max_dynamic_lds(fn, (int)lds);
-  if (e != hipSuccess) return (int)e;
   const int64_t nwg = ptiles8 * (nct / ipw);
   if (nwg >= (int64_t)1 << 31) return PD3_EUNSUPPORTED;
-  conv3x3_winograd43_ppv_kernel<<<(unsigned)nwg, 512, lds, static_cast<hipStream_t>(stream)>>>(
-      v_pre, u_lane, bias, out, cin, cout, h, w, w_valid, relu, (int)ptiles, ipw);
+#define PD3_PV(RELU, WHOLE)                                                                                              \
+  do {                                                                                                                   \
+    const void* fn = reinterpret_cast<const void*>(conv3x3_winograd43_ppv_kernel<RELU, WHOLE>);                          \
+    const hipError_t e = pd3_max_dynamic_lds(fn, (int)lds);                                                              \
+    if (e != hipSuccess) return (int)e;                                                                                  \
+    conv3x3_winograd43_ppv_kernel<RELU, WHOLE><<<(unsigned)nwg, 512, lds, static_cast<hipStream_t>(stream)>>>(           \
+        v_pre, u_lane, bias, out, cin, cout, h, w, w_valid, relu, (int)ptiles, ipw);                                     \
+  } while (0)
+  if (!w4_whole(h, w, w_valid)) PD3_PV(-1, false);
+  else if (relu) PD3_PV(1, true);
+  else PD3_PV(0, true);
+#undef PD3_PV
   return launch_status();
 }
diff --git a/paddle3d_amd/csrc/lds_dma.hpp b/paddle3d_amd/csrc/lds_dma.hpp
--- /dev/null
+++ b/paddle3d_amd/csrc/lds_dma.hpp
@@ -0,0 +1,12 @@
+#pragma once
+
+namespace pd3 {
+
+__device__ __forceinline__ void w4_lds_barrier() { asm volatile("s_waitcnt lgkmcnt(0)\n\ts_barrier" ::: "memory"); }
+
+__device__ __forceinline__ void pp_dma(const float* base, unsigned bytes, float* lds, unsigned voff, unsigned soff) {
+  const __amdgpu_buffer_rsrc_t r = __builtin_amdgcn_make_buffer_rsrc(const_cast<float*>(base), 0, (int)bytes, 0x00020000);
+  __builtin_amdgcn_raw_ptr_buffer_load_lds(r, (__attribute__((address_space(3))) void*)lds, 16, (int)voff, (int)soff, 0, 0);
+}
+
+}
diff --git a/paddle3d_amd/ops/conv.py b/paddle3d_amd/ops/conv.py
--- a/paddle3d_amd/ops/conv.py
+++ b/paddle3d_amd/ops/conv.py
@@ -1,4 +1,6 @@
 from __future__ import annotations
+
+import ctypes
 
 import torch
 
@@ -337,9 +339,12 @@
     return weight.reshape(groups, co, cg, 9).permute(0, 2, 1, 3).contiguous()
 
 
+GROUPED_COUNTS_MAX_GROUPS = 64
+
+
 def grouped_conv3x3_small(x: torch.Tensor, w_grouped: torch.Tensor, bias, groups: int,
                           out: torch.Tensor | None = None, out_groups: int | None = None,
-                          out_group0: int = 0) -> torch.Tensor:
+                          out_group0: int = 0, group_couts=None) -> torch.Tensor:
     xx = require_gpu(x, "grouped_conv3x3_small")
     n, c, h, w = xx.shape
     cg, co = w_grouped.shape[1], w_grouped.shape[2]
@@ -348,6 +353,13 @@
     if out is None:
         out = torch.empty((n, total * co, h, w), dtype=torch.float32, device=xx.device)
     assert out.is_contiguous() and tuple(out.shape) == (n, total * co, h, w)
+    if group_couts is not None:
+        assert len(group_couts) == groups
+        counts = (ctypes.c_int * groups)(*[int(c) for c in group_couts])
+        check(lib().pd3_grouped_conv3x3_small_counts_slice(ptr(xx), ptr(w_grouped), ptr(bias), n, groups, cg, co, counts, h,
+                                                           w, ptr(out), total, int(out_group0), stream_ptr(xx.device)),
+              "grouped_conv3x3_small")
+        return out
     check(lib().pd3_grouped_conv3x3_small_slice(ptr(xx), ptr(w_grouped), ptr(bias), n, groups, cg, co, h, w, ptr(out),
                                                 total, int(out_group0), stream_ptr(xx.device)),
           "grouped_conv3x3_small")
```
